# nv-tlabs/DiffusionTexturePainting

Hardware: AMD Instinct MI355X
Metric: 512x512 inpaint stamps/sec @20 DDIM steps (higher is better)
Workload: dtype f16

## Files before the change

diffusiontexturepainting_amd/_lib.py:

```python
import ctypes as C
import os

import torch

_HERE = os.path.dirname(os.path.abspath(__file__))
LIB_PATH = os.environ.get("DTP_LIB") or os.path.join(_HERE, "libdtp.so")
_lib = None
MAX_SLOTS = 16
SCHEDULERS = {"DDIM": 0, "DPM": 1, "LMSD": 2}
SCHED_ROW = 8


def scheduler_id(name):
    if name not in SCHEDULERS:
        raise ValueError(f"scheduler {name!r} is not supported: choose one of {', '.join(SCHEDULERS)}")
    return SCHEDULERS[name]


class DtpError(RuntimeError):
    pass


class Settings(C.Structure):
    _fields_ = [("steps", C.c_int), ("context_pad", C.c_int), ("tg_steps", C.c_int), ("cfg_weight", C.c_float),
# ... 85 lines not shown
                                   "host_ids_offset", "host_tiles_offset", "host_bytes")]


class ProfRow(C.Structure):
    _fields_ = [("kind", C.c_int), ("launches", C.c_int), ("ms", C.c_double), ("flops", C.c_double), ("bytes", C.c_double)]


_SHAPES = [(128, 128), (128, 64), (64, 64), (64, 128)]
PROF_KINDS = [f"gemm_kernel<{_SHAPES[i & 3][0]}, {_SHAPES[i & 3][1]}, {2 + i // 4}>" for i in range(12)] + \
    ["attention_kernel", "groupnorm (gn_stats+gn_apply | gn_fused)", "layernorm_kernel", "concat_kernel / small elementwise",
     "softmax_rows_kernel", "conv_halo_kernel<8, 16, 64>", "conv_halo_kernel<8, 16, 128>", "conv_halo_kernel<8, 8, 64>",
     "conv_halo_kernel<8, 8, 128>", "gemm_kernel<256, 128, 2>", "gemm_kernel<256, 128, 3>", "gemm_kernel<128, 256, 2>",
     "gemm_kernel<128, 256, 3>", "gemm_wide_kernel<256, 256>", "gemm_wide_kernel<256, 320>", "gemm_fp8_kernel"] + \
    [f"gemm_kernel<{_SHAPES[i & 3][0]}, {_SHAPES[i & 3][1]}, {2 + i // 4}, 2>" for i in range(8)] + \
    [f"gemm_kernel<{_SHAPES[i & 3][0]}, {_SHAPES[i & 3][1]}, 3, 1, {(4, 8)[i // 4]}>" for i in range(8)] + \
    ["xattn_kernel (cross-attention GEMM pair)", "conv_halo_kernel<8, 8, 64, 3 images>", "conv_halo_kernel<8, 8, 128, 3 images>",
     "lnlin_kernel (activation-stationary LayerNorm-folded Linear / GEGLU)", "convws_kernel<8, 8, 3 images>", "convws_kernel<16, 16>", "convws_kernel<8, 16, 2 n-tiles>", "convws_kernel<8, 16, 2 n-tiles, 2 workgroups per CU>",
     "gemmws_kernel (weight-streaming dense GEMM)", "gemm_f8f8_kernel (two-operand e4m3 GEMM)", "quant8_kernel (e4m3 quantise pass)"]


class GemmDesc(C.Structure):
    _fields_ = [("A", C.c_void_p), ("W", C.c_void_p), ("C", C.c_void_p), ("bias", C.c_void_p), ("R", C.c_void_p),
                ("M", C.c_int), ("N", C.c_int), ("K", C.c_int),
                ("lda", C.c_int), ("ldw", C.c_int), ("ldc", C.c_int), ("ldr", C.c_int),
                ("conv", C.c_int), ("Hi", C.c_int), ("Wi", C.c_int), ("Ho", C.c_int), ("Wo", C.c_int), ("Cin", C.c_int),
                ("stride", C.c_int), ("pad", C.c_int), ("upsample2x", C.c_int),
                ("flags", C.c_int), ("tile", C.c_int), ("splits", C.c_int), ("lns", C.c_void_p), ("ln_eps", C.c_float),
                ("A2", C.c_void_p), ("lda2", C.c_int), ("Cin2", C.c_int), ("Wcb", C.c_void_p),
                ("batch", C.c_int), ("a_bs", C.c_int64), ("w_bs", C.c_int64), ("c_bs", C.c_int64), ("r_bs", C.c_int64),
                ("bias_bs", C.c_int), ("lns_bs", C.c_int), ("sm_valid", C.c_int),
                ("st_out", C.c_void_p), ("st_in", C.c_void_p), ("st_parts", C.c_int), ("st_parts_out", C.c_int),
                ("W8", C.c_void_p), ("ldw8", C.c_int), ("a_scale", C.c_float), ("w_scale", C.c_float), ("gn_cpg", C.c_int), ("Wfr", C.c_void_p),
                ("A8", C.c_void_p), ("lda8", C.c_int), ("A2_8", C.c_void_p), ("lda2_8", C.c_int), ("C8", C.c_void_p), ("ldc8", C.c_int),
                ("c_scale", C.c_float), ("a2_scale", C.c_float)]


GF_BIAS, GF_BIAS_M, GF_RESID, GF_GEGLU, GF_GELU, GF_QUICKGELU, GF_OUT_F32, GF_SILU, GF_LNFOLD = 1, 2, 4, 8, 64, 128, 256, 512, 1024
GF_SOFTMAX16 = 4096
GF_ROWSTATS = 2048
GF_GNSTATS = 1 << 24
GF_RAGGED = 1 << 25

_vp, _i, _f, _i64 = C.c_void_p, C.c_int, C.c_float, C.c_int64
SYMBOLS = {
    "dtp_abi_version": (_i, []),
    "dtp_last_error": (C.c_char_p, []),
    "dtp_create": (_i, [_i, _i, _i, C.POINTER(_vp)]),
    "dtp_destroy": (None, [_vp]),
    "dtp_load_tensor": (_i, [_vp, C.c_char_p, _vp, _i, C.POINTER(_i64), _i]),
    "dtp_finalize_weights": (_i, [_vp]),
    "dtp_vae_encode": (_i, [_vp, _vp, _vp, _vp, _i, _vp]),
    "dtp_unet": (_i, [_vp, _vp, _f, _vp, _vp, _i, _vp]),
    "dtp_vae_decode": (_i, [_vp, _vp, _vp, _i, _vp]),
    "dtp_set_brush": (_i, [_vp, _vp, _i, _i, _vp, _vp]),
    "dtp_set_conditioning": (_i, [_vp, _vp, _vp, _vp, _vp]),
    "dtp_get_conditioning": (_i, [_vp, _vp, _vp, _vp]),
    "dtp_stamp": (_i, [_vp, _vp, C.POINTER(Settings), _vp, _vp, _vp, _i, _vp]),
    "dtp_stamp_slots": (_i, [_vp, _vp, C.POINTER(Settings), _vp, _vp, _vp, _i, C.POINTER(_i), _vp]),
    "dtp_stamp_mixed": (_i, [_vp, _vp, C.POINTER(Settings), _vp, _vp, _vp, _i, C.POINTER(_i), _vp]),
    "dtp_set_brush_slot": (_i, [_vp, _i, _vp, _i, _i, _vp, _vp]),
    "dtp_set_conditioning_slot": (_i, [_vp, _i, _vp, _vp, _vp, _vp]),
    "dtp_get_conditioning_slot": (_i, [_vp, _i, _vp, _vp, _vp]),
    "dtp_ddim_tables": (_i, [_i, C.POINTER(_i64), C.POINTER(_f), C.POINTER(_f)]),
    "dtp_last_stamp_times": (_i, [_vp, C.POINTER(_f * 3)]),
    "dtp_last_stamp_info": (_i, [_vp, C.POINTER(_i), C.POINTER(_i)]),
    "dtp_last_stamp_unet_rows": (_i, [_vp, C.POINTER(_i)]),
    "dtp_profile": (_i, [_vp, _i]),
    "dtp_profile_rows": (_i, [_vp, C.POINTER(ProfRow), _i, C.POINTER(_i)]),
    "dtp_profile_dump": (_i, [_vp, C.c_char_p]),
    "dtp_set_option": (_i, [_vp, C.c_char_p, _i]),
    "dtp_last_stamp_finite": (_i, [_vp, C.POINTER(_i)]),
    "dtp_op_gemm": (_i, [C.POINTER(GemmDesc), _vp]),
    "dtp_op_gemm_f8f8": (_i, [C.POINTER(GemmDesc), _vp]),
    "dtp_op_quant_e4m3": (_i, [_vp, _i, _vp, _i, _i, _f, _i, _vp, _i, _vp, _i, _i, _f, _i, _i, _vp, _i, _f, _vp]),
    "dtp_op_pack_linear": (_i, [_vp, _vp, _i, _i, _i, _i, _vp]),
    "dtp_op_pack_conv": (_i, [_vp, _vp, _i, _i, _i, _i, _i, _vp]),
    "dtp_op_rowsum": (_i, [_vp, _i, _i, _vp, _i, _vp]),
    "dtp_op_quantize_w8": (_i, [_vp, _i, _i, _i, _vp, _i, C.POINTER(_f), _vp]),
    "dtp_op_pack_conv_cb": (_i, [_vp, _vp, _i, _i, _i, _vp]),
    "dtp_op_groupnorm_apply": (_i, [_vp, _i, _vp, _i, _vp, _vp, _vp, _i, _i, _i, _i, _i, _f, _i, _vp]),
    "dtp_op_groupnorm_stats_apply": (_i, [_vp, _i, _vp, _vp, _vp, _vp, _vp, _vp, _i, _i, _i, _i, _f, _i, _vp]),
    "dtp_op_pack_conv_ws": (_i, [_vp, _vp, _vp, _i, _i, _i, _vp]),
    "dtp_op_pack_conv_ws_elems": (C.c_longlong, [_i, _i, _i]),
    "dtp_op_pack_linear_ws": (_i, [_vp, _i, _vp, _i, _i, _vp]),
    "dtp_op_pack_linear_ws_elems": (C.c_longlong, [_i, _i]),
    "dtp_op_groupnorm": (_i, [_vp, _i, _vp, _i, _vp, _vp, _i, _i, _i, _i, _f, _i, _vp]),
    "dtp_op_measure_peaks": (_i, [C.POINTER(C.c_double), C.POINTER(C.c_double)]),
    "dtp_op_reduce_groupnorm": (_i, [_vp, _i, _vp, _vp, _vp, _vp, _vp, _vp, _i, _i, _i, _i, _f, _i, _vp]),
    "dtp_op_xattn": (_i, [_vp, _vp, _vp, _vp, _vp, _i, _vp, _vp, _vp, _vp, _vp, _i, _i, _i, _i, _f, _vp]),
    "dtp_op_reduce_groupnorm_cx": (_i, [_vp, _i, _vp, _vp, _vp, _vp, _vp, _vp, _i, _i, _i, _i, _f, _i, _i, _vp]),
    "dtp_op_xattn_ct": (_i, [_vp, _vp, _vp, _vp, _vp, _i, _vp, _vp, _vp, _vp, _vp, _i, _i, _i, _i, _f, _i, _vp]),
    "dtp_op_gn_fold_weights": (_i, [_vp, _vp, _i, _vp, _vp, _vp, _i, _i, _i, _i, _i, _f, _vp, _vp, _vp]),
    "dtp_op_ffchain": (_i, [_vp, _vp, _i, _vp, _vp, _vp, _i, _vp, _vp, _vp, _i, _i, _f, _vp]),
    "dtp_op_xchain": (_i, [_vp, _vp, _i, _vp, _vp, _vp, _vp, _vp, _vp, _vp, _vp, _vp, _i, _i, _i, _i, _f, _vp]),
    "dtp_op_gn_linear": (_i, [_vp, _vp, _i, _vp, _vp, _vp, _i, _i, _i, _i, _i, _f, _vp, _vp, _i, _vp]),
    "dtp_op_layernorm": (_i, [_vp, _i, _vp, _i, _vp, _vp, _i, _i, _f, _vp]),
    "dtp_op_attention": (_i, [_vp, _vp, _vp, _vp, _i, _i, _i, _i, _i, _i, _i, _i, _i, _i64, _i64, _i64, _i64, _f, _vp]),
    "dtp_op_attention_dma": (_i, [_vp, _vp, _vp, _vp, _i, _i, _i, _i, _i, _i, _i, _i, _i, _i64, _i64, _i64, _i64, _f, _i, _vp]),
    "dtp_op_softmax_rows": (_i, [_vp, _i, _vp, _i, _i, _i, _f, _vp]),
    "dtp_op_attention_fp8": (_i, [_vp, _vp, _vp, _vp, _i, _i, _i, _i, _i, _i, _i, _i, _i, _i64, _i64, _i64, _i64, _f, _f, _f, _vp]),
    "dtp_op_dilate": (_i, [_vp, _vp, _vp, _i, _i, _i, _vp]),
    "dtp_op_dilate_pads": (_i, [_vp, _vp, _vp, _i, _i, C.POINTER(_i), _vp]),
    "dtp_scheduler_tables": (_i, [_i, _i, C.POINTER(_i), C.POINTER(_f), C.POINTER(_f), C.POINTER(_f), C.POINTER(_f)]),
    "dtp_op_sched_step": (_i, [_i, _vp, _vp, _vp, _vp, _vp, _vp, _vp, _vp, _vp, _i, _i, _i, _i, _vp]),
    "dtp_stamp_strength": (_i, [_vp, _vp, C.POINTER(Settings), _vp, _vp, _vp, C.c_double, _vp, _i, C.POINTER(_i), _vp]),
    "dtp_strength_schedule": (_i, [_i, _i, C.c_double, C.POINTER(_i), C.POINTER(_i), C.POINTER(_f)]),
    "dtp_op_strength_init": (_i, [_vp, _vp, _f, _f, _vp, C.c_longlong, _vp]),
    "dtp_stamp_seeded": (_i, [_vp, _vp, C.POINTER(Settings), C.POINTER(C.c_uint64), _i, C.c_double, _vp, _i, C.POINTER(_i), _vp]),
    "dtp_op_stamp_noise": (_i, [C.c_uint64, _i, _vp, C.c_longlong, _vp]),
    "dtp_philox4x32": (_i, [C.POINTER(C.c_uint32), C.POINTER(C.c_uint32), C.POINTER(C.c_uint32)]),
    "dtp_refit_stage": (_i, [_vp, C.c_char_p, _vp, _i, C.POINTER(_i64), _i]),
    "dtp_refit_lora": (_i, [_vp, _f]),
    "dtp_last_refit_info": (_i, [_vp, C.POINTER(_i), C.POINTER(_i), C.POINTER(_f)]),
    "dtp_op_lora_refit": (_i, [_vp, _vp, _vp, _i, _f, _vp, _vp, _i, _i, _i, _i, _vp]),
    "dtp_stroke": (_i, [_vp, _vp, _i, _i, C.POINTER(StrokeStamp), _i, C.POINTER(Settings), C.POINTER(StrokeOpts), _vp, _vp]),
    "dtp_stroke_plan": (_i, [_i, _i, _i, _i, C.POINTER(StrokeStamp), _i, _i, C.POINTER(_i), C.POINTER(_i)]),
    "dtp_last_stroke_info": (_i, [_vp, C.POINTER(_i), C.POINTER(_i), C.POINTER(_i)]),
    "dtp_op_stroke_gather": (_i, [_vp, _i, _i, _vp, _i, _i, C.POINTER(_i), C.POINTER(_i), C.POINTER(_i), _i, _i, _i, _vp]),
    "dtp_op_stroke_paste": (_i, [_vp, _vp, _vp, _i, _i, _i, _i, C.POINTER(_i), C.POINTER(_i), C.POINTER(_i), _i, _vp]),
    "dtp_mesh_create": (_i, [_vp, _vp, _i, _vp, _i, _vp, C.POINTER(_vp)]),
    "dtp_mesh_destroy": (_i, [_vp]),
    "dtp_mesh_camera": (_i, [C.POINTER(_f * 3), C.POINTER(_f * 3), C.POINTER(_f * 3), _f, C.POINTER(_f * 12)]),
    "dtp_mesh_stroke": (_i, [_vp, _vp, _vp, _i, _i, C.POINTER(MeshStamp), _i, C.POINTER(Settings), C.POINTER(MeshStrokeOpts), _vp, _vp]),
    "dtp_op_mesh_render": (_i, [_vp, C.POINTER(_f * 12), _f, _i, _vp, _i, _i, _i, _i, _i, _i, _vp, _vp, _vp]),
    "dtp_op_mesh_backproject": (_i, [_vp, _vp, _i, _vp, _vp, _i, _vp, _i, _i, _vp]),
    "dtp_mesh_stroke_bleed": (_i, [_vp, _vp, _vp, _i, _i, C.POINTER(MeshStamp), _i, C.POINTER(Settings), C.POINTER(MeshStrokeOpts), _vp, _i, _vp]),
    "dtp_mesh_bleed": (_i, [_vp, _vp, _i, _i, _i, C.POINTER(_i * 4), _vp]),
    "dtp_op_mesh_coverage": (_i, [_vp, _i, _i, _vp, _vp]),
    "dtp_mesh_bleed_offsets": (_i, [_i, C.POINTER(_i), C.POINTER(C.c_byte)]),
    "dtp_mesh_pick": (_i, [_vp, C.POINTER(Ray), _i, _vp, _vp]),
    "dtp_mesh_ray_frame": (_i, [C.POINTER(_f * 3), C.POINTER(_f * 3), C.POINTER(_f * 12)]),
    "dtp_mesh_path_plan": (_i, [_vp, _i, _f, C.POINTER(PathState), _vp, _vp, _vp, _i, C.POINTER(_i)]),
    "dtp_op_mesh_pick": (_i, [_vp, C.POINTER(Ray), _i, _vp, _vp]),
    "dtp_view_camera": (_i, [C.POINTER(_f * 3), C.POINTER(_f * 3), C.POINTER(_f * 3), _f, _i, _i, _f, C.POINTER(ViewCam)]),
    "dtp_view_rays": (_i, [C.POINTER(ViewCam), _i, _i, _vp, _i, _vp]),
    "dtp_mesh_view": (_i, [_vp, _vp, _i, _i, C.POINTER(ViewCam), _i, _i, C.POINTER(ViewOpts), _vp, _vp, _vp, _vp]),
    "dtp_op_mesh_view": (_i, [_vp, _vp, _i, _i, C.POINTER(ViewCam), _i, _i, C.POINTER(ViewOpts), _vp, _vp, _vp, _i, _vp]),
    "dtp_mip_layout": (_i, [_i, _i, C.POINTER(MipLevels)]),
    "dtp_texture_mips": (_i, [_vp, _i, _i, _vp, C.c_uint64, _vp]),
    "dtp_mesh_view_mips": (_i, [_vp, _vp, _i, _i, _vp, C.POINTER(ViewCam), _i, _i, C.POINTER(ViewOpts), _vp, _vp, _vp, _vp, _vp]),
    "dtp_mesh_view_clip": (_i, [_vp, _vp, _i, _i, _vp, C.POINTER(ViewCam), _i, _i, C.POINTER(ViewOpts), _i, _vp, _vp, _vp, _vp, _vp]),
    "dtp_op_mesh_view_clip": (_i, [_vp, _vp, _i, _i, _vp, C.POINTER(ViewCam), _i, _i, C.POINTER(ViewOpts), _i, _vp, _vp, _vp, _vp, _i, _vp]),
    "dtp_mesh_view_aa": (_i, [_vp, _vp, _i, _i, _vp, C.POINTER(ViewCam), _i, _i, C.POINTER(ViewOpts), _i, _i, _i, _vp, _vp, _vp, _vp, _vp, _vp]),
    "dtp_op_mesh_view_aa": (_i, [_vp, _vp, _i, _i, _vp, C.POINTER(ViewCam), _i, _i, C.POINTER(ViewOpts), _i, _i, _i, _vp, _vp, _vp, _vp, _vp, _i,
                                 _vp]),
    "dtp_mesh_view_aniso": (_i, [_vp, _vp, _i, _i, _vp, C.POINTER(ViewCam), _i, _i, C.POINTER(ViewOpts), _i, _i, _i, _vp, _vp, _vp, _vp, _vp, _vp,
                                 _vp]),
    "dtp_op_mesh_view_aniso": (_i, [_vp, _vp, _i, _i, _vp, C.POINTER(ViewCam), _i, _i, C.POINTER(ViewOpts), _i, _i, _i, _vp, _vp, _vp, _vp, _vp, _vp,
                                    _i, _vp]),
    "dtp_mesh_select": (_i, [_vp, _vp, _i, _i, _vp, _i, _i, _vp, _i, _vp]),
    "dtp_mesh_stroke_masked": (_i, [_vp, _vp, _vp, _i, _i, C.POINTER(MeshStamp), _i, C.POINTER(Settings), C.POINTER(MeshStrokeOpts), _vp, _i, _vp, _i,
                                    _vp]),
    "dtp_view_tint": (_i, [_vp, _vp, _vp, _i, _i, _vp, _i, _i, C.POINTER(C.c_uint8 * 3), _i, _vp]),
    "dtp_op_mesh_backproject_masked": (_i, [_vp, _vp, _i, _vp, _vp, _i, _vp, _i, _i, _vp, _i, _vp]),
    "dtp_journal_create": (_i, [_vp, _vp, _i, _i, _i, _i, C.POINTER(_vp)]),
    "dtp_journal_destroy": (_i, [_vp]),
    "dtp_journal_begin": (_i, [_vp, _vp]),
    "dtp_journal_end": (_i, [_vp, _vp]),
    "dtp_journal_touch": (_i, [_vp, C.POINTER(_i), _i, _vp]),
    "dtp_journal_undo": (_i, [_vp, _vp]),
    "dtp_journal_redo": (_i, [_vp, _vp]),
    "dtp_journal_info": (_i, [_vp, C.POINTER(_i), C.POINTER(_i), C.POINTER(_i), C.POINTER(C.c_uint64)]),
    "dtp_journal_record_info": (_i, [_vp, _i, C.POINTER(C.c_uint64), C.POINTER(C.c_uint64), C.POINTER(_i)]),
    "dtp_op_journal_tiles": (_i, [_vp, _i, C.POINTER(_i), _i, C.POINTER(_i)]),
    "dtp_journal_window_tiles": (_i, [_i, _i, _i, _i, _i, _i, C.POINTER(_i), _i, C.POINTER(_i)]),
    "dtp_delta_layout": (_i, [_i, _i, _i, C.POINTER(DeltaSizes)]),
# ... 38 lines not shown
```

diffusiontexturepainting_amd/csrc/api_ops.hip:

```cpp
#include <stdarg.h>
#include <stdio.h>
#include <stdlib.h>
#include <mutex>
#include <vector>

#include "../../include/dtp.h"
#include "common.h"

static thread_local char g_err[1024] = "";

void dtp_set_error(const char* fmt, ...) {
  va_list ap;
  va_start(ap, fmt);
  vsnprintf(g_err, sizeof(g_err), fmt, ap);
  va_end(ap);
}

namespace {
struct OpsScratch {
  f16* zero = nullptr;
  float* ws = nullptr;
  size_t ws_bytes = 0;
  int* geglu_map = nullptr;
  int geglu_map_n = 0;
  int num_cu = 256;
  bool init = false;
};
OpsScratch g_ops;
std::mutex g_ops_mu;

int ops_init() {
  if (g_ops.init) return DTP_OK;
  HIP_CHECK(hipMalloc(&g_ops.zero, 256));
  HIP_CHECK(hipMemset(g_ops.zero, 0, 256));
  hipDeviceProp_t prop;
  int dev = 0;
  HIP_CHECK(hipGetDevice(&dev));
  HIP_CHECK(hipGetDeviceProperties(&prop, dev));
  g_ops.num_cu = prop.multiProcessorCount;
  g_ops.init = true;
  return DTP_OK;
}

int ops_ws(size_t bytes) {
  if (bytes <= g_ops.ws_bytes) return DTP_OK;
  HIP_CHECK(hipDeviceSynchronize());
  if (g_ops.ws) HIP_CHECK(hipFree(g_ops.ws));
  g_ops.ws = nullptr;
  g_ops.ws_bytes = 0;
  HIP_CHECK(hipMalloc(&g_ops.ws, bytes));
  g_ops.ws_bytes = bytes;
  return DTP_OK;
}
}

extern "C" {

int dtp_abi_version(void) { return DTP_ABI_VERSION; }
const char* dtp_last_error(void) { return g_err; }

int dtp_op_gemm(dtp_gemm_desc* d, dtp_stream s) {
  std::lock_guard<std::mutex> lk(g_ops_mu);
  int rc = ops_init();
  if (rc) return rc;
  static bool halo_init = false;
  if (!halo_init) { dtp_conv_halo_init(); dtp_gemm_wide_init(); dtp_lnlin_init(); dtp_conv_ws_init(); dtp_gemm_ws_init(); halo_init = true; }
  GemmParams p = {};
  p.A = (const f16*)d->A; p.W = (const f16*)d->W; p.C = d->C; p.bias = d->bias; p.R = (const f16*)d->R;
  p.zero = g_ops.zero;
  p.M = d->M; p.N = d->N; p.K = d->K;
  p.lda = d->lda; p.ldw = d->ldw; p.ldc = d->ldc; p.ldr = d->ldr;
  p.nkb = (d->K + 63) / 64;
  p.Hi = d->Hi; p.Wi = d->Wi; p.Ho = d->Ho; p.Wo = d->Wo; p.Cin = d->Cin; p.stride = d->stride; p.pad = d->pad;
  p.flags = d->flags | (d->conv ? GF_CONV3 : 0) | (d->upsample2x ? GF_UPS2 : 0);
  p.lns = d->lns; p.ln_eps = d->ln_eps;
  p.A2 = (const f16*)d->A2; p.lda2 = d->lda2; p.Cin2 = d->Cin2;
  p.batch = d->batch; p.a_bs = d->a_bs; p.w_bs = d->w_bs; p.c_bs = d->c_bs; p.r_bs = d->r_bs;
  p.bias_bs = d->bias_bs; p.lns_bs = d->lns_bs; p.sm_valid = d->sm_valid;
  p.st_out = d->st_out; p.st_in = d->st_in; p.st_parts = d->st_parts;
  if (p.batch > 1) p.st_rows = p.batch * p.M;
  p.W8 = (const unsigned char*)d->W8; p.ldw8 = d->ldw8; p.a_scale = d->a_scale; p.w_scale = d->w_scale;
  p.Wfr = (const f16*)d->Wfr;
  p.gn_cpg = d->gn_cpg;
  static bool fp8_init = false;
  if (!fp8_init) { dtp_gemm_fp8_init(); fp8_init = true; }
  if (p.ldw < p.nkb * 64) { dtp_set_error("gemm: ldw=%d smaller than padded K=%d", p.ldw, p.nkb * 64); return DTP_ERR_ARG; }
  int tile = 0;
  dtp_gemm_pick(p, &tile, g_ops.num_cu);
  if (d->tile >= 0) tile = d->tile;
  const DtpTile t = dtp_tile(tile);
  int sp = t.split == SPLIT_COLS ? 4 : t.split == SPLIT_K ? p.splits : 1;
  if (d->splits >= 1 && (d->batch <= 1 || t.split != SPLIT_K)) sp = d->splits;
  if ((t.fam == TF_FP8) != (p.W8 != nullptr)) { dtp_set_error("gemm: tiles 24..28 and W8 go together"); return DTP_ERR_ARG; }
  if (t.fam == TF_HALO && !d->Wcb) { dtp_set_error("conv_halo: Wcb missing"); return DTP_ERR_ARG; }
  p.Wcb = (const f16*)d->Wcb;
  (void)dtp_tile_apply(p, tile, sp);
  rc = ops_ws(dtp_gemm_workspace_bytes(p));
  if (rc) return rc;
  p.part = g_ops.ws;
  if (p.flags & GF_ROWSTATS) d->st_parts_out = dtp_tile_row_parts(p, tile);
  return dtp_launch_tile(p, tile, (hipStream_t)s);
}

int dtp_op_gemm_f8f8(dtp_gemm_desc* d, dtp_stream s) {
  std::lock_guard<std::mutex> lk(g_ops_mu);
  int rc = ops_init();
  if (rc) return rc;
  static bool f8f8_init = false;
  if (!f8f8_init) { dtp_gemm_f8f8_init(); f8f8_init = true; }
  GemmParams p = {};
  p.A8 = (const unsigned char*)d->A8; p.lda8 = d->lda8;
  p.A2_8 = (const unsigned char*)d->A2_8; p.lda2_8 = d->lda2_8; p.Cin2 = d->A2_8 ? d->Cin2 : 0;
  p.W8 = (const unsigned char*)d->W8; p.ldw8 = d->ldw8;
  p.C = d->C; p.ldc = d->ldc; p.C8 = (unsigned char*)d->C8; p.ldc8 = d->ldc8;
  p.bias = d->bias; p.R = (const f16*)d->R; p.ldr = d->ldr;
  p.zero = g_ops.zero;
  p.M = d->M; p.N = d->N; p.K = d->K;
  p.flags = d->flags;
  p.st_out = d->st_out;
  p.a_scale = d->a_scale; p.w_scale = d->w_scale; p.c_scale = d->c_scale; p.a2_scale = d->a2_scale;
  p.splits = 1;
  const int tile = d->tile >= 0 ? d->tile : dtp_gemm_f8f8_pick(p, g_ops.num_cu);
  if (p.flags & GF_ROWSTATS) d->st_parts_out = (p.N + 127) / 128;
  return dtp_launch_gemm_f8f8(p, tile, (hipStream_t)s);
}

int dtp_op_quant_e4m3(const void* x, int ldx, void* y, int ldy, int K, float scale, int ln, const void* x2, int ldx2, void* y2, int ldy2,
                      int K2, float scale2, int ln2, int M, const float* st_in, int st_parts, float eps, dtp_stream s) {
  Quant8Params q = {};
  q.M = M; q.njobs = x2 ? 2 : 1;
  q.job[0] = Quant8Job{(const f16*)x, ldx, K, (unsigned char*)y, ldy, scale, ln};
  if (x2) q.job[1] = Quant8Job{(const f16*)x2, ldx2, K2, (unsigned char*)y2, ldy2, scale2, ln2};
  q.st_in = st_in; q.st_parts = st_parts; q.st_rows = M; q.eps = eps;
  return dtp_launch_quant8(q, (hipStream_t)s);
}

int dtp_op_pack_linear(const float* w, void* out, int N, int K, int ldw, int geglu, dtp_stream s) {
  std::lock_guard<std::mutex> lk(g_ops_mu);
  int rc = ops_init();
  if (rc) return rc;
  const int* map = nullptr;
  if (geglu) {
    if (N % 256) { dtp_set_error("pack_linear: GEGLU needs N %% 256 == 0"); return DTP_ERR_ARG; }
    std::vector<int> h(N);
    for (int f = 0; f < N / 2; ++f) {
      h[f] = (f / 64) * 128 + (f % 64);
      h[N / 2 + f] = (f / 64) * 128 + 64 + (f % 64);
    }
    if (g_ops.geglu_map_n < N) {
      if (g_ops.geglu_map) HIP_CHECK(hipFree(g_ops.geglu_map));
      HIP_CHECK(hipMalloc(&g_ops.geglu_map, sizeof(int) * N));
      g_ops.geglu_map_n = N;
    }
    HIP_CHECK(hipMemcpyAsync(g_ops.geglu_map, h.data(), sizeof(int) * N, hipMemcpyHostToDevice, (hipStream_t)s));
    HIP_CHECK(hipStreamSynchronize((hipStream_t)s));
    map = g_ops.geglu_map;
  }
  return dtp_launch_pack_linear_weight(w, (f16*)out, N, K, ldw, map, (hipStream_t)s);
}

int dtp_op_quantize_w8(const void* w, int ldw, int K, int rows, void* out, int ldw8, float* w_scale, dtp_stream s) {
  if (!w || !out || !w_scale || (ldw8 & 127) || ldw8 < K) { dtp_set_error("quantize_w8: bad argument"); return DTP_ERR_ARG; }
  return dtp_quantize_weights_fp8((const f16*)w, ldw, K, rows, (unsigned char*)out, ldw8, w_scale, (hipStream_t)s);
}

int dtp_op_rowsum(const void* w, int ld, int K, float* out, int rows, dtp_stream s) {
  return dtp_launch_rowsum_f16((const f16*)w, ld, K, out, rows, (hipStream_t)s);
}

int dtp_op_pack_conv(const float* w, void* out, int Cout, int Cin, int Cin_pad, int taps, int ldw, dtp_stream s) {
  return dtp_launch_pack_conv_weight(w, (f16*)out, Cout, Cin, Cin_pad, taps, ldw, (hipStream_t)s);
}

int dtp_op_pack_conv_cb(const float* w, void* out, int Cout, int Cin, int ldw, dtp_stream s) {
  return dtp_launch_pack_conv_weight_cb(w, (f16*)out, Cout, Cin, ldw, (hipStream_t)s);
}

int dtp_op_pack_conv_ws(const float* w, const float* w1, void* out, int Cout, int Cin, int Cin2, dtp_stream s) {
  return dtp_launch_pack_conv_ws(w, w1, (f16*)out, Cout, Cin, Cin2, (hipStream_t)s);
}
int dtp_op_pack_linear_ws(const void* w, int ldw, void* out, int N, int K, dtp_stream s) {
  return dtp_launch_pack_linear_ws((const f16*)w, ldw, (f16*)out, N, K, (hipStream_t)s);
}
long long dtp_op_pack_linear_ws_elems(int N, int K) { return (long long)dtp_gemm_ws_packed_elems(N, K); }
long long dtp_op_pack_conv_ws_elems(int Cout, int Cin, int Cin2) { return (long long)dtp_conv_ws_packed_elems(Cout, Cin, Cin2); }

int dtp_op_groupnorm(const void* x, int ldx, void* y, int ldy, const float* gamma, const float* beta, int B, int HW, int C,
                     int groups, float eps, int silu, dtp_stream s) {
  std::lock_guard<std::mutex> lk(g_ops_mu);
  int rc = ops_init();
  if (rc) return rc;
  rc = ops_ws(dtp_groupnorm_ws_bytes(B, HW, C, groups));
  if (rc) return rc;
  return dtp_launch_groupnorm(GnParams{(const f16*)x, ldx, (f16*)y, ldy, gamma, beta, B, HW, C, groups, eps, silu}, g_ops.ws, (hipStream_t)s);
}

int dtp_op_groupnorm_apply(const void* x, int ldx, void* y, int ldy, const float* gamma, const float* beta, const float* partial, int nchunk,
                           int B, int HW, int C, int groups, float eps, int silu, dtp_stream s) {
  return dtp_launch_groupnorm_apply(GnParams{(const f16*)x, ldx, (f16*)y, ldy, gamma, beta, B, HW, C, groups, eps, silu}, partial, nchunk, (hipStream_t)s);
}

int dtp_op_reduce_groupnorm_cx(const float* part, int splits, const float* bias, const void* resid, void* conv_out, void* y, const float* gamma,
                               const float* beta, int B, int HW, int C, int groups, float eps, int silu, int cx, dtp_stream s) {
  std::lock_guard<std::mutex> lk(g_ops_mu);
  int rc = ops_init();
  if (rc) return rc;
  rc = ops_ws(dtp_groupnorm_ws_bytes(B, HW, C, groups));
  if (rc) return rc;
  if (cx <= 0 || cx > C) { dtp_set_error("reduce_groupnorm: cx %d outside (0, C = %d]", cx, C); return DTP_ERR_ARG; }
  const GnReduceSrc rd = {part, splits, (long long)B * HW * cx, cx, bias, (const f16*)resid, cx};
  return dtp_launch_reduce_groupnorm(GnParams{(const f16*)conv_out, C, (f16*)y, C, gamma, beta, B, HW, C, groups, eps, silu}, rd, cx, g_ops.ws, (hipStream_t)s);
}

int dtp_op_reduce_groupnorm(const float* part, int splits, const float* bias, const void* resid, void* conv_out, void* y, const float* gamma,
                            const float* beta, int B, int HW, int C, int groups, float eps, int silu, dtp_stream s) {
  return dtp_op_reduce_groupnorm_cx(part, splits, bias, resid, conv_out, y, gamma, beta, B, HW, C, groups, eps, silu, C, s);
}

int dtp_op_gn_fold_weights(const void* x, const void* W, int ldw, const float* bias, const float* gamma, const float* beta, int B, int HW, int C,
                           int Nout, int groups, float eps, void* Wout, float* bias_out, dtp_stream s) {
  std::lock_guard<std::mutex> lk(g_ops_mu);
  int rc = ops_init();
  if (rc) return rc;
  rc = ops_ws(dtp_groupnorm_ws_bytes(B, HW, C, groups));
  if (rc) return rc;
  const GnParams gp = {(const f16*)x, C, nullptr, 0, gamma, beta, B, HW, C, groups, eps, 0};
  rc = dtp_launch_groupnorm_stats(gp, g_ops.ws, nullptr, (hipStream_t)s);
  if (rc) return rc;
  const int rows = (Nout + 127) / 128 * 128;
  return dtp_launch_gn_fold_weights(gp, g_ops.ws, 0, (const f16*)W, ldw, bias, Nout, (f16*)Wout, (long long)rows * ldw, bias_out, rows, (hipStream_t)s);
}

int dtp_op_groupnorm_stats_apply(const float* part, int splits, const float* bias, const void* resid, void* x, void* y, const float* gamma,
                                 const float* beta, int B, int HW, int C, int groups, float eps, int silu, dtp_stream s) {
  if (part && splits < 1) { dtp_set_error("groupnorm_stats_apply: %d slabs", splits); return DTP_ERR_ARG; }
  std::lock_guard<std::mutex> lk(g_ops_mu);
  int rc = ops_init();
  if (rc) return rc;
  rc = ops_ws(dtp_groupnorm_ws_bytes(B, HW, C, groups));
  if (rc) return rc;
  const GnParams gp = {(const f16*)x, C, (f16*)y, C, gamma, beta, B, HW, C, groups, eps, silu};
  const GnReduceSrc rd = {part, splits, (long long)B * HW * C, C, bias, (const f16*)resid, C};
  rc = dtp_launch_groupnorm_stats(gp, g_ops.ws, part ? &rd : nullptr, (hipStream_t)s);
  if (rc) return rc;
  return dtp_launch_groupnorm_apply(gp, g_ops.ws, dtp_groupnorm_stat_chunks(HW), (hipStream_t)s);
}

int dtp_op_gn_linear(const void* x, const void* W, int ldw, const float* bias, const float* gamma, const float* beta, int B, int HW, int C,
                     int Nout, int groups, float eps, void* y, float* st_out, int col_ranges, dtp_stream s) {
  std::lock_guard<std::mutex> lk(g_ops_mu);
  int rc = ops_init();
  if (rc) return rc;
  static bool init = false;
  if (!init) { dtp_lnlin_init(); init = true; }
  if (groups != 32) { dtp_set_error("gn_linear: 32 groups (got %d)", groups); return DTP_ERR_ARG; }
  rc = ops_ws(dtp_groupnorm_ws_bytes(B, HW, C, groups));
  if (rc) return rc;
  rc = dtp_launch_groupnorm_stats(GnParams{(const f16*)x, C, nullptr, 0, gamma, beta, B, HW, C, groups, eps, 0}, g_ops.ws, nullptr, (hipStream_t)s);
  if (rc) return rc;
  GemmParams p = {};
  p.A = (const f16*)x; p.lda = C; p.W = (const f16*)W; p.ldw = ldw; p.nkb = ldw / 64;
  p.M = HW; p.N = Nout; p.K = C; p.C = y; p.ldc = Nout;
  p.bias = bias; p.flags = (bias ? GF_BIAS : 0) | GF_GNAPPLY | (st_out ? GF_ROWSTATS : 0);
  p.batch = B; p.a_bs = (long long)HW * C; p.c_bs = (long long)HW * Nout; p.w_bs = 0; p.bias_bs = 0;
  p.st_out = st_out; p.st_rows = B * HW;
  p.gn_part = g_ops.ws; p.gn_gamma = gamma; p.gn_beta = beta; p.gn_nchunk = dtp_groupnorm_stat_chunks(HW); p.gn_cpg = C / groups; p.gn_eps = eps;
  p.zero = g_ops.zero;
  return dtp_launch_lnlin(p, col_ranges >= 1 ? col_ranges : 4, (hipStream_t)s);
// ... 99 lines not shown
```

diffusiontexturepainting_amd/csrc/builder.hip:

```cpp
#include "engine.h"

#include <math.h>
#include <stdio.h>

#include <algorithm>

static Op make_gemm_op(Ctx* c, GemmParams p, int tile, int bias_step_off);

static const float* step_bias(const Ctx* c, int bias_step_off, int step, const float* fallback) {
  return bias_step_off >= 0 ? c->temb_table + (size_t)step * c->unet.temb_total + bias_step_off : fallback;
}
static constexpr int GF_CLAIMABLE = GF_BIAS | GF_RESID | GF_CONV3 | GF_UPS2 | GF_MFAST | GF_RAGGED;

void prog_push(Ctx* c, Prog* prog, int kind, double flops, double bytes, Op fn, const std::string& label) {
  prog->last_gemm.valid = false;
  prog->ops.push_back([=](hipStream_t s, int step) -> int {
    if (!c->profile) return fn(s, step);
    ProfRec r;
    r.kind = kind; r.flops = flops; r.bytes = bytes; r.label = label.c_str();
    HIP_CHECK(hipEventCreate(&r.e0));
    HIP_CHECK(hipEventCreate(&r.e1));
    HIP_CHECK(hipEventRecord(r.e0, s));
    const int rc = fn(s, step);
    HIP_CHECK(hipEventRecord(r.e1, s));
// ... 23 lines not shown
  if ((p.flags & ~GF_CLAIMABLE) || !(p.flags & GF_CONV3) || p.batch > 1) return false;
  if ((p.N % 32) || p.N / 32 < 4 || p.N / 32 > 64) return false;
  if (!(p.flags & GF_RAGGED) && ((p.Ho & 7) || (p.Wo & 15))) return false;
  if (dtp_conv_ws_gn_chunks(p.Ho, p.Wo) > 1024) return false;
  return true;
}

static void* pool_get_clear_of(Ctx* c, size_t need, const std::vector<MemRange>& ranges, int attempts = 6) {
  std::vector<void*> aside;
  void* got = nullptr;
  for (int attempt = 0; attempt < attempts; ++attempt) {
    void* pp = nullptr;
    if (ctx_pool_get(c, need, &pp) != DTP_OK) break;
    bool hit = false;
    for (const MemRange& r : ranges)
      if (r.p && r.bytes && (const char*)pp < (const char*)r.p + r.bytes && (const char*)r.p < (const char*)pp + need) { hit = true; break; }
    if (!hit) { got = pp; break; }
    aside.push_back(pp);
  }
  for (void* q : aside) ctx_pool_put(c, q);
  return got;
}
static std::vector<MemRange> gemm_operand_ranges(const GemmParams& gp, long long images) {
  const size_t in_bytes = (gp.flags & GF_CONV3) ? (size_t)images * gp.Hi * gp.Wi * gp.lda * sizeof(f16) : (size_t)gp.M * gp.lda * sizeof(f16);
  return {{gp.A, in_bytes}, {gp.A2, gp.A2 ? (size_t)gp.M * gp.lda2 * sizeof(f16) : 0}, {gp.R, gp.R ? (size_t)gp.M * gp.ldr * sizeof(f16) : 0}};
}

ReduceClaim Builder::claim_reduce(const T& x, bool allow_concat) {
  const LastGemm lg = prog->last_gemm;
  const bool whole = lg.p.N == x.C;
  const bool front = allow_concat && lg.p.N < x.C && (lg.p.N & 7) == 0 && x.H * x.W <= 256 && dtp_reduce_groupnorm_supported(x.H * x.W, x.C, 32);
  if (!(c->fuse_reduce_gn && lg.valid && lg.p.splits > 1 && (f16*)lg.p.C == x.p && lg.p.ldc == x.ld && lg.p.M == (int)x.rows() && (whole || front) &&
        !(lg.p.flags & ~GF_CLAIMABLE) && lg.p.batch <= 1 && (x.C & 7) == 0))
    return ReduceClaim();
  if (!dtp_groupnorm_reduce_accepts(x.C, 32, x.ld, lg.p.N, (lg.p.flags & GF_RESID) ? lg.p.ldr : 0)) return ReduceClaim();
  ReduceClaim claim = {true, lg.p, lg.bias_step_off};
  claim.p.flags |= GF_NOREDUCE;
  prog->ops[lg.op_index] = Op();
  prog->ops.pop_back();
  prog_push(c, prog, lg.kind, lg.flops, lg.bytes, make_gemm_op(c, claim.p, lg.tile, lg.bias_step_off), lg.label + " (reduce in gn)");
  return claim;
}

size_t ReduceClaim::slab_bytes() const { return claimed ? ((dtp_gemm_workspace_bytes(p) + 255) & ~(size_t)255) : 0; }
std::vector<MemRange> ReduceClaim::busy() const {
  return claimed && (p.flags & GF_RESID) ? std::vector<MemRange>{{p.R, (size_t)p.M * p.ldr * sizeof(f16)}} : std::vector<MemRange>();
}
GnReduceSrc ReduceClaim::src(const Ctx* c, int step) const {
  const float* bias = (p.flags & GF_BIAS) ? step_bias(c, bias_step_off, step, p.bias) : nullptr;
  return {c->ws, p.splits, (long long)p.M * p.N, p.N, bias, (p.flags & GF_RESID) ? p.R : nullptr, p.ldr};
}

static void* block_clear_of_claim(Ctx* c, size_t bytes, const ReduceClaim& claim, const char* who, const char* what) {
  void* p = pool_get_clear_of(c, bytes, claim.busy());
  if (!p) dtp_set_error("%s: no %s block clear of the claimed reduce's residual", who, what);
  return p;
}

static GnParams gn_params(const T& x, const NormW& n, float eps, bool silu, const T* y = nullptr) {
  return {x.p, x.ld, y ? y->p : nullptr, y ? y->ld : 0, n.g, n.b, x.B, x.H * x.W, x.C, 32, eps, silu ? 1 : 0};
}
static std::string gn_label(const GnParams& gp) { return " B=" + std::to_string(gp.B) + " HW=" + std::to_string(gp.HW) + " C=" + std::to_string(gp.C); }

static void push_gn_stats(Builder& b, const GnParams& gp, float* part, const ReduceClaim& claim, const char* label_suffix) {
  Ctx* cc = b.c;
  const size_t slab_bytes = claim.slab_bytes();
  b.push(PK_GN, 0.0, 2.0 * (double)gp.B * gp.HW * gp.C, [=](hipStream_t s, int step) {
    const GnReduceSrc rd = claim.src(cc, step);
    return dtp_launch_groupnorm_stats(gp, part ? part : (float*)((char*)cc->ws + slab_bytes), claim ? &rd : nullptr, s);
  }, (claim ? "reduce+gn-stats" : "gn-stats") + gn_label(gp) + label_suffix);
}

static bool emit_rowstats(GemmParams& p, const RowStats* emit) {
  if (!emit || !emit->buf) return false;
  p.flags |= GF_ROWSTATS;
  p.st_out = emit->buf; p.st_rows = (p.batch > 1 ? p.batch : 1) * p.M;
  if (emit->rows_total > 0) { p.st_out = emit->buf + (size_t)emit->row_off * 2; p.st_rows = emit->rows_total; }
  return true;
}

bool Builder::claim_stats(const T& x, float** partials, int* nchunk) {
  const LastGemm lg = prog->last_gemm;
  const DtpTile t = dtp_tile(lg.tile);
  if (!c->gn_epilogue || !lg.valid || t.fam != TF_CONVWS || t.var < 2 || lg.p.splits != 1 || (f16*)lg.p.C != x.p || lg.p.ldc != x.ld ||
      lg.p.M != (int)x.rows() || lg.p.N != x.C || !dtp_conv_output_can_carry_gn_stats(lg.p))
    return false;
  GemmParams gp = lg.p;
  const int chunks = dtp_conv_ws_gn_chunks(gp.Ho, gp.Wo);
  const size_t need = (size_t)x.B * chunks * 32 * 2 * sizeof(float);
  void* pp = pool_get_clear_of(c, need, gemm_operand_ranges(gp, x.B), 4);
  if (!pp) return false;
  gp.flags |= GF_GNSTATS;
  gp.st_out = (float*)pp;
  gp.gn_cpg = x.C / 32;
  if (!dtp_conv_ws_supported(gp, t.var, 1)) { ctx_pool_put(c, pp); return false; }
  prog->ops.pop_back();
  prog_push(c, prog, lg.kind, lg.flops, lg.bytes, make_gemm_op(c, gp, lg.tile, lg.bias_step_off), lg.label + " (+gn stats)");
  *partials = (float*)pp;
  *nchunk = chunks;
  return true;
}

int Builder::gn(const T& x, const NormW& n, float eps, bool silu, T& y) {
  Ctx* cc = c;
  const ReduceClaim claim = claim_reduce(x, cc->reduce_in_concat_gn);
  y = T();
  y.B = x.B; y.H = x.H; y.W = x.W; y.C = x.C; y.ld = x.C;
  y.p = (f16*)block_clear_of_claim(cc, (size_t)x.B * x.H * x.W * x.C * sizeof(f16), claim, "gn", "output");
  if (!y.p) return DTP_ERR_HIP;
  const size_t slab_bytes = claim.slab_bytes();
  cc->ws_need = std::max(cc->ws_need, slab_bytes + dtp_groupnorm_ws_bytes(x.B, x.H * x.W, x.C, 32));
  const GnParams gp = gn_params(x, n, eps, silu, &y);
  const double bytes = 4.0 * (double)x.rows() * x.C;
  if (claim) {
    const int Cx = claim.p.N;
    push(PK_GN, 0.0, bytes, [=](hipStream_t s, int step) {
      return dtp_launch_reduce_groupnorm(gp, claim.src(cc, step), Cx, (float*)((char*)cc->ws + slab_bytes), s);
    }, (Cx < x.C ? "reduce(front " + std::to_string(Cx) + ")+gn" : std::string("reduce+gn")) + gn_label(gp) + " splits=" + std::to_string(claim.p.splits));
    return DTP_OK;
  }
  float* partials = nullptr;
  int nchunk = 0;
  if (claim_stats(x, &partials, &nchunk)) {
    push(PK_GN, 0.0, bytes, [=](hipStream_t s, int) { return dtp_launch_groupnorm_apply(gp, partials, nchunk, s); }, "gn-apply" + gn_label(gp));
    ctx_pool_put(cc, partials);
    return DTP_OK;
  }
  push(PK_GN, 0.0, bytes, [=](hipStream_t s, int) { return dtp_launch_groupnorm(gp, cc->ws, s); }, "gn" + gn_label(gp));
  return DTP_OK;
}

bool Builder::gn_linear_supported(const T& x, const ConvW& w) const {
  const int HW = x.H * x.W, C = x.C;
  return c->fold_gn_linear && HW >= 1024 && w.taps == 1 && w.K == C && w.ldw == C && (C % 64) == 0 && C <= 2048 && (C % 32) == 0 && !w.lns &&
         !(fp8 && w.w8) && C / 32 >= 8;
}

int Builder::gn_linear(const T& x, const NormW& n, float eps, const ConvW& w, T& y, RowStats* emit) {
  Ctx* cc = c;
  const int HW = x.H * x.W, C = x.C, N = x.B, Cp = (w.cout + 127) / 128 * 128;
  const GnParams gp = gn_params(x, n, eps, false);
  const ReduceClaim claim = claim_reduce(x);
  float* ep_part = nullptr;
  int ep_chunks = 0;
  const bool from_epilogue = !claim && claim_stats(x, &ep_part, &ep_chunks);
  const size_t slab_bytes = claim.slab_bytes();
  cc->ws_need = std::max(cc->ws_need, slab_bytes + dtp_groupnorm_ws_bytes(N, HW, C, 32));
  GemmParams lin = {};
  lin.A = x.p; lin.lda = x.ld; lin.ldw = w.ldw; lin.nkb = w.ldw / 64;
  lin.M = HW; lin.N = w.cout; lin.K = w.K;
  lin.batch = N; lin.a_bs = (long long)HW * x.ld;
  if (cc->gna_lnlin && (C == 320 || C == 640) && (HW & 127) == 0 && !fp8) {
    GemmParams g = lin;
    g.W = w.w; g.bias = w.b; g.flags = (w.b ? GF_BIAS : 0) | GF_GNAPPLY;
    g.c_bs = (long long)HW * w.cout;
    g.gn_gamma = n.g; g.gn_beta = n.b; g.gn_eps = eps; g.gn_cpg = C / 32;
    g.gn_nchunk = from_epilogue ? ep_chunks : dtp_groupnorm_stat_chunks(HW);
    g.gn_part = (const float*)x.p;
    g.ldc = w.cout;
    if (lnlin_default_ranges(g) > 0) {
      float* part = ep_part;
      if (!from_epilogue) {
        part = (float*)block_clear_of_claim(cc, dtp_groupnorm_ws_bytes(N, HW, C, 32), claim, "gn_linear", "partials");
        if (!part) return DTP_ERR_HIP;
        push_gn_stats(*this, gp, part, claim, " (apply in proj_in)");
      }
      g.gn_part = part;
      y = alloc(x.B, x.H, x.W, w.cout);
      if (!y.p) return DTP_ERR_HIP;
      g.C = y.p; g.ldc = y.ld; g.c_bs = (long long)HW * y.ld;
      RC(push_gemm(cc, prog, g, -1, (double)w.K, emit));
      ctx_pool_put(cc, part);
      return DTP_OK;
    }
  }
  void *pw = nullptr, *pb = nullptr;
  RC(ctx_pool_get(cc, (size_t)N * Cp * w.ldw * sizeof(f16), &pw));
  RC(ctx_pool_get(cc, (size_t)N * Cp * sizeof(float), &pb));
// ... 39 lines not shown
  Fp8Cal r;
  r.kind = 0; r.slot0 = c->fp8_nslots; r.s0 = &c->fp8_scales.back();
  c->fp8_cals.push_back(r);
  *slot1 = ++c->fp8_nslots;
  return r.s0;
}

int fp8_calibrate(Ctx* c, UNetProg* up, hipStream_t s, int step) {
  if (up->fp8_calibrated || up->cal_begin == up->cal_end) { up->fp8_calibrated = true; return DTP_OK; }
  if (!c->fp8_amax) { void* p; RC(ctx_persistent(c, DTP_FP8_SLOTS * sizeof(unsigned int), &p, true)); c->fp8_amax = (unsigned int*)p; }
  HIP_CHECK(hipMemsetAsync(c->fp8_amax, 0, DTP_FP8_SLOTS * sizeof(unsigned int), s));
  c->calibrating = true;
  const int rc = up->main.run(s, step);
  c->calibrating = false;
  RC(rc);
  std::vector<float> amax(DTP_FP8_SLOTS);
  HIP_CHECK(hipMemcpyAsync(amax.data(), c->fp8_amax, DTP_FP8_SLOTS * sizeof(float), hipMemcpyDeviceToHost, s));
  HIP_CHECK(hipStreamSynchronize(s));
  auto pow2_for = [](float a) { return a > 0.f ? exp2f(ceilf(log2f(a * DTP_FP8_MARGIN / 448.0f))) : 1.0f; };
  for (size_t i = up->cal_begin; i < up->cal_end; ++i) {
    Fp8Cal& r = c->fp8_cals[i];
    if (r.kind == 0) {
      *r.s0 = pow2_for(amax[r.slot0]);
    } else {
      const float aq = amax[r.slot0] * r.softmax_scale * 1.4426950408889634f, ak = amax[r.slot0 + 1], av = amax[r.slot0 + 2];
      *r.s0 = (aq > 0.f && ak > 0.f) ? exp2f(roundf(0.5f * log2f(ak / aq))) : 1.0f;
      *r.s1 = pow2_for(av);
    }
  }
  up->fp8_calibrated = true;
  return DTP_OK;
}

static Op make_gemm_op(Ctx* c, GemmParams p, int tile, int bias_step_off) {
  return [=](hipStream_t s, int step) -> int {
    GemmParams q = p;
    q.part = c->ws;
    if (p.a_scale_host) {
      if (c->calibrating && p.amax_slot1 > 0) {
        const int ka = p.A2 ? p.K - p.Cin2 : p.K;
        RC(dtp_launch_amax_f16(p.A, p.M, ka, p.lda, c->fp8_amax + p.amax_slot1 - 1, s));
        if (p.A2) RC(dtp_launch_amax_f16(p.A2, p.M, p.Cin2, p.lda2, c->fp8_amax + p.amax_slot1 - 1, s));
      }
      q.a_scale = *p.a_scale_host;
    }
    q.bias = step_bias(c, bias_step_off, step, q.bias);
    return dtp_launch_tile(q, tile, s);
  };
}

int push_gemm(Ctx* c, Prog* prog, GemmParams p, int bias_step_off, double k_alg, RowStats* emit) {
  if (!emit_rowstats(p, emit)) emit = nullptr;
  int tile = 0;
  dtp_gemm_pick(p, &tile, c->num_cu);
  int sp = p.splits;
  if (p.W8) { tile = 24 + ((p.flags & GF_GEGLU) ? (p.M >= 512 ? 0 : 3) : (p.M >= 512 ? 0 : 2)); sp = 1; }
  if ((p.flags & GF_GNAPPLY) && (p.flags & GF_CONV3)) { tile = (p.Hi * p.Wi <= 256) ? 14 : 12; sp = 1; }
  if ((p.flags & GF_GNAPPLY) && !(p.flags & GF_CONV3)) {
    tile = DTP_TILE_LNLIN;
    sp = lnlin_default_ranges(p);
    if (!sp) { dtp_set_error("push_gemm: no lnlin configuration for the GroupNorm-on-load Linear (M %d N %d K %d)", p.M, p.N, p.K); return DTP_ERR_ARG; }
  }
  if (c->autotune) RC(tune_gemm(c, p, &tile, &sp));
  (void)dtp_tile_apply(p, tile, sp);
  const DtpTile t = dtp_tile(tile);
  if (emit) {
    emit->parts = dtp_tile_row_parts(p, tile);
    emit->M = p.M * (p.batch > 1 ? p.batch : 1);
  }
  c->ws_need = std::max(c->ws_need, dtp_gemm_workspace_bytes(p));
  p.zero = c->zero;
  const double n_out = (p.flags & GF_GEGLU) ? p.N / 2.0 : (double)p.N;
  const double a_elems = (p.flags & GF_CONV3) ? (double)p.M * (k_alg / 9.0) * ((p.flags & GF_UPS2) ? 0.25 : (double)(p.stride * p.stride))
                                               : (double)p.M * k_alg;
  const double nb = p.batch > 1 ? (double)p.batch : 1.0;
  const double bytes = 2.0 * nb * (a_elems + (double)p.N * k_alg + (double)p.M * n_out);
  char lab[160];
  const bool f8tile = t.fam == TF_FP8;
  snprintf(lab, sizeof(lab), "%s M=%d N=%d K=%d tile=%d splits=%d%s%s%s%s", (p.flags & GF_CONV3) ? "conv3" : "gemm", p.M, p.N, p.K, tile,
           t.split == SPLIT_COLS ? p.col_ranges : p.splits, (p.flags & GF_UPS2) ? " ups" : "", (p.flags & GF_GEGLU) ? (f8tile ? " geglu fp8" : " geglu") : (f8tile ? " fp8" : ""), p.stride == 2 ? " s2" : "",
           p.batch > 1 ? (" x" + std::to_string(p.batch)).c_str() : "");
  const double flops = 2.0 * nb * p.M * (double)p.N * k_alg;
  prog_push(c, prog, t.pk, flops, bytes, make_gemm_op(c, p, tile, bias_step_off), lab);
  if (p.splits > 1 || (t.fam == TF_CONVWS && t.var >= 2)) {
    LastGemm& lg = prog->last_gemm;
    lg.valid = true; lg.p = p; lg.tile = tile; lg.bias_step_off = bias_step_off; lg.op_index = prog->ops.size() - 1;
    lg.kind = t.pk; lg.flops = flops; lg.bytes = bytes; lg.label = lab;
  }
  return DTP_OK;
}

int Builder::conv3(const T& x, const ConvW& w, int stride, int pad, bool ups, int Ho, int Wo, const T* resid, int bias_step_off, T& y,
                   const Conv3Opts& o) {
  if ((w.cin2 > 0) != (o.tail != nullptr) || (o.tail && o.tail->C != w.cin2)) { dtp_set_error("conv3: shortcut tail mismatch"); return DTP_ERR_ARG; }
  if (x.C != w.cin || w.taps != 9) { dtp_set_error("conv3: channel mismatch %d vs %d", x.C, w.cin); return DTP_ERR_ARG; }
  GemmParams p = {};
  p.A = x.p; p.W = w.w;
  p.M = x.B * Ho * Wo; p.N = w.cout; p.K = w.K;
  p.lda = x.ld; p.ldw = w.ldw;
  p.nkb = w.ldw / 64;
  p.Hi = x.H; p.Wi = x.W; p.Ho = Ho; p.Wo = Wo; p.Cin = w.cin; p.stride = stride; p.pad = pad;
  p.flags = GF_CONV3 | (ups ? GF_UPS2 : 0) | o.extra_flags;
  if (c->R % 64) p.flags |= GF_RAGGED;
  if (o.tail) { p.A2 = o.tail->p; p.lda2 = o.tail->ld; p.Cin2 = w.cin2; }
  p.Wcb = w.wcb;
  p.Wfr = w.wfr;
  if (o.extra_flags & GF_GNAPPLY) {
    if (!o.gn.part) { dtp_set_error("conv3: GF_GNAPPLY without GroupNorm parameters"); return DTP_ERR_ARG; }
    p.gn_part = o.gn.part; p.gn_gamma = o.gn.gamma; p.gn_beta = o.gn.beta; p.gn_eps = o.gn.eps;
    p.gn_nchunk = o.gn.nchunk; p.gn_cpg = o.gn.cpg; p.gn_silu = 1;
  }
  if (o.out_override) {
    y = T();
    y.p = (f16*)o.out_override; y.B = x.B; y.H = Ho; y.W = Wo; y.C = w.cout; y.ld = o.ldc_override;
  } else if (o.dst) {
    if (o.dst->C != w.cout || o.dst->rows() != (long long)x.B * Ho * Wo) { dtp_set_error("conv3: destination view mismatch"); return DTP_ERR_ARG; }
    y = *o.dst;
  } else {
    y = alloc(x.B, Ho, Wo, w.cout);
    if (!y.p) return DTP_ERR_HIP;
  }
  p.C = y.p; p.ldc = y.ld;
  if (w.b || bias_step_off >= 0) { p.flags |= GF_BIAS; p.bias = w.b; }
  if (resid) { p.flags |= GF_RESID; p.R = resid->p; p.ldr = resid->ld; }
  return push_gemm(c, prog, p, bias_step_off, 9.0 * w.cin_true + w.cin2);
}

int Builder::gn_conv3(const T& x, const NormW& n, float eps, const ConvW& w, const T* resid, int bias_step_off, T& y, const T* tail, const T* dst) {
  Ctx* cc = c;
  const int HW = x.H * x.W, C = x.C;
  Conv3Opts opts;
  opts.tail = tail; opts.dst = dst;
  const bool fuse = cc->fuse_gn_conv && HW >= 1024 && x.rows() <= 16384 && w.wcb && w.taps == 9 && (C & 63) == 0 && C <= 1024 && x.C == w.cin && (C % 32) == 0 && C / 32 >= 8 &&
                    (w.cout & 7) == 0 && (x.ld & 7) == 0;
  if (!fuse) {
    T t;
    RC(gn(x, n, eps, true, t));
    RC(conv3(t, w, 1, 1, false, x.H, x.W, resid, bias_step_off, y, opts));
    release(t);
    return DTP_OK;
  }
  const ReduceClaim claim = claim_reduce(x);
  float* partials = (float*)block_clear_of_claim(cc, dtp_groupnorm_ws_bytes(x.B, HW, C, 32), claim, "gn_conv3", "partials");
  if (!partials) return DTP_ERR_HIP;
  cc->ws_need = std::max(cc->ws_need, claim.slab_bytes());
  push_gn_stats(*this, gn_params(x, n, eps, true), partials, claim, " (apply in conv)");
  opts.extra_flags = GF_GNAPPLY; opts.gn = {partials, n.g, n.b, eps, dtp_groupnorm_stat_chunks(HW), C / 32};
  const int rc = conv3(x, w, 1, 1, false, x.H, x.W, resid, bias_step_off, y, opts);
  ctx_pool_put(cc, partials);
  return rc;
}

int Builder::alloc_stats(long long rows, int C, RowStats& st) {
  void* p = nullptr;
  RC(ctx_pool_get(c, (size_t)((C + 63) / 64) * rows * 2 * sizeof(float), &p));
  st.buf = (float*)p;
  st.parts = 0;
  st.M = (int)rows;
  return DTP_OK;
}
void Builder::release_stats(RowStats& st) { ctx_pool_put(c, st.buf); st.buf = nullptr; }

int Builder::linear(const T& x, const ConvW& w, const T* resid, int flags, T& y, RowStats* emit, const RowStats* use, const T* dst) {
  if (x.C != w.K || w.taps != 1) { dtp_set_error("linear: K mismatch %d vs %d", x.C, w.K); return DTP_ERR_ARG; }
  GemmParams p = {};
  p.A = x.p; p.W = w.w; p.Wfr = w.wfr;
  p.M = (int)x.rows(); p.N = w.cout; p.K = w.K;
  p.lda = x.ld; p.ldw = w.ldw; p.nkb = w.ldw / 64;
  p.flags = flags;
  if (dst) {
    if (dst->C != w.cout || (flags & GF_GEGLU) || dst->rows() != x.rows()) { dtp_set_error("linear: destination view mismatch"); return DTP_ERR_ARG; }
    y = *dst;
  } else {
    y = alloc(x.B, x.H, x.W, (flags & GF_GEGLU) ? w.cout / 2 : w.cout);
    if (!y.p) return DTP_ERR_HIP;
  }
  p.C = y.p; p.ldc = y.ld;
  if (w.b) { p.flags |= GF_BIAS; p.bias = w.b; }
  if (w.lns) {
    p.flags |= GF_LNFOLD; p.lns = w.lns; p.ln_eps = 1e-5f;
    if (use && use->buf && use->parts > 0 && use->M == p.M) { p.st_in = use->buf; p.st_parts = use->parts; }
  }
  if (resid) { p.flags |= GF_RESID; p.R = resid->p; p.ldr = resid->ld; }
  if (fp8 && w.w8) {
    GemmParams q = p;
    q.W8 = w.w8; q.ldw8 = w.ldw8; q.w_scale = w.w8_scale; q.splits = 1;
    q.a_scale = (p.flags & GF_LNFOLD) ? DTP_FP8_LN_A_SCALE : DTP_FP8_LN_A_SCALE * 8.0f;
    if (dtp_gemm_fp8_supported(q)) {
      if (!(p.flags & GF_LNFOLD) && (q.K & 7) == 0) q.a_scale_host = fp8_new_linear_scale(c, &q.amax_slot1);
// ... 146 lines not shown
```

diffusiontexturepainting_amd/csrc/common.h:

```cpp
#pragma once
#include <hip/hip_runtime.h>
#include <stdint.h>

#include "../../include/dtp.h"

typedef _Float16 f16;
typedef f16 f16x2 __attribute__((ext_vector_type(2)));
typedef f16 f16x4 __attribute__((ext_vector_type(4)));
typedef f16 f16x8 __attribute__((ext_vector_type(8)));
typedef float f32x4 __attribute__((ext_vector_type(4)));
typedef float f32x16 __attribute__((ext_vector_type(16)));

static __device__ __forceinline__ uint32_t lds_addr(const void* p) {
  return (uint32_t)(uintptr_t)(const __attribute__((address_space(3))) void*)p;
}
static __device__ __forceinline__ f16x8 lds_read16(uint32_t addr) {
  f16x8 v;
  asm volatile("ds_read_b128 %0, %1" : "=v"(v) : "v"(addr));
  return v;
}
template <int N, int NF>
static __device__ __forceinline__ void wait_lds_frags(f16x8 (&f)[NF]) {
  static_assert(NF == 2 || NF == 3 || NF == 4 || NF == 5 || NF == 6 || NF == 7 || NF == 8, "fragment count");
  if constexpr (NF == 2) asm volatile("s_waitcnt lgkmcnt(%2)" : "+v"(f[0]), "+v"(f[1]) : "n"(N));
// ... 150 lines not shown
}

#define DTP_WAVE 64

#define HIP_CHECK(x)                                                                        \
  do {                                                                                      \
    hipError_t e_ = (x);                                                                    \
    if (e_ != hipSuccess) {                                                                 \
      dtp_set_error("%s:%d %s -> %s", __FILE__, __LINE__, #x, hipGetErrorString(e_));       \
      return DTP_ERR_HIP;                                                                   \
    }                                                                                       \
  } while (0)


void dtp_set_error(const char* fmt, ...);

enum {
  GF_BIAS = 1,
  GF_BIAS_M = 2,
  GF_RESID = 4,
  GF_GEGLU = 8,
  GF_CONV3 = 16,
  GF_UPS2 = 32,
  GF_GELU = 64,
  GF_QUICKGELU = 128,
  GF_OUT_F32 = 256,
  GF_SILU = 512,
  GF_LNFOLD = 1024,
  GF_ROWSTATS = 2048,
  GF_SOFTMAX16 = 4096,
  GF_MFAST = 1 << 20,
  GF_NOREDUCE = 1 << 21,
  GF_XCDSPLIT = 1 << 23,
  GF_GNSTATS = 1 << 24,
  GF_RAGGED = 1 << 25,
  GF_GNAPPLY = 1 << 22,
};

struct GemmParams {
  const f16* A;
  const f16* W;
  const f16* Wcb;
  const f16* Wfr;
  void* C;
  float* part;
  const float* bias;
  const f16* R;
  const f16* zero;
  const float* lns;
  float ln_eps;
  const float* st_in;
  int st_parts;
  float* st_out;
  int M, N, K;
  int lda, ldw, ldc, ldr;
  int nkb;
  int splits;
  int kb_per_split;
  int col_ranges;
  int Hi, Wi, Ho, Wo, Cin, stride, pad;
  const f16* A2;
  int lda2, Cin2;
  int flags;
  int batch;
  long long a_bs, w_bs, c_bs, r_bs;
  int bias_bs, lns_bs, st_rows;
  int sm_valid;
  const float *gn_part, *gn_gamma, *gn_beta;
  int gn_nchunk, gn_cpg, gn_silu;
  float gn_eps;
  const unsigned char* W8;
  int ldw8;
  float a_scale, w_scale;
  const float* a_scale_host;
  int amax_slot1;
  const unsigned char* A8;
  int lda8;
  const unsigned char* A2_8;
  int lda2_8;
  unsigned char* C8;
  int ldc8;
  float c_scale;
  float a2_scale;
};

struct Quant8Job {
  const f16* x; int ld, K;
  unsigned char* y; int ldy;
  float scale;
  int ln;
};
struct Quant8Params {
  int M, njobs;
  Quant8Job job[2];
  const float* st_in; int st_parts, st_rows;
  float eps;
};
bool dtp_quant8_supported(const Quant8Params& q);
int dtp_launch_quant8(const Quant8Params& q, hipStream_t s);
bool dtp_gemm_f8f8_supported(const GemmParams& p);
int dtp_gemm_f8f8_pick(const GemmParams& p, int num_cu);
int dtp_launch_gemm_f8f8(const GemmParams& p, int tile, hipStream_t s);
void dtp_gemm_f8f8_init();

static inline bool dtp_xcd_split_ok(int tiles, int splits) {
  if (splits < 2 || (splits & (splits - 1)) || splits > 32) return false;
  return splits >= 8 || (tiles % (8 / splits)) == 0;
}
static __device__ __forceinline__ void dtp_xcd_split(int id, int tiles, int splits, int& tile, int& z) {
  const int xcd = id & 7, idx = id >> 3;
  if (splits >= 8) { const int r = splits >> 3; z = xcd + 8 * (idx % r); tile = idx / r; }
  else { const int g = 8 / splits; z = xcd % splits; tile = idx * g + xcd / splits; }
}

int dtp_launch_gemm(const GemmParams& p, int tile, hipStream_t s);
void dtp_gemm_init();
int dtp_launch_tile(const GemmParams& p, int tile, hipStream_t s);
int dtp_launch_splitk_reduce(const GemmParams& p, hipStream_t s);
size_t dtp_gemm_workspace_bytes(const GemmParams& p);
void dtp_gemm_pick(GemmParams& p, int* tile, int num_cu);

struct GnParams {
  const f16* x; int ldx; f16* y; int ldy; const float *gamma, *beta; int B, HW, C, groups; float eps; int silu;
};
struct GnReduceSrc {
  const float* part; int splits; long long slab; int ldp; const float* bias; const f16* R; int ldr;
};
int dtp_launch_groupnorm(const GnParams& p, float* stats_ws, hipStream_t s);
size_t dtp_groupnorm_ws_bytes(int B, int HW, int C, int groups);
int dtp_groupnorm_stat_chunks(int HW);
int dtp_launch_groupnorm_apply(const GnParams& p, const float* partial, int nchunk, hipStream_t s);
int dtp_launch_groupnorm_stats(const GnParams& p, float* ws, const GnReduceSrc* rd, hipStream_t s);
bool dtp_reduce_groupnorm_supported(int HW, int C, int groups);
int dtp_launch_reduce_groupnorm(const GnParams& p, const GnReduceSrc& rd, int Cx, float* stats_ws, hipStream_t s);
bool dtp_groupnorm_reduce_accepts(int C, int groups, int ldx, int ldp, int ldr);
int dtp_launch_gn_fold_weights(const GnParams& p, const float* partial, int nchunk, const f16* W, int ldw, const float* bias, int Nout, f16* Wout,
                               long long w_bs, float* bias_out, int bias_bs, hipStream_t s);
int dtp_launch_layernorm(const f16* x, int ldx, f16* y, int ldy, const float* gamma, const float* beta, int rows, int C,
                         float eps, hipStream_t s);
int dtp_launch_softmax_rows(const f16* x, int ldx, f16* y, int ldy, int rows, int cols, float scale, hipStream_t s);

struct AttnParams {
  const f16 *Q, *K, *V;
  f16* O;
  int ldq, ldk, ldv, ldo;
  int B, H, Sq, Skv, D;
  long long qbs, kbs, vbs, obs;
  float scale;
  int prio;
  int skew;
};
int dtp_launch_attention(const AttnParams& p, hipStream_t s);
bool dtp_attention_uses_dma(const AttnParams& p);
bool dtp_attention_dma_supported(const AttnParams& p);
int dtp_launch_attention_dma(const AttnParams& p, hipStream_t s, int nw_force = 0);
int dtp_launch_attention_fp8(const AttnParams& p, float q_scale, float v_scale, hipStream_t s);

struct XattnParams {
  const f16* X; int ldx;
  const f16* W1; long long w1_bs;
  const float *b1, *lns1;
  const float* st_in; int st_parts, st_rows; float ln_eps;
  const f16* W2; long long w2_bs;
  const float* b2;
  const f16* R; int ldr;
  f16* Y; int ldy;
  float* st_out;
  int S, C, N, sm_valid;
  const f16* zero;
  int ct;
};
int dtp_xattn_tiles_per_wg(int S, int C, int N);
bool dtp_xattn_supported(const XattnParams& p);
int dtp_launch_xattn(const XattnParams& p, hipStream_t s);
void dtp_xattn_init();

struct XchainParams {
  const f16* A; int lda;
  const f16* Wo; int ldwo;
  const float* bo;
  const f16* Y; int ldy;
  const f16* W1; long long w1_bs;
  const float *b1, *lns1;
  const f16* W2; long long w2_bs;
  const float* b2;
  f16* Y3; int ldy3;
  float* st_out;
  int S, C, N, sm_valid;
  float ln_eps;
  int dup;
};
bool dtp_xchain_supported(const XchainParams& p);
int dtp_launch_xchain(const XchainParams& p, hipStream_t s);
void dtp_xchain_init();

struct FfchainParams {
  const f16* X; int ldx;
  const f16* W1; int ldw1;
  const float *lns1, *b1;
  const f16* Wm; int ldwm;
  const float* bm;
  const f16* R; int ldr;
  f16* Out; int ldo;
  int M, C;
  float ln_eps;
};
bool dtp_ffchain_supported(const FfchainParams& p);
int dtp_launch_ffchain(const FfchainParams& p, hipStream_t s);
void dtp_ffchain_init();

int dtp_launch_concat_channels(const f16* a, int lda, int Ca, const f16* b, int ldb, int Cb, f16* y, int ldy, long long rows,
                               hipStream_t s);
#define DTP_COPY_SEGS 8
struct CopySegs {
  int n;
  const char* src[DTP_COPY_SEGS];
  char* dst[DTP_COPY_SEGS];
  long long rows[DTP_COPY_SEGS], row_bytes[DTP_COPY_SEGS], src_stride[DTP_COPY_SEGS], dst_stride[DTP_COPY_SEGS];
  long long chunks[DTP_COPY_SEGS], total;
};
int dtp_launch_copy_rows(CopySegs segs, hipStream_t s);
int dtp_launch_f32_to_f16(const float* x, f16* y, long long n, hipStream_t s);
int dtp_launch_nchw_f32_to_nhwc_f16(const float* x, f16* y, int B, int C, int HW, int Cpad, hipStream_t s);
int dtp_launch_nhwc_f16_to_nchw_f32(const f16* x, int ldx, float* y, int B, int C, int HW, hipStream_t s);
int dtp_launch_pack_conv_weight(const float* w, f16* out, int Cout, int Cin, int Cin_pad, int taps, int ldw, hipStream_t s);
int dtp_launch_pack_linear_weight(const float* w, f16* out, int N, int K, int ldw, const int* row_map, hipStream_t s);
int dtp_launch_rowdot(const float* w, const float* v, float* out, int N, int K, hipStream_t s);
int dtp_launch_scale_cols(float* w, const float* g, int N, int K, hipStream_t s);
int dtp_launch_rowsum_f16(const f16* w, int ld, int K, float* out, int rows, hipStream_t s);
int dtp_launch_matmul_f32(const float* A, const float* B, float* C, int M, int N, int K, hipStream_t s);
int dtp_launch_expand_kv(const f16* kv, f16* kexp, f16* vexp, int N, int T, int C, int H, float scale, hipStream_t s);
int dtp_launch_transpose_f16(const f16* src, int lds_, f16* dst, int ldd, int rows, int cols, hipStream_t s);
int dtp_launch_rowdot_f16(const f16* a, int ld, const float* v, float* out, int rows, int K, hipStream_t s);
bool dtp_gemm_fp8_supported(const GemmParams& p);
int dtp_launch_gemm_fp8(const GemmParams& p, int tile, hipStream_t s);
void dtp_gemm_fp8_init();
int dtp_quantize_weights_fp8(const f16* w, int ldw, int K, int rows, unsigned char* out, int ldw8, float* scale_out, hipStream_t s);
bool dtp_gemm_wide_supported(const GemmParams& p, int variant);
int dtp_launch_gemm_wide(const GemmParams& p, int variant, hipStream_t s);
void dtp_gemm_wide_init();
constexpr int DTP_TILE_LNLIN = 50;
constexpr int DTP_TILE_WS0 = 51;
constexpr int DTP_WS_VARIANTS = 4;
constexpr int DTP_TILE_GEMMWS = 55;
constexpr int DTP_TILE_IDS = 56;

enum { PK_GEMM0 = 0, PK_ATTN = 12, PK_GN = 13, PK_LN = 14, PK_ELEM = 15, PK_SOFTMAX = 16, PK_HALO0 = 17, PK_BIG0 = 21, PK_WIDE0 = 25, PK_FP8 = 27, PK_KH2 = 28, PK_LW = 36, PK_XATTN = 44, PK_HALO3 = 45, PK_LNLIN = 47, PK_WS0 = 48, PK_GEMMWS = 52, PK_F8F8 = 53, PK_QUANT8 = 54, PK_COUNT = 55 };

enum DtpFamily : unsigned char { TF_NONE, TF_GEMM, TF_HALO, TF_WIDE, TF_FP8, TF_LNLIN, TF_CONVWS, TF_GEMMWS };
enum DtpSplit : unsigned char {
  SPLIT_K,
  SPLIT_HALO,
  SPLIT_BLOCKS,
  SPLIT_COLS,
  SPLIT_NONE,
};
struct DtpTile {
  DtpFamily fam;
  int var;
  int bm, bn, ns;
  int kh, lw;
  DtpSplit split;
  int pk;
};
inline DtpTile dtp_tile(int id) {
  static constexpr int sm[4] = {128, 128, 64, 64}, sn[4] = {128, 64, 64, 128};
  const int s = id & 3;
  if (id >= 0 && id < 12) return {TF_GEMM, 0, sm[s], sn[s], 2 + id / 4, 1, 0, SPLIT_K, PK_GEMM0 + id};
  if (id >= 12 && id < 16) return {TF_HALO, id - 12, 0, 0, 0, 0, 0, SPLIT_HALO, PK_HALO0 + id - 12};
  if (id >= 16 && id < 20) return {TF_GEMM, 0, id < 18 ? 256 : 128, id < 18 ? 128 : 256, 2 + (id & 1), 1, 0, SPLIT_K, PK_BIG0 + id - 16};
  if (id == 20 || id == 21) return {TF_WIDE, id - 20, 256, id == 20 ? 256 : 320, 2, 0, 0, SPLIT_NONE, PK_WIDE0 + id - 20};
  if (id >= 24 && id < 28) return {TF_FP8, id - 24, sm[s], sn[s], 2, 0, 0, SPLIT_NONE, PK_FP8};
  if (id == 28) return {TF_FP8, 4, 256, 256, 2, 0, 0, SPLIT_NONE, PK_FP8};
  if (id >= 32 && id < 40) return {TF_GEMM, 0, sm[s], sn[s], 2 + (id - 32) / 4, 2, 0, SPLIT_K, PK_KH2 + id - 32};
  if (id >= 40 && id < 48) return {TF_GEMM, 0, sm[s], sn[s], 3, 1, id < 44 ? 4 : 8, SPLIT_K, PK_LW + id - 40};
  if (id == 48 || id == 49) return {TF_HALO, id - 44, 0, 0, 0, 0, 0, SPLIT_HALO, PK_HALO3 + id - 48};
  if (id == DTP_TILE_LNLIN) return {TF_LNLIN, 0, 0, 0, 0, 0, 0, SPLIT_COLS, PK_LNLIN};
  if (id >= DTP_TILE_WS0 && id < DTP_TILE_WS0 + DTP_WS_VARIANTS) return {TF_CONVWS, id - DTP_TILE_WS0, 0, 0, 0, 0, 0, SPLIT_BLOCKS, PK_WS0 + id - DTP_TILE_WS0};
  if (id == DTP_TILE_GEMMWS) return {TF_GEMMWS, 0, 64, 64, 0, 0, 0, SPLIT_BLOCKS, PK_GEMMWS};
  return {};
}
inline bool dtp_tile_apply(GemmParams& p, int tile, int sp) {
  const DtpTile t = dtp_tile(tile);
  if (sp < 1) sp = 1;
  if (t.fam == TF_HALO) p.W = p.Wcb;
  if (t.split == SPLIT_NONE || t.split == SPLIT_COLS) {
    p.kb_per_split = p.nkb; p.splits = 1;
    if (t.split == SPLIT_COLS) p.col_ranges = sp;
    return t.split == SPLIT_COLS || sp == 1;
  }
  p.kb_per_split = (p.nkb + sp - 1) / sp;
  if (t.split == SPLIT_BLOCKS) { p.splits = sp; return true; }
  if (t.split == SPLIT_HALO && sp > 1) p.kb_per_split = (((p.nkb + 8) / 9 + sp - 1) / sp) * 9;
  p.splits = (p.nkb + p.kb_per_split - 1) / p.kb_per_split;
  return p.splits == sp;
}
inline int dtp_tile_row_parts(const GemmParams& p, int tile) {
  const DtpTile t = dtp_tile(tile);
  if (t.split == SPLIT_COLS) return p.col_ranges;
  if (!t.bn) return 0;
  return p.splits > 1 ? 1 : (p.N + t.bn - 1) / t.bn;
}
bool dtp_lnlin_supported(const GemmParams& p, int nsplit);
int dtp_launch_lnlin(const GemmParams& p, int nsplit, hipStream_t s);
void dtp_lnlin_init();
bool dtp_conv_ws_supported(const GemmParams& p, int variant, int nsplit);
int dtp_launch_conv_ws(const GemmParams& p, int variant, hipStream_t s);
void dtp_conv_ws_init();
size_t dtp_conv_ws_packed_elems(int Cout, int Cin, int Cin2);
int dtp_conv_ws_gn_chunks(int Ho, int Wo);
int dtp_launch_pack_conv_ws(const float* w, const float* w1, f16* out, int Cout, int Cin, int Cin2, hipStream_t s);
bool dtp_gemm_ws_supported(const GemmParams& p, int nsplit);
int dtp_launch_gemm_ws(const GemmParams& p, hipStream_t s);
void dtp_gemm_ws_init();
size_t dtp_gemm_ws_packed_elems(int N, int K);
int dtp_launch_pack_linear_ws(const f16* w, int ldw, f16* out, int N, int K, hipStream_t s);
bool dtp_conv_halo_supported(const GemmParams& p);
bool dtp_conv_halo3_supported(const GemmParams& p);
int dtp_launch_conv_halo(const GemmParams& p, int variant, hipStream_t s);
void dtp_conv_halo_init();
int dtp_launch_pack_conv_weight_cb(const float* w, f16* out, int Cout, int Cin, int ldw, hipStream_t s);
int dtp_launch_touch(const void* p, size_t bytes, float* sink, hipStream_t s);
int dtp_launch_amax_f16(const f16* x, long long rows, int cols, int ld, unsigned int* slot, hipStream_t s);
int dtp_launch_lora_merge(float* w, const float* up, const float* down, int N, int K, int rank, float scale, hipStream_t s);
```

diffusiontexturepainting_amd/csrc/context.hip:

```cpp
#include <stdio.h>
#include <stdlib.h>
#include <string.h>
#include <algorithm>

#include "engine.h"

int stamp_init(Ctx* c) {
  void* p;
  const size_t hw = (size_t)c->h * c->h, RR = (size_t)c->R * c->R;
  RC(ctx_persistent(c, c->maxB * hw * 4 * 4, &p, true)); c->x32 = (float*)p;
  RC(ctx_persistent(c, 3 * c->maxB * hw * 4 * 4, &p, true)); c->hist32 = (float*)p;
  RC(ctx_persistent(c, c->maxB * 4 * RR * 4, &p, true)); c->canvas32 = (float*)p;
  RC(ctx_persistent(c, 2 * c->maxB * RR * 4, &p, true)); c->alpha_tmp = (float*)p;
  RC(ctx_persistent(c, sizeof(StampParams), &p, true)); c->stamp_params = (StampParams*)p;
  RC(ctx_persistent(c, (size_t)DTP_MAX_SLOTS * 2 * 14 * 768 * 4, &p, true)); c->cond32 = (float*)p;
  RC(ctx_persistent(c, (size_t)DTP_MAX_SLOTS * 3 * RR * 4, &p, true)); c->brush32 = (float*)p;
  RC(ctx_persistent(c, 64 * sizeof(int), &p, true)); c->slot_map = (int*)p;
  RC(ctx_persistent(c, 256, &p, true)); c->finite_flag = (int*)p;
  RC(ctx_persistent(c, RR * 4, &p, true)); c->mesh_face_idx = (int*)p;
  return DTP_OK;
}

extern "C" {

int dtp_create(int device, int resolution, int max_batch, dtp_ctx** out) {
  if (!out || resolution < 64 || resolution % 8 || max_batch < 1 || max_batch > 64) {
    dtp_set_error("dtp_create: resolution must be a multiple of 8 and at least 64, 1 <= max_batch <= 64 (got resolution %d, max_batch %d)", resolution, max_batch);
    return DTP_ERR_ARG;
  }
  HIP_CHECK(hipSetDevice(device));
  Ctx* c = new Ctx();
  c->device = device; c->R = resolution; c->h = resolution / 8; c->maxB = max_batch;
  hipDeviceProp_t prop;
  HIP_CHECK(hipGetDeviceProperties(&prop, device));
  c->num_cu = prop.multiProcessorCount;
  void* z;
  HIP_CHECK(hipMalloc(&z, 4096));
  HIP_CHECK(hipMemset(z, 0, 4096));
  c->zero = (f16*)z;
  for (int i = 0; i < 4; ++i) HIP_CHECK(hipEventCreate(&c->ev[i]));
  tune_cache_load(c);
  auto on = [](const char* name) { const char* e = getenv(name); return e && e[0] && e[0] != '0'; };
  c->fuse_reduce_gn = !on("DTP_NO_FUSE_REDUCE_GN"); c->dedupe_prefix = !on("DTP_NO_DEDUPE");
#ifdef DTP_EXPERIMENTAL
  c->fuse_gn_conv = on("DTP_GN_CONV");
#endif
  c->fuse_xattn = !on("DTP_NO_XATTN"); c->fold_gn_linear = !on("DTP_NO_FOLD_GN");
  c->conv_ws = !on("DTP_NO_WS"); c->conv_ws_vae = !on("DTP_NO_WS_VAE"); c->gemm_ws = on("DTP_GEMMWS");
  c->gn_epilogue = !on("DTP_NO_GN_EPILOGUE"); c->reduce_in_concat_gn = !on("DTP_NO_REDUCE_IN_CONCAT_GN"); c->gna_lnlin = !on("DTP_NO_GNA_LNLIN");
  c->tune_lnlin = !on("DTP_NO_LNLIN"); c->tune_halo3 = !on("DTP_NO_HALO3");
  c->xchain = !on("DTP_NO_XCHAIN"); c->xattn_tiles = !on("DTP_XATTN_CT1");
  if (const char* e = getenv("DTP_FFCHAIN")) c->ffchain = atoi(e);
  *out = (dtp_ctx*)c;
  return DTP_OK;
}

void dtp_destroy(dtp_ctx* ctx) {
  Ctx* c = (Ctx*)ctx;
  if (!c) return;
  (void)hipSetDevice(c->device);
  (void)hipDeviceSynchronize();
  graphs_drop_all(c);
  journal_drop_ctx(c);
  delta_drop_ctx(c);
  mesh_drop_ctx(c);
  for (auto& s : c->staged) (void)hipFree(s.second.d);
  for (auto& s : c->refit_staged) (void)hipFree(s.second.d);
  for (int i = 0; i < 2; ++i) if (c->refit_ev[i]) (void)hipEventDestroy(c->refit_ev[i]);
  for (void* p : c->chunks) (void)hipFree(p);
  for (auto& b : c->pool.blocks) (void)hipFree(b.p);
  for (void* p : c->persistent) (void)hipFree(p);
  if (c->ws) (void)hipFree(c->ws);
  if (c->zero) (void)hipFree(c->zero);
  if (c->tune_thrash) (void)hipFree(c->tune_thrash);
  for (int i = 0; i < 4; ++i) if (c->ev[i]) (void)hipEventDestroy(c->ev[i]);
  delete c;
}

int dtp_load_tensor(dtp_ctx* ctx, const char* name, const float* data, int is_device, const int64_t* shape, int ndim) {
  Ctx* c = (Ctx*)ctx;
  if (!c || !name || !data || ndim < 1 || ndim > 4) { dtp_set_error("dtp_load_tensor: bad argument"); return DTP_ERR_ARG; }
  if (c->finalized) { dtp_set_error("dtp_load_tensor: weights already finalized"); return DTP_ERR_STATE; }
  HIP_CHECK(hipSetDevice(c->device));
  Staged s;
  s.n = 1;
  for (int i = 0; i < ndim; ++i) { s.shape.push_back(shape[i]); s.n *= (size_t)shape[i]; }
  HIP_CHECK(hipMalloc(&s.d, std::max<size_t>(s.n * 4, 16)));
  HIP_CHECK(hipMemcpy(s.d, data, s.n * 4, is_device ? hipMemcpyDeviceToDevice : hipMemcpyHostToDevice));
  auto it = c->staged.find(name);
  if (it != c->staged.end()) { (void)hipFree(it->second.d); c->staged.erase(it); }
  c->staged.emplace(name, std::move(s));
  return DTP_OK;
}

int dtp_finalize_weights(dtp_ctx* ctx) {
  Ctx* c = (Ctx*)ctx;
  if (!c) { dtp_set_error("dtp_finalize_weights: null handle"); return DTP_ERR_ARG; }
  if (c->finalized) { dtp_set_error("dtp_finalize_weights: already finalized"); return DTP_ERR_STATE; }
  HIP_CHECK(hipSetDevice(c->device));
  dtp_gemm_init();
  dtp_conv_halo_init();
  dtp_gemm_wide_init();
  dtp_gemm_fp8_init();
  dtp_gemm_f8f8_init();
  dtp_xattn_init();
  dtp_lnlin_init();
  dtp_xchain_init();
  dtp_ffchain_init();
  dtp_conv_ws_init();
  dtp_gemm_ws_init();
  RC(load_unet_weights(c));
  RC(load_vae_weights(c));
  bool has_clip = false;
  for (auto& kv : c->staged)
    if (kv.first.rfind("clip.", 0) == 0) { has_clip = true; break; }
  if (has_clip) RC(load_imgenc_weights(c));
  HIP_CHECK(hipDeviceSynchronize());
  for (auto& s : c->staged) (void)hipFree(s.second.d);
  c->staged.clear();
  RC(stamp_init(c));
  c->finalized = true;
  return DTP_OK;
}

int dtp_set_conditioning_slot(dtp_ctx* ctx, int slot, const float* cond, const float* uncond, const float* brush, dtp_stream s_) {
  Ctx* c = (Ctx*)ctx;
  hipStream_t s = (hipStream_t)s_;
  if (!c || !c->finalized || !cond || !uncond || !brush) { dtp_set_error("dtp_set_conditioning: bad state/argument"); return DTP_ERR_STATE; }
  if (slot < 0 || slot >= DTP_MAX_SLOTS) { dtp_set_error("dtp_set_conditioning: slot %d outside 0..%d", slot, DTP_MAX_SLOTS - 1); return DTP_ERR_ARG; }
  HIP_CHECK(hipSetDevice(c->device));
  float* dst = c->cond32 + (size_t)slot * 2 * 14 * 768;
  HIP_CHECK(hipMemcpyAsync(dst, cond, 14 * 768 * 4, hipMemcpyDeviceToDevice, s));
  HIP_CHECK(hipMemcpyAsync(dst + 14 * 768, uncond, 14 * 768 * 4, hipMemcpyDeviceToDevice, s));
  HIP_CHECK(hipMemcpyAsync(c->brush32 + (size_t)slot * 3 * c->R * c->R, brush, (size_t)3 * c->R * c->R * 4, hipMemcpyDeviceToDevice, s));
  c->slot_set[slot] = true;
  c->slot_version[slot] = ++c->cond_version;
  return DTP_OK;
}

int dtp_set_conditioning(dtp_ctx* ctx, const float* cond, const float* uncond, const float* brush, dtp_stream s) {
  return dtp_set_conditioning_slot(ctx, 0, cond, uncond, brush, s);
}

int dtp_get_conditioning_slot(dtp_ctx* ctx, int slot, float* cond, float* uncond, dtp_stream s_) {
  Ctx* c = (Ctx*)ctx;
  hipStream_t s = (hipStream_t)s_;
  if (!c || slot < 0 || slot >= DTP_MAX_SLOTS || !c->slot_set[slot]) { dtp_set_error("dtp_get_conditioning: no brush set in slot %d", slot); return DTP_ERR_STATE; }
  const float* src = c->cond32 + (size_t)slot * 2 * 14 * 768;
  HIP_CHECK(hipMemcpyAsync(cond, src, 14 * 768 * 4, hipMemcpyDeviceToDevice, s));
  HIP_CHECK(hipMemcpyAsync(uncond, src + 14 * 768, 14 * 768 * 4, hipMemcpyDeviceToDevice, s));
  return DTP_OK;
}

int dtp_get_conditioning(dtp_ctx* ctx, float* cond, float* uncond, dtp_stream s) { return dtp_get_conditioning_slot(ctx, 0, cond, uncond, s); }

int dtp_last_stamp_finite(dtp_ctx* ctx, int* finite) {
  Ctx* c = (Ctx*)ctx;
  if (!c || !finite) return DTP_ERR_ARG;
  if (!c->finite_pending) { dtp_set_error("dtp_last_stamp_finite: the last stamp ran without the \"check_finite\" option"); return DTP_ERR_STATE; }
  HIP_CHECK(hipEventSynchronize(c->ev[3]));
  int flag = 0;
  HIP_CHECK(hipMemcpy(&flag, c->finite_flag, sizeof(int), hipMemcpyDeviceToHost));
  *finite = flag ? 0 : 1;
  return DTP_OK;
}

int dtp_last_stamp_times(dtp_ctx* ctx, float ms[3]) {
  Ctx* c = (Ctx*)ctx;
  if (!c || !ms) return DTP_ERR_ARG;
  HIP_CHECK(hipEventSynchronize(c->ev[3]));
  for (int i = 0; i < 3; ++i) HIP_CHECK(hipEventElapsedTime(&ms[i], c->ev[i], c->ev[i + 1]));
  return DTP_OK;
}

int dtp_profile(dtp_ctx* ctx, int enable) {
  Ctx* c = (Ctx*)ctx;
  if (!c) return DTP_ERR_ARG;
  HIP_CHECK(hipDeviceSynchronize());
  for (ProfRec& r : c->prof) { (void)hipEventDestroy(r.e0); (void)hipEventDestroy(r.e1); }
  c->prof.clear();
  c->profile = enable != 0;
  return DTP_OK;
}

int dtp_profile_rows(dtp_ctx* ctx, dtp_prof_row* rows, int max_rows, int* n_rows) {
  Ctx* c = (Ctx*)ctx;
  if (!c || !rows || !n_rows) return DTP_ERR_ARG;
  HIP_CHECK(hipDeviceSynchronize());
  dtp_prof_row acc[PK_COUNT] = {};
  for (int k = 0; k < PK_COUNT; ++k) acc[k].kind = k;
  for (const ProfRec& r : c->prof) {
    float ms = 0.f;
// ... 93 lines not shown
```

diffusiontexturepainting_amd/csrc/engine.h:

```cpp
#pragma once
#include <deque>
#include <functional>
#include <map>
#include <string>
#include <tuple>
#include <unordered_map>
#include <vector>

#include "../../include/dtp.h"
#include "common.h"

#define RC(x)            \
  do {                   \
    int rc_ = (x);       \
    if (rc_) return rc_; \
  } while (0)

struct Staged {
  float* d = nullptr;
  std::vector<int64_t> shape;
  size_t n = 0;
};

struct ConvW {
  f16* w = nullptr;
  f16* wcb = nullptr;
  f16* wfr = nullptr;
  float* b = nullptr;
  float* lns = nullptr;
  int cout = 0, cin = 0 , cin_true = 0, taps = 1, K = 0, ldw = 0;
  int cin2 = 0;
  unsigned char* w8 = nullptr;
  int ldw8 = 0;
  float w8_scale = 1.f;
};
struct NormW {
  float *g = nullptr, *b = nullptr;
  int c = 0;
};

struct T {
  f16* p = nullptr;
  int B = 0, H = 0, W = 0, C = 0, ld = 0;
  long long rows() const { return (long long)B * H * W; }
};

struct T8 {
  unsigned char* p = nullptr;
  int B = 0, H = 0, W = 0, C = 0, ld = 0;
  const float* scale_host = nullptr;
  float scale = 1.f;
  int amax_slot1 = 0;
  long long rows() const { return (long long)B * H * W; }
  float now() const { return scale_host ? *scale_host : scale; }
};

struct Ctx;

using Op = std::function<int(hipStream_t, int )>;
struct ProfRec {
  int kind;
  double flops, bytes;
  hipEvent_t e0, e1;
  const char* label;
};
struct LastGemm {
  bool valid = false;
  GemmParams p;
  int tile = 0, bias_step_off = -1;
  size_t op_index = 0;
  int kind = 0;
  double flops = 0, bytes = 0;
  std::string label;
};
struct Prog {
  std::vector<Op> ops;
  LastGemm last_gemm;
  int run(hipStream_t s, int step) const {
    for (const Op& o : ops) RC(o(s, step));
    return DTP_OK;
  }
};

struct ResW {
  NormW n1, n2;
  ConvW c1, c2, sc;
  bool has_sc = false;
  int temb_off = -1;
};
struct XfW {
  NormW gn, ln1, ln2, ln3;
  ConvW proj_in, qkv, out1, q2, kv2, out2, ff1;
  ConvW ff2_proj;
  int kv_index = -1;
  f16* q2T = nullptr;
};
struct VaeAttnW {
  NormW gn;
  ConvW qk, out;
  f16* wv = nullptr;
  float* bv = nullptr;
};

struct LoraRefitJob {
  const float *base, *up, *down;
  const float* gamma;
  const float* beta;
  float* wbeta;
  f16* dst;
  int rank, N, K, row0, ldw;
// ... 114 lines not shown
  int k0 = 0;
  bool vae_eps = false, init_image = false, init_eps = false;
  int sched = 0, steps = 0, row0 = 0;
  std::vector<int> tg_profile;
  bool operator<(const StageKey& o) const {
    return std::tie(stage, B, k0, vae_eps, init_image, init_eps, sched, steps, row0, tg_profile) <
           std::tie(o.stage, o.B, o.k0, o.vae_eps, o.init_image, o.init_eps, o.sched, o.steps, o.row0, o.tg_profile);
  }
};
constexpr int DTP_LOOP_GRAPH_CAP = 16;

constexpr int DTP_STAMP_MAXB = 64;
struct StampCoefs {
  float cfg[DTP_STAMP_MAXB], tg[DTP_STAMP_MAXB];
  int order[DTP_STAMP_MAXB];
  int rank[DTP_STAMP_MAXB];
};
struct StampStrength {
  float a, b;
  int row;
  int pad_;
};
struct StampParams {
  StampCoefs coef;
  StampStrength strength;
  float sched[DTP_SCHED_ROW * 1000];
  float in_scale[1001];
  float init_sigma;
};

struct Ctx {
  int device = 0, R = 0, h = 0, maxB = 1, num_cu = 256;
  bool finalized = false;
  std::unordered_map<std::string, Staged> staged;

  std::vector<void*> chunks;
  char* cur = nullptr;
  size_t cur_left = 0, arena_total = 0;
  Pool pool;
  std::vector<void*> persistent;
  f16* zero = nullptr;
  float* ws = nullptr;
  size_t ws_bytes = 0, ws_need = 0;

  UNetW unet;
  VaeW vae;
  ImgEncW ienc;

  std::map<int, UNetProg> unet_progs;
  std::map<int, VaeEncProg> enc_progs;
  std::map<int, VaeDecProg> dec_progs;

  float* temb_table = nullptr;
  int temb_rows = 0;
  f16* temb_sin = nullptr;
  f16 *temb_h1 = nullptr, *temb_h2 = nullptr;
  int sched_steps = -1;
  int sched_kind = -1;
  int scheduler = DTP_SCHED_DDIM;

  float* cond32 = nullptr;
  float* brush32 = nullptr;
  bool slot_set[DTP_MAX_SLOTS] = {};
  unsigned long long slot_version[DTP_MAX_SLOTS] = {};
  unsigned long long cond_version = 0;
  int* slot_map = nullptr;

  float* x32 = nullptr;
  float* hist32 = nullptr;
  float* canvas32 = nullptr;
  float* alpha_tmp = nullptr;
  StampParams* stamp_params = nullptr;
  std::map<int, StampBufs> stamp_bufs;
  IencBufs ienc_bufs;
  int* finite_flag = nullptr;
  bool check_finite = false;
  bool dedupe_prefix = true;
  bool fuse_gn_conv = false;
  bool fuse_xattn = true;
  bool fold_gn_linear = true;
  bool fuse_reduce_gn = true;
  bool pack_ws = false;
  bool conv_ws = true, conv_ws_vae = true;
  bool gemm_ws = false;
  bool gn_epilogue = true;
  bool reduce_in_concat_gn = true;
  bool gna_lnlin = true;
  bool tune_lnlin = true, tune_halo3 = true;
  bool xchain = true;
  bool xattn_tiles = true;
  int ffchain = -1;
  bool fp8_linear = false;
  bool fp8_attention = false;
  bool fp8_operands = false;
  std::deque<float> fp8_scales;
  std::deque<Fp8Cal> fp8_cals;
  unsigned int* fp8_amax = nullptr;
  int fp8_nslots = 0;
  bool calibrating = false;
  bool finite_pending = false;
  std::map<StageKey, StampGraph> graphs;
  unsigned long long graph_clock = 0;
  hipEvent_t ev[4] = {nullptr, nullptr, nullptr, nullptr};
  int last_evals = 0, last_nodes = 0, last_unet_rows = 0;
  std::map<int, unsigned char*> stroke_masks;
  int last_stroke_stamps = -1, last_stroke_groups = 0, last_stroke_evals = 0;
  int* mesh_face_idx = nullptr;
  unsigned char* mesh_disc = nullptr;
  struct Journal* journal_open = nullptr;
  bool use_graph = true;
  bool exec_imgenc_ready = false;
  bool profile = false;
  std::vector<ProfRec> prof;
  bool autotune = true;
  std::map<std::string, std::pair<int, int>> tuned;
  std::map<std::string, std::pair<float, float>> tune_ms;
  double rep_cold_ms = 0, rep_hot_ms = 0;
  hipEvent_t tune_ev[2] = {nullptr, nullptr};
  void* tune_thrash = nullptr;
  std::string tune_cache_path;
  size_t tune_saved = 0;

  std::unordered_map<std::string, float*> refit_base;
  std::vector<RefitTarget> refit_targets;
  std::vector<RowsumJob> refit_rowsums;
  std::vector<TransposeJob> refit_transposes;
  std::unordered_map<std::string, Staged> refit_staged;
  void* refit_tables = nullptr;
  hipEvent_t refit_ev[2] = {nullptr, nullptr};
  int refit_matrices = -1, refit_launches = 0;
  float refit_ms = 0.f;
};

int ctx_arena_alloc(Ctx* c, size_t bytes, void** out);
int ctx_pool_get(Ctx* c, size_t bytes, void** out);
void ctx_pool_put(Ctx* c, void* p);
int ctx_persistent(Ctx* c, size_t bytes, void** out, bool zero);
void mesh_drop_ctx(Ctx* c);
void journal_drop_ctx(Ctx* c);
struct Journal* journal_armed(Ctx* c, const void* texture, int H, int W);
int journal_save_windows(struct Journal* j, int R, const int* xs, const int* ys, int k, int wrap, hipStream_t s);
int journal_save_box(struct Journal* j, const int* bb, int grow, hipStream_t s);
void delta_drop_ctx(Ctx* c);
const Staged* ctx_find(Ctx* c, const std::string& name);
int ctx_fetch_host(Ctx* c, const std::string& name, std::vector<float>& out);
int ctx_upload_f32(Ctx* c, const std::vector<float>& v, float** out);
int load_norm(Ctx* c, const std::string& name, NormW& n);
int load_conv(Ctx* c, const std::string& name, ConvW& w, int cin_pad = 0, bool bias = true);
int load_conv_with_shortcut(Ctx* c, const std::string& conv, const std::string& shortcut, ConvW& w);
int load_linear_pair(Ctx* c, const std::string& first, const std::string& second, ConvW& w);
int load_linear(Ctx* c, const std::vector<std::string>& names, ConvW& w, bool bias, bool geglu = false,
                const std::string& fold_ln = std::string());
int load_plain_f16(Ctx* c, const std::string& name, f16** out);

int dtp_launch_lora_refit(const LoraRefitJob* jobs, int njobs, int max_n, int max_k, float scale, hipStream_t s);
int dtp_launch_lora_wbeta(const LoraRefitJob* jobs, int njobs, int max_n, float scale, hipStream_t s);
int dtp_launch_rowsum_f16_grouped(const RowsumJob* jobs, int njobs, int max_rows, hipStream_t s);
int dtp_launch_transpose_f16_grouped(const TransposeJob* jobs, int njobs, int max_rows, int max_cols, hipStream_t s);

struct RowStats {
  float* buf = nullptr;
  int parts = 0, M = 0;
  int rows_total = 0, row_off = 0;
};

void prog_push(Ctx* c, Prog* prog, int kind, double flops, double bytes, Op fn, const std::string& label);
// ... 136 lines not shown
```

diffusiontexturepainting_amd/csrc/engine.hip:

```cpp
#include "engine.h"

#include <algorithm>

static size_t up_to(size_t x, size_t m) { return (x + m - 1) / m * m; }

int ctx_arena_alloc(Ctx* c, size_t bytes, void** out) {
  bytes = up_to(bytes, 256);
  if (bytes > c->cur_left) {
    const size_t chunk = std::max(bytes, (size_t)512 << 20);
    void* p = nullptr;
    HIP_CHECK(hipMalloc(&p, chunk));
    HIP_CHECK(hipMemset(p, 0, chunk));
    c->chunks.push_back(p);
    c->cur = (char*)p;
    c->cur_left = chunk;
    c->arena_total += chunk;
  }
  *out = c->cur;
  c->cur += bytes;
  c->cur_left -= bytes;
  return DTP_OK;
}

int ctx_pool_get(Ctx* c, size_t bytes, void** out) {
  bytes = up_to(bytes, 4096);
  int best = -1;
  for (size_t i = 0; i < c->pool.blocks.size(); ++i) {
    const Pool::Block& b = c->pool.blocks[i];
    if (b.free && b.bytes >= bytes && b.bytes <= bytes + bytes / 2 + (1 << 20) &&
        (best < 0 || b.bytes < c->pool.blocks[best].bytes))
      best = (int)i;
  }
  if (best < 0) {
    void* p = nullptr;
    HIP_CHECK(hipMalloc(&p, bytes + (256 << 10)));
    HIP_CHECK(hipMemset(p, 0, bytes + (256 << 10)));
    c->pool.blocks.push_back({(char*)p, bytes, false});
    c->pool.total += bytes;
    *out = p;
    return DTP_OK;
  }
  c->pool.blocks[best].free = false;
  *out = c->pool.blocks[best].p;
  return DTP_OK;
}

void ctx_pool_put(Ctx* c, void* p) {
  for (auto& b : c->pool.blocks)
    if (b.p == (char*)p) { b.free = true; return; }
}

int ctx_persistent(Ctx* c, size_t bytes, void** out, bool zero) {
  void* p = nullptr;
  HIP_CHECK(hipMalloc(&p, bytes + (256 << 10)));
  if (zero) HIP_CHECK(hipMemset(p, 0, bytes + (256 << 10)));
  c->persistent.push_back(p);
  *out = p;
  return DTP_OK;
}

const Staged* ctx_find(Ctx* c, const std::string& name) {
  auto it = c->staged.find(name);
  return it == c->staged.end() ? nullptr : &it->second;
}

int ctx_fetch_host(Ctx* c, const std::string& name, std::vector<float>& out) {
  const Staged* s = ctx_find(c, name);
  if (!s) { dtp_set_error("missing tensor '%s'", name.c_str()); return DTP_ERR_MISSING; }
  out.resize(s->n);
  HIP_CHECK(hipMemcpy(out.data(), s->d, s->n * sizeof(float), hipMemcpyDeviceToHost));
  return DTP_OK;
}

int ctx_upload_f32(Ctx* c, const std::vector<float>& v, float** out) {
  void* p;
  RC(ctx_arena_alloc(c, v.size() * sizeof(float), &p));
  HIP_CHECK(hipMemcpy(p, v.data(), v.size() * sizeof(float), hipMemcpyHostToDevice));
  *out = (float*)p;
  return DTP_OK;
}

int load_norm(Ctx* c, const std::string& name, NormW& n) {
  const Staged *g = ctx_find(c, name + ".weight"), *b = ctx_find(c, name + ".bias");
  if (!g || !b) { dtp_set_error("missing norm '%s'", name.c_str()); return DTP_ERR_MISSING; }
  void *pg, *pb;
  RC(ctx_arena_alloc(c, g->n * 4, &pg));
  RC(ctx_arena_alloc(c, b->n * 4, &pb));
  HIP_CHECK(hipMemcpy(pg, g->d, g->n * 4, hipMemcpyDeviceToDevice));
  HIP_CHECK(hipMemcpy(pb, b->d, b->n * 4, hipMemcpyDeviceToDevice));
  n.g = (float*)pg; n.b = (float*)pb; n.c = (int)g->n;
  return DTP_OK;
}

int load_conv(Ctx* c, const std::string& name, ConvW& w, int cin_pad, bool bias) {
  const Staged* s = ctx_find(c, name + ".weight");
  if (!s) { dtp_set_error("missing weight '%s.weight'", name.c_str()); return DTP_ERR_MISSING; }
  const int cout = (int)s->shape[0], cin = (int)s->shape[1];
  const int taps = s->shape.size() == 4 ? (int)(s->shape[2] * s->shape[3]) : 1;
  if (cin_pad <= 0) cin_pad = (int)up_to(cin, 8);
  w.cout = cout; w.cin = cin_pad; w.cin_true = cin; w.taps = taps; w.K = taps * cin_pad; w.ldw = (int)up_to(w.K, 64);
  void* p;
  RC(ctx_arena_alloc(c, up_to(cout, 128) * (size_t)w.ldw * 2, &p));
  w.w = (f16*)p;
  RC(dtp_launch_pack_conv_weight(s->d, w.w, cout, cin, cin_pad, taps, w.ldw, 0));
  if (taps == 9 && (cin & 63) == 0) {
    void* p2;
    RC(ctx_arena_alloc(c, up_to(cout, 128) * (size_t)w.ldw * 2, &p2));
    w.wcb = (f16*)p2;
    RC(dtp_launch_pack_conv_weight_cb(s->d, w.wcb, cout, cin, w.ldw, 0));
  }
  if (c->pack_ws && taps == 9 && (cin & 63) == 0 && cout >= 32) {
    void* p3;
    RC(ctx_arena_alloc(c, dtp_conv_ws_packed_elems(cout, cin, 0) * 2, &p3));
    w.wfr = (f16*)p3;
    RC(dtp_launch_pack_conv_ws(s->d, nullptr, w.wfr, cout, cin, 0, 0));
  }
  w.b = nullptr;
  if (bias) {
    const Staged* b = ctx_find(c, name + ".bias");
    if (!b) { dtp_set_error("missing bias '%s.bias'", name.c_str()); return DTP_ERR_MISSING; }
    void* pb;
    RC(ctx_arena_alloc(c, b->n * 4, &pb));
    HIP_CHECK(hipMemcpy(pb, b->d, b->n * 4, hipMemcpyDeviceToDevice));
    w.b = (float*)pb;
  }
  return DTP_OK;
}

int load_conv_with_shortcut(Ctx* c, const std::string& conv, const std::string& shortcut, ConvW& w) {
  const Staged *s = ctx_find(c, conv + ".weight"), *t = ctx_find(c, shortcut + ".weight");
  const Staged *sb = ctx_find(c, conv + ".bias"), *tb = ctx_find(c, shortcut + ".bias");
  if (!s || !t || !sb || !tb) { dtp_set_error("missing tensors for '%s' + '%s'", conv.c_str(), shortcut.c_str()); return DTP_ERR_MISSING; }
  const int cout = (int)s->shape[0], cin = (int)s->shape[1], cin2 = (int)t->shape[1];
  if ((int)t->shape[0] != cout || ((9 * cin) & 63) || (cin2 & 63)) { dtp_set_error("shortcut fusion: unsupported shape at '%s'", conv.c_str()); return DTP_ERR_ARG; }
  w.cout = cout; w.cin = cin; w.cin_true = cin; w.taps = 9; w.cin2 = cin2;
  w.K = 9 * cin + cin2; w.ldw = (int)up_to(w.K, 64);
  void* p;
  RC(ctx_arena_alloc(c, up_to(cout, 128) * (size_t)w.ldw * 2, &p));
  w.w = (f16*)p;
  RC(dtp_launch_pack_conv_weight(s->d, w.w, cout, cin, cin, 9, w.ldw, 0));
  RC(dtp_launch_pack_conv_weight(t->d, w.w + 9 * cin, cout, cin2, cin2, 1, w.ldw, 0));
  void* p2;
  RC(ctx_arena_alloc(c, up_to(cout, 128) * (size_t)w.ldw * 2, &p2));
  w.wcb = (f16*)p2;
  RC(dtp_launch_pack_conv_weight_cb(s->d, w.wcb, cout, cin, w.ldw, 0));
  RC(dtp_launch_pack_conv_weight(t->d, w.wcb + 9 * cin, cout, cin2, cin2, 1, w.ldw, 0));
  if (c->pack_ws && (cin & 63) == 0 && cout >= 32) {
    void* p3;
    RC(ctx_arena_alloc(c, dtp_conv_ws_packed_elems(cout, cin, cin2) * 2, &p3));
    w.wfr = (f16*)p3;
    RC(dtp_launch_pack_conv_ws(s->d, t->d, w.wfr, cout, cin, cin2, 0));
  }
  std::vector<float> b1, b2;
  RC(ctx_fetch_host(c, conv + ".bias", b1));
  RC(ctx_fetch_host(c, shortcut + ".bias", b2));
  for (size_t i = 0; i < b1.size(); ++i) b1[i] += b2[i];
  b1.resize(up_to(b1.size(), 128), 0.f);
  return ctx_upload_f32(c, b1, &w.b);
}

static int pack_linear_ws(Ctx* c, ConvW& w) {
  if (!c->pack_ws || !c->gemm_ws || w.taps != 1 || (w.K & 63) || w.K < 128 || w.cout < 32 || (w.cout & 3)) return DTP_OK;
  void* p;
  RC(ctx_arena_alloc(c, dtp_gemm_ws_packed_elems(w.cout, w.K) * 2, &p));
  w.wfr = (f16*)p;
  return dtp_launch_pack_linear_ws(w.w, w.ldw, w.wfr, w.cout, w.K, 0);
}

int load_linear_pair(Ctx* c, const std::string& first, const std::string& second, ConvW& w) {
  const Staged *wa = ctx_find(c, first + ".weight"), *wb = ctx_find(c, second + ".weight");
  const Staged *ba = ctx_find(c, first + ".bias"), *bb = ctx_find(c, second + ".bias");
  if (!wa || !wb || !ba || !bb) { dtp_set_error("linear pair: missing '%s' / '%s'", first.c_str(), second.c_str()); return DTP_ERR_MISSING; }
  const int Na = (int)wa->shape[0], Ka = (int)(wa->n / Na), Nb = (int)wb->shape[0], Kb = (int)(wb->n / Nb);
  if (Kb != Na || (Ka & 63) || (Kb & 63)) { dtp_set_error("linear pair: shapes [%d,%d] then [%d,%d] do not chain", Na, Ka, Nb, Kb); return DTP_ERR_ARG; }
  const int K = Ka + Kb;
  float *prod = nullptr, *cat = nullptr, *bias = nullptr;
  HIP_CHECK(hipMalloc(&prod, (size_t)Nb * Ka * 4));
  HIP_CHECK(hipMalloc(&cat, (size_t)Nb * K * 4));
  HIP_CHECK(hipMalloc(&bias, (size_t)Nb * 4));
  RC(dtp_launch_matmul_f32(wb->d, wa->d, prod, Nb, Ka, Kb, 0));
  HIP_CHECK(hipMemcpy2DAsync(cat, (size_t)K * 4, prod, (size_t)Ka * 4, (size_t)Ka * 4, Nb, hipMemcpyDeviceToDevice, 0));
  HIP_CHECK(hipMemcpy2DAsync(cat + Ka, (size_t)K * 4, wb->d, (size_t)Kb * 4, (size_t)Kb * 4, Nb, hipMemcpyDeviceToDevice, 0));
  RC(dtp_launch_rowdot(wb->d, ba->d, bias, Nb, Kb, 0));
  w = ConvW();
  w.cout = Nb; w.cin = K; w.cin_true = K; w.taps = 1; w.K = K; w.ldw = (int)up_to(K, 64);
  void* p;
  RC(ctx_arena_alloc(c, up_to(Nb, 128) * (size_t)w.ldw * 2, &p));
  w.w = (f16*)p;
  RC(dtp_launch_pack_linear_weight(cat, w.w, Nb, K, w.ldw, nullptr, 0));
  RC(pack_linear_ws(c, w));
  std::vector<float> hb(Nb), hb2;
  HIP_CHECK(hipMemcpy(hb.data(), bias, (size_t)Nb * 4, hipMemcpyDeviceToHost));
  RC(ctx_fetch_host(c, second + ".bias", hb2));
  for (int i = 0; i < Nb; ++i) hb[i] += hb2[i];
  hb.resize(up_to(hb.size(), 128), 0.f);
  RC(ctx_upload_f32(c, hb, &w.b));
  HIP_CHECK(hipDeviceSynchronize());
  HIP_CHECK(hipFree(prod)); HIP_CHECK(hipFree(cat)); HIP_CHECK(hipFree(bias));
  return DTP_OK;
}

int load_linear(Ctx* c, const std::vector<std::string>& names, ConvW& w, bool bias, bool geglu, const std::string& fold_ln) {
  int N = 0, K = -1;
  for (const auto& nm : names) {
    const Staged* s = ctx_find(c, nm + ".weight");
    if (!s) { dtp_set_error("missing weight '%s.weight'", nm.c_str()); return DTP_ERR_MISSING; }
    const int k = (int)(s->n / s->shape[0]);
    if (K >= 0 && k != K) { dtp_set_error("stacked linear '%s': K mismatch", nm.c_str()); return DTP_ERR_ARG; }
    K = k;
    N += (int)s->shape[0];
  }
  w.cout = N; w.cin = K; w.cin_true = K; w.taps = 1; w.K = K; w.ldw = (int)up_to(K, 64);
  void* p;
  RC(ctx_arena_alloc(c, up_to(N, 128) * (size_t)w.ldw * 2, &p));
  w.w = (f16*)p;
  std::vector<int> map;
  int* dmap = nullptr;
  if (geglu) {
    if (names.size() != 1 || N % 256) { dtp_set_error("geglu pack: bad shape"); return DTP_ERR_ARG; }
    map.resize(N);
    for (int f = 0; f < N / 2; ++f) {
      map[f] = (f / 64) * 128 + (f % 64);
      map[N / 2 + f] = (f / 64) * 128 + 64 + (f % 64);
    }
    HIP_CHECK(hipMalloc(&dmap, N * sizeof(int)));
    HIP_CHECK(hipMemcpy(dmap, map.data(), N * sizeof(int), hipMemcpyHostToDevice));
  }
  std::vector<float> wbeta;
  if (!fold_ln.empty()) {
    const Staged *g = ctx_find(c, fold_ln + ".weight"), *be = ctx_find(c, fold_ln + ".bias");
    if (!g || !be || (int)g->n != K) { dtp_set_error("LN fold: missing or mismatched norm '%s'", fold_ln.c_str()); return DTP_ERR_MISSING; }
    float* tmp = nullptr;
    HIP_CHECK(hipMalloc(&tmp, (size_t)N * 4));
    int r0 = 0;
// ... 79 lines not shown
```

diffusiontexturepainting_amd/csrc/gemm_conv.hip:

```cpp
#include <stdlib.h>
#include <type_traits>

#include "common.h"
#include "tile_epilogue.h"

namespace {

__device__ __forceinline__ void glds16(const void* src, void* lds_uniform) {
  __builtin_amdgcn_global_load_lds((const __attribute__((address_space(1))) void*)src,
                                   (__attribute__((address_space(3))) void*)lds_uniform, 16, 0, 0);
}

typedef __attribute__((address_space(3))) void* lds_ptr_t;
template <int N>
__device__ __forceinline__ void wait_vmcnt() { asm volatile("s_waitcnt vmcnt(%0)" ::"n"(N) : "memory"); }

template <int BM, int BN, int NS, int KH = 1, int LW = 0, bool CONV = false>
__global__ __launch_bounds__(256 * KH + 64 * LW) void gemm_kernel(const GemmParams pin) {
  GemmParams p = pin;
  const int st_rows = p.st_rows > 0 ? p.st_rows : p.M;
  const int st_m0 = (p.batch > 1) ? (int)blockIdx.y * p.M : 0;
  if (p.batch > 1) {
    const long long bz = blockIdx.y;
    p.A += bz * p.a_bs; p.W += bz * p.w_bs;
// ... 649 lines not shown
  static_assert(lds <= 160 * 1024, "LDS budget");
  const dim3 grid = xs ? dim3(tiles * p.splits, 1, 1) : dim3(tiles, p.batch > 1 ? p.batch : 1, p.splits);
  hipLaunchKernelGGL((gemm_kernel<BM, BN, NS, KH, LW, CONV>), grid, dim3(256 * KH + 64 * LW), lds, s, p);
  return hipGetLastError() == hipSuccess ? DTP_OK : DTP_ERR_HIP;
}

template <int BM, int BN, int NS, int KH = 1, int LW = 0>
int launch_tile(const GemmParams& p, hipStream_t s) {
  return (p.flags & GF_CONV3) ? launch_tile_mode<BM, BN, NS, KH, LW, true>(p, s) : launch_tile_mode<BM, BN, NS, KH, LW, false>(p, s);
}

}

#define FOR_ALL_VARIANTS(X) \
  X(128, 128, 2) X(128, 128, 3) X(128, 128, 4) X(128, 64, 2) X(128, 64, 3) X(128, 64, 4) \
  X(64, 64, 2) X(64, 64, 3) X(64, 64, 4) X(64, 128, 2) X(64, 128, 3) X(64, 128, 4) \
  X(256, 128, 2) X(256, 128, 3) X(128, 256, 2) X(128, 256, 3)
#define FOR_ALL_KH2(X) \
  X(128, 128, 2) X(128, 128, 3) X(128, 64, 2) X(128, 64, 3) X(64, 64, 2) X(64, 64, 3) X(64, 128, 2) X(64, 128, 3)

#define FOR_ALL_LW(X) \
  X(128, 128, 3, 4) X(128, 64, 3, 4) X(64, 64, 3, 4) X(64, 128, 3, 4) \
  X(128, 128, 3, 8) X(128, 64, 3, 8) X(64, 64, 3, 8) X(64, 128, 3, 8)

void dtp_gemm_init() {
#define SET_ATTR(BM, BN, NS) \
  (void)hipFuncSetAttribute((const void*)gemm_kernel<BM, BN, NS, 1, 0, false>, hipFuncAttributeMaxDynamicSharedMemorySize, gemm_lds_bytes(BM, BN, NS)); \
  (void)hipFuncSetAttribute((const void*)gemm_kernel<BM, BN, NS, 1, 0, true>, hipFuncAttributeMaxDynamicSharedMemorySize, gemm_lds_bytes(BM, BN, NS));
  FOR_ALL_VARIANTS(SET_ATTR)
#undef SET_ATTR
#define SET_ATTR2(BM, BN, NS) \
  (void)hipFuncSetAttribute((const void*)gemm_kernel<BM, BN, NS, 2, 0, false>, hipFuncAttributeMaxDynamicSharedMemorySize, gemm_lds_bytes(BM, BN, NS)); \
  (void)hipFuncSetAttribute((const void*)gemm_kernel<BM, BN, NS, 2, 0, true>, hipFuncAttributeMaxDynamicSharedMemorySize, gemm_lds_bytes(BM, BN, NS));
  FOR_ALL_KH2(SET_ATTR2)
#undef SET_ATTR2
#define SET_ATTR3(BM, BN, NS, LW) \
  (void)hipFuncSetAttribute((const void*)gemm_kernel<BM, BN, NS, 1, LW, false>, hipFuncAttributeMaxDynamicSharedMemorySize, gemm_lds_bytes(BM, BN, NS)); \
  (void)hipFuncSetAttribute((const void*)gemm_kernel<BM, BN, NS, 1, LW, true>, hipFuncAttributeMaxDynamicSharedMemorySize, gemm_lds_bytes(BM, BN, NS));
  FOR_ALL_LW(SET_ATTR3)
#undef SET_ATTR3
}

size_t dtp_gemm_workspace_bytes(const GemmParams& p) {
  return p.splits > 1 ? (size_t)p.splits * p.M * p.N * sizeof(float) : 0;
}

void dtp_gemm_pick(GemmParams& p, int* tile, int num_cu) {
  const bool geglu = (p.flags & GF_GEGLU) != 0;
  int t;
  const bool n128 = (p.N % 128) == 0;
  if (p.M >= 512) t = (n128 || p.N < 64 ? 0 : 1);
  else t = (n128 ? 3 : 2);
  if (p.N <= 64 && p.M >= 512) t = 1;
  if (geglu) t = (p.M >= 512) ? 0 : 3;
  static const int bm[4] = {128, 128, 64, 64}, bn[4] = {128, 64, 64, 128};
  const long long blocks = (long long)((p.M + bm[t] - 1) / bm[t]) * ((p.N + bn[t] - 1) / bn[t]) * (p.batch > 1 ? p.batch : 1);
  int splits = 1;
  if (!geglu && !(p.flags & GF_LNFOLD) && p.batch <= 1 && blocks * 2 <= num_cu && p.nkb >= 8) {
    splits = (int)((2LL * num_cu + blocks - 1) / blocks);
    if (splits > p.nkb / 4) splits = p.nkb / 4;
    if (splits > 32) splits = 32;
    if (splits < 1) splits = 1;
  }
  p.kb_per_split = (p.nkb + splits - 1) / splits;
  p.splits = (p.nkb + p.kb_per_split - 1) / p.kb_per_split;
  const double a_bytes = (double)p.M * (double)(p.flags & GF_CONV3 ? p.Cin : p.K);
  const double w_bytes = (double)p.N * (double)p.K;
  if (w_bytes > a_bytes) p.flags |= GF_MFAST; else p.flags &= ~GF_MFAST;
  *tile = t;
}

static int gemm_family_args(const GemmParams& p) {
  if (p.nkb <= 0 || p.M <= 0 || p.N <= 0) { dtp_set_error("gemm: empty problem"); return DTP_ERR_ARG; }
  if (p.flags & GF_GNAPPLY) { dtp_set_error("gemm: GroupNorm-on-the-staged-patch is a conv_halo_kernel feature (tile ids 12..15)"); return DTP_ERR_ARG; }
  return DTP_OK;
}

int dtp_launch_tile(const GemmParams& p, int tile, hipStream_t s) {
  const DtpTile t = dtp_tile(tile);
  switch (t.fam) {
    case TF_HALO: return dtp_launch_conv_halo(p, t.var, s);
    case TF_LNLIN: return dtp_launch_lnlin(p, p.col_ranges, s);
    case TF_CONVWS: return dtp_launch_conv_ws(p, t.var, s);
    case TF_GEMMWS: return dtp_launch_gemm_ws(p, s);
    case TF_WIDE:
    case TF_FP8: {
      const int rc = gemm_family_args(p);
      if (rc != DTP_OK) return rc;
      return t.fam == TF_WIDE ? dtp_launch_gemm_wide(p, t.var, s) : dtp_launch_gemm_fp8(p, t.var, s);
    }
    default: return dtp_launch_gemm(p, tile, s);
  }
}

int dtp_launch_gemm(const GemmParams& p, int tile, hipStream_t s) {
  const int arc = gemm_family_args(p);
  if (arc != DTP_OK) return arc;
  if ((p.lda & 7) || (p.ldw & 7)) { dtp_set_error("gemm: lda/ldw must be multiples of 8"); return DTP_ERR_ARG; }
  {
    const size_t a_rows = (p.flags & GF_CONV3) ? (size_t)(p.M / (p.Ho * p.Wo) + 1) * p.Hi * p.Wi : (size_t)p.M;
    const size_t lim = (size_t)1 << 31;
    if (a_rows * p.lda * 2 >= lim || (p.A2 && (size_t)p.M * p.lda2 * 2 >= lim) || ((size_t)p.N + 256) * p.ldw * 2 >= lim) {
      dtp_set_error("gemm: an operand of 2 GiB or more (M %d lda %d, N %d ldw %d)", p.M, p.lda, p.N, p.ldw);
      return DTP_ERR_ARG;
    }
  }
  if ((p.flags & GF_CONV3) && (p.Cin & 7)) { dtp_set_error("conv: Cin must be a multiple of 8"); return DTP_ERR_ARG; }
  if (p.A2 && (p.flags & GF_CONV3) && (((9 * p.Cin) & 63) || (p.Cin2 & 63) || (p.lda2 & 7) || p.stride != 1)) {
    dtp_set_error("conv: fused shortcut tail needs stride 1 and 9*Cin, Cin2 multiples of 64");
    return DTP_ERR_ARG;
  }
  if (p.A2 && !(p.flags & GF_CONV3) && ((p.Cin2 & 63) || ((p.K - p.Cin2) & 63) || p.Cin2 <= 0 || p.Cin2 >= p.K || (p.lda2 & 7) ||
                                       (p.flags & GF_LNFOLD))) {
    dtp_set_error("gemm: a second activation matrix needs K - Cin2 and Cin2 to be multiples of 64 and no LayerNorm fold");
    return DTP_ERR_ARG;
  }
  if (p.batch > 1 && (p.splits > 1 || (p.flags & GF_CONV3))) { dtp_set_error("gemm: batched problems are dense and unsplit"); return DTP_ERR_ARG; }
  if ((p.flags & GF_SOFTMAX16) && ((p.N & 15) || p.splits > 1 || p.sm_valid < 1 || p.sm_valid > 16 || (p.ldc & 7) ||
                                   (p.flags & (GF_GEGLU | GF_OUT_F32 | GF_RESID | GF_ROWSTATS)))) {
    dtp_set_error("gemm: the group-softmax epilogue needs N %% 16 == 0, fp16 output, no split-K / residual / row statistics");
    return DTP_ERR_ARG;
  }
  if ((p.flags & GF_ROWSTATS) && (!p.st_out || (p.flags & (GF_GEGLU | GF_OUT_F32)))) {
    dtp_set_error("gemm: row statistics need st_out and an fp16, non-GEGLU output");
    return DTP_ERR_ARG;
  }
  if ((p.flags & GF_LNFOLD) && (p.splits > 1 || (p.flags & GF_CONV3) || !p.lns)) {
    dtp_set_error("gemm: LayerNorm fold needs a dense, unsplit GEMM with lns");
    return DTP_ERR_ARG;
  }
  const DtpTile t = dtp_tile(tile);
  if (t.fam != TF_GEMM) { dtp_set_error("gemm: bad tile id %d", tile); return DTP_ERR_ARG; }
  if ((p.flags & GF_GEGLU) && (p.splits > 1 || t.bn != 128 || (p.N % 128))) {
    dtp_set_error("gemm: GEGLU needs a 128-wide N tile, N %% 128 == 0 and no split-K");
    return DTP_ERR_ARG;
  }
  int rc = -1;
#define DISPATCH(BM, BN, NS) \
  if (rc < 0 && t.kh == 1 && !t.lw && t.bm == BM && t.bn == BN && t.ns == NS) rc = launch_tile<BM, BN, NS>(p, s);
  FOR_ALL_VARIANTS(DISPATCH)
#undef DISPATCH
#define DISPATCH2(BM, BN, NS) \
  if (rc < 0 && t.kh == 2 && t.bm == BM && t.bn == BN && t.ns == NS) rc = launch_tile<BM, BN, NS, 2>(p, s);
  FOR_ALL_KH2(DISPATCH2)
#undef DISPATCH2
#define DISPATCH3(BM, BN, NS, LW) \
  if (rc < 0 && t.lw == LW && t.bm == BM && t.bn == BN && t.ns == NS) rc = launch_tile<BM, BN, NS, 1, LW>(p, s);
  FOR_ALL_LW(DISPATCH3)
#undef DISPATCH3
  if (rc != DTP_OK) { dtp_set_error("gemm launch failed: %s", hipGetErrorString(hipGetLastError())); return rc; }
  if (p.splits > 1 && !(p.flags & GF_NOREDUCE)) return dtp_launch_splitk_reduce(p, s);
  return DTP_OK;
}

int dtp_launch_splitk_reduce(const GemmParams& p, hipStream_t s) {
  if (p.flags & GF_ROWSTATS) {
    if (p.flags & (GF_BIAS_M | GF_GELU | GF_QUICKGELU | GF_SILU | GF_OUT_F32 | GF_LNFOLD)) {
      dtp_set_error("gemm: split-K row statistics support bias/residual epilogues only");
      return DTP_ERR_ARG;
    }
    hipLaunchKernelGGL(splitk_reduce_rows_kernel, dim3((p.M + 3) / 4), dim3(256), 0, s, p);
    return hipGetLastError() == hipSuccess ? DTP_OK : DTP_ERR_HIP;
  }
  long long total = (long long)p.M * p.N;
  const bool vec = (p.N & 3) == 0 && !(p.flags & GF_OUT_F32) && (p.ldc & 3) == 0 && (!(p.flags & GF_RESID) || (p.ldr & 3) == 0) &&
                   (((uintptr_t)p.C | (uintptr_t)p.R) & 7) == 0 && (!(p.flags & GF_BIAS) || ((uintptr_t)p.bias & 15) == 0);
// ... 8 lines not shown
```

diffusiontexturepainting_amd/csrc/tune.hip:

```cpp
#include "engine.h"

#include <stdio.h>
#include <stdlib.h>
#include <string.h>
#include <unistd.h>

#include <algorithm>

static void tune_read_file(Ctx* c, const char* path) {
  FILE* f = fopen(path, "r");
  if (!f) return;
  char key[256];
  int tile, splits;
  while (fscanf(f, "%255s %d %d", key, &tile, &splits) == 3)
    if (tile >= 0 && tile < DTP_TILE_IDS && splits >= 1 && splits <= 64) c->tuned[key] = std::make_pair(tile, splits);
  fclose(f);
}

void tune_cache_load(Ctx* c) {
  const char* seed = getenv("DTP_TUNE_SEED");
  if (seed && *seed) tune_read_file(c, seed);
  const char* e = getenv("DTP_TUNE_CACHE");
  if (!e || !*e) return;
  c->tune_cache_path = e;
  tune_read_file(c, e);
  c->tune_saved = c->tuned.size();
}

static bool tune_entry_valid(const GemmParams& p, int tile, int sp) {
  const DtpTile t = dtp_tile(tile);
  GemmParams q = p;
  if (sp < 1 || (sp > p.nkb && t.fam != TF_LNLIN) || !dtp_tile_apply(q, tile, sp)) return false;
  switch (t.fam) {
    case TF_NONE: return false;
    case TF_GEMMWS: return dtp_gemm_ws_supported(p, sp);
    case TF_LNLIN: return dtp_lnlin_supported(p, sp);
    case TF_CONVWS: return dtp_conv_ws_supported(p, t.var, sp);
    case TF_HALO: return p.Wcb && (t.var >= 4 ? dtp_conv_halo3_supported(p) : dtp_conv_halo_supported(p)) && p.batch <= 1;
    default: break;
  }
  if (p.flags & GF_GNAPPLY) return false;
  if (t.fam == TF_FP8) return dtp_gemm_fp8_supported(q) && !((p.flags & GF_GEGLU) && (t.bn % 128));
  if (t.fam == TF_WIDE) return dtp_gemm_wide_supported(q, t.var);
  if ((p.flags & GF_GEGLU) && (t.bn != 128 || sp != 1)) return false;
  if (sp > 1 && ((p.flags & (GF_LNFOLD | GF_SOFTMAX16)) || p.batch > 1)) return false;
  if (sp > 1 && (size_t)sp * p.M * p.N * sizeof(float) > ((size_t)512 << 20)) return false;
  return true;
}

void tune_cache_save(Ctx* c) {
  if (c->rep_cold_ms > 0) fprintf(stderr, "[tune] sum over pushed GEMMs: cold %.2f ms, hot %.2f ms\n", c->rep_cold_ms, c->rep_hot_ms);
  if (c->tune_thrash) { (void)hipDeviceSynchronize(); (void)hipFree(c->tune_thrash); c->tune_thrash = nullptr; }
  if (c->tune_cache_path.empty() || c->tuned.size() == c->tune_saved) return;
  const std::string tmp = c->tune_cache_path + ".tmp." + std::to_string((long long)getpid());
  FILE* f = fopen(tmp.c_str(), "w");
  if (!f) return;
  for (auto& kv : c->tuned) fprintf(f, "%s %d %d\n", kv.first.c_str(), kv.second.first, kv.second.second);
  fclose(f);
  (void)rename(tmp.c_str(), c->tune_cache_path.c_str());
  c->tune_saved = c->tuned.size();
}

struct TuneCfg { int tile, sp; };
static std::vector<TuneCfg> tune_candidates(const Ctx* c, const GemmParams& p, const bool* ws_ok, bool gw_ok) {
  static const int cand_splits[] = {1, 2, 3, 4, 6, 8, 12, 16, 24, 32};
  const bool geglu = (p.flags & GF_GEGLU) != 0;
  std::vector<TuneCfg> out;
  auto add = [&](int tile, int sp) {
    GemmParams q = p;
    if (dtp_tile_apply(q, tile, sp) && dtp_gemm_workspace_bytes(q) <= ((size_t)512 << 20)) out.push_back({tile, sp});
  };
  for (int tile = 0; tile < DTP_TILE_IDS && !(p.flags & GF_GNAPPLY); ++tile) {
    const DtpTile t = dtp_tile(tile);
    if (t.fam != TF_GEMM && t.fam != TF_WIDE && t.fam != TF_FP8) continue;
    if (t.fam == TF_FP8 ? !p.W8 : (p.W8 && p.M >= 6144)) continue;
    const long long ntiles = (long long)((p.M + t.bm - 1) / t.bm) * ((p.N + t.bn - 1) / t.bn);
    if (t.fam == TF_FP8) {
      if (!(geglu && (t.bn % 128)) && !(t.var == 4 && ntiles < 96)) add(tile, 1);
      continue;
    }
    if (t.fam == TF_WIDE) {
      GemmParams q = p;
      q.splits = 1;
      if (!dtp_gemm_wide_supported(q, t.var) || ntiles < 96) continue;
      if (t.var == 1 && (p.N % 320) > 0 && (p.N % 320) <= 192) continue;
      add(tile, 1);
      continue;
    }
    if (geglu && t.bn != 128) continue;
    if (p.nkb < 3 && t.ns > 2) continue;
    if ((t.bm == 256 && p.M < 192) || (t.bn == 256 && p.N < 192)) continue;
    for (int sp : cand_splits) {
      if (sp > 1 && (geglu || (p.flags & GF_LNFOLD) || p.batch > 1 || p.nkb / sp < 2)) break;
      add(tile, sp);
    }
  }
  {
    static const int ranges[] = {1, 2, 3, 4, 5, 6, 8, 10, 12, 16, 20, 24, 32, 40};
    for (int sp : ranges)
      if (c->tune_lnlin && dtp_lnlin_supported(p, sp)) add(DTP_TILE_LNLIN, sp);
  }
  for (int tile = 0; tile < DTP_TILE_IDS && p.Wcb && dtp_conv_halo_supported(p); ++tile) {
    const DtpTile t = dtp_tile(tile);
    if (t.fam != TF_HALO) continue;
    const bool small = p.Hi * p.Wi <= 256;
    if (t.var < 4 ? (t.var >= 2) != small : (!c->tune_halo3 || !small || !dtp_conv_halo3_supported(p))) continue;
    for (int sp : cand_splits) {
      if (sp > 1 && p.nkb / sp < 9) break;
      add(tile, sp);
    }
  }
  for (int tile = 0; tile < DTP_TILE_IDS; ++tile) {
    const DtpTile t = dtp_tile(tile);
    static const int slices[] = {1, 2, 3, 4, 5, 6, 8, 10};
    if (t.fam != TF_CONVWS) continue;
    for (int sp : slices) {
      if (!c->conv_ws || !ws_ok[t.var] || !dtp_conv_ws_supported(p, t.var, sp)) continue;
      if (t.var >= 2 && sp > 4) continue;
      add(tile, sp);
    }
  }
  if (gw_ok) {
    static const int slices[] = {1, 2, 3, 4, 5, 6, 8};
    for (int sp : slices)
      if (dtp_gemm_ws_supported(p, sp) && !(sp > 1 && p.nkb / sp < 4)) add(DTP_TILE_GEMMWS, sp);
  }
  return out;
}

int tune_gemm(Ctx* c, const GemmParams& p, int* tile, int* sp) {
  char key[200];
  int kl = snprintf(key, sizeof(key), "k8|%d,%d,%d,%d,%d,%d,%d,%d,%d,%d,%d,%d,%d,%d", p.M, p.N, p.K, p.flags & ~GF_MFAST, p.Hi, p.Wi, p.Cin,
                    p.stride, p.lda, p.ldc, p.ldw, p.st_parts, p.Cin2, p.lda2);
  if (p.batch > 1) kl += snprintf(key + kl, sizeof(key) - kl, ",b%d", p.batch);
  if (p.W8) kl += snprintf(key + kl, sizeof(key) - kl, ",f8");
  bool ws_ok[DTP_WS_VARIANTS];
  bool ws_any = false;
  for (int v = 0; v < DTP_WS_VARIANTS; ++v) { ws_ok[v] = p.Wfr && (p.flags & GF_CONV3) && dtp_conv_ws_supported(p, v, 1); ws_any = ws_any || ws_ok[v]; }
  if (ws_any) kl += snprintf(key + kl, sizeof(key) - kl, ",ws2");
  if (!(p.flags & GF_LNFOLD)) {
    bool ll = false;
    for (int r = 1; r <= 40 && !ll; ++r) ll = dtp_lnlin_supported(p, r);
    if (ll) snprintf(key + kl, sizeof(key) - kl, ",ll");
  }
  const bool gw_ok = dtp_gemm_ws_supported(p, 1);
  if (gw_ok) { kl = (int)strlen(key); snprintf(key + kl, sizeof(key) - kl, ",gw"); }
  auto it = c->tuned.find(key);
  if (it != c->tuned.end() && !tune_entry_valid(p, it->second.first, it->second.second)) {
    fprintf(stderr, "[dtp] tune table entry '%s' -> (%d, %d) does not fit the problem; re-tuning\n", key, it->second.first, it->second.second);
    c->tuned.erase(it);
    it = c->tuned.end();
  }
  if (it == c->tuned.end()) {
    if (!c->tune_ev[0]) { HIP_CHECK(hipEventCreate(&c->tune_ev[0])); HIP_CHECK(hipEventCreate(&c->tune_ev[1])); }
    constexpr size_t THRASH_BYTES = (size_t)512 << 20;
    if (!c->tune_thrash) HIP_CHECK(hipMalloc(&c->tune_thrash, THRASH_BYTES));
    const size_t a_bytes = (p.flags & GF_CONV3) ? (size_t)(p.M / (p.Ho * p.Wo)) * p.Hi * p.Wi * p.lda * 2 : (size_t)p.M * p.lda * 2;
    auto time_cfg = [&](int cfg_tile, int cfg_sp, int reps, bool cold, float* out_ms) -> int {
      GemmParams q = p;
      (void)dtp_tile_apply(q, cfg_tile, cfg_sp);
      const size_t need = dtp_gemm_workspace_bytes(q);
      if (need > c->ws_bytes) { c->ws_need = std::max(c->ws_need, need); RC(ensure_ws(c)); }
      q.part = c->ws;
      q.zero = c->zero;
      float ms = 1e30f;
      for (int rep = 0; rep < reps; ++rep) {
        if (cold) {
          HIP_CHECK(hipMemsetAsync(c->tune_thrash, rep, THRASH_BYTES, 0));
          RC(dtp_launch_touch(q.A, a_bytes, (float*)c->tune_thrash, 0));
          if (q.R) RC(dtp_launch_touch(q.R, (size_t)q.M * q.ldr * 2, (float*)c->tune_thrash, 0));
        }
        HIP_CHECK(hipEventRecord(c->tune_ev[0], 0));
        RC(dtp_launch_tile(q, cfg_tile, 0));
        HIP_CHECK(hipEventRecord(c->tune_ev[1], 0));
        HIP_CHECK(hipEventSynchronize(c->tune_ev[1]));
        float ev = 0.f;
        HIP_CHECK(hipEventElapsedTime(&ev, c->tune_ev[0], c->tune_ev[1]));
        if (cold || rep) ms = std::min(ms, ev);
      }
      *out_ms = ms;
      return DTP_OK;
    };
    struct Cand { float ms; int tile, sp; };
    std::vector<Cand> cands;
    for (const TuneCfg& cfg : tune_candidates(c, p, ws_ok, gw_ok)) {
      float ms;
      RC(time_cfg(cfg.tile, cfg.sp, 5, true, &ms));
      cands.push_back({ms, cfg.tile, cfg.sp});
    }
    std::sort(cands.begin(), cands.end(), [](const Cand& x, const Cand& y) { return x.ms < y.ms; });
    for (size_t i = 0; i < cands.size() && i < 3; ++i) {
      float ms;
      RC(time_cfg(cands[i].tile, cands[i].sp, 8, true, &ms));
      cands[i].ms = std::min(cands[i].ms, ms);
    }
    float best = 1e30f;
    int bt = *tile, bs = *sp;
    for (size_t i = 0; i < cands.size() && i < 3; ++i)
      if (cands[i].ms < best) { best = cands[i].ms; bt = cands[i].tile; bs = cands[i].sp; }
    if (ws_any && dtp_tile(bt).fam != TF_CONVWS && dtp_conv_output_can_carry_gn_stats(p)) {
      const float stats_ms = 0.005f + (float)((double)p.M * p.N * 2.0 / 4.0e12 * 1e3);
      for (const Cand& cd : cands) {
        const DtpTile t = dtp_tile(cd.tile);
        if (cd.sp == 1 && t.fam == TF_CONVWS && t.var >= 2 && cd.ms - stats_ms < best) { best = cd.ms - stats_ms; bt = cd.tile; bs = 1; }
      }
    }
    it = c->tuned.emplace(key, std::make_pair(bt, bs)).first;
    if (getenv("DTP_TUNE_REPORT")) {
      float hot;
      RC(time_cfg(bt, bs, 4, false, &hot));
      c->tune_ms[key] = std::make_pair(best, hot);
    }
  }
  {
    auto m = c->tune_ms.find(key);
    if (m != c->tune_ms.end()) {
      c->rep_cold_ms += m->second.first;
      c->rep_hot_ms += m->second.second;
      fprintf(stderr, "[tune] %s tile=%d sp=%d cold %.1f us hot %.1f us\n", key, it->second.first, it->second.second, m->second.first * 1e3,
              m->second.second * 1e3);
    }
  }
  *tile = it->second.first;
  *sp = it->second.second;
  return DTP_OK;
}
```

diffusiontexturepainting_amd/ops.py:

```python
import ctypes as C

import torch

from . import _lib
from ._lib import (GF_BIAS, GF_BIAS_M, GF_GEGLU, GF_GELU, GF_LNFOLD, GF_OUT_F32, GF_QUICKGELU, GF_RESID, GemmDesc, check,
                   ptr)


def _stream():
    return C.c_void_p(torch.cuda.current_stream().cuda_stream)


def _up(x, m):
    return (x + m - 1) // m * m


def pack_linear(w, geglu=False):
    lib = _lib.load()
    n, k = w.shape
    out = torch.zeros(_up(n, 128), _up(k, 64), dtype=torch.float16, device=w.device)
    w = w.contiguous().float()
    check(lib.dtp_op_pack_linear(ptr(w), ptr(out), n, k, out.shape[1], int(geglu), _stream()), "pack_linear")
    return out


def pack_conv(w, cin_pad=None):
    lib = _lib.load()
    cout, cin, kh, kw = w.shape
    cin_pad = cin_pad or _up(cin, 8)
    out = torch.zeros(_up(cout, 128), _up(kh * kw * cin_pad, 64), dtype=torch.float16, device=w.device)
    w = w.contiguous().float()
    check(lib.dtp_op_pack_conv(ptr(w), ptr(out), cout, cin, cin_pad, kh * kw, out.shape[1], _stream()), "pack_conv")
    return out


def pack_conv_cb(w):
    lib = _lib.load()
    cout, cin = w.shape[:2]
    out = torch.zeros(_up(cout, 128), 9 * cin, dtype=torch.float16, device=w.device)
    w = w.contiguous().float()
    check(lib.dtp_op_pack_conv_cb(ptr(w), ptr(out), cout, cin, out.shape[1], _stream()), "pack_conv_cb")
    return out


def pack_conv_ws(w, w1=None):
    lib = _lib.load()
    cout, cin = w.shape[:2]
    cin2 = w1.shape[1] if w1 is not None else 0
    out = torch.zeros(lib.dtp_op_pack_conv_ws_elems(cout, cin, cin2), dtype=torch.float16, device=w.device)
    w = w.contiguous().float()
    w1 = w1.reshape(cout, cin2).contiguous().float() if w1 is not None else None
    check(lib.dtp_op_pack_conv_ws(ptr(w), ptr(w1), ptr(out), cout, cin, cin2, _stream()), "pack_conv_ws")
    return out


def pack_linear_ws(wp, n, k):
    lib = _lib.load()
    out = torch.zeros(lib.dtp_op_pack_linear_ws_elems(n, k), dtype=torch.float16, device=wp.device)
    check(lib.dtp_op_pack_linear_ws(ptr(wp), wp.stride(0), ptr(out), n, k, _stream()), "pack_linear_ws")
    return out


def lora_refit(w0, up, down, scale=1.0, gamma=None, out=None, row0=0):
    lib = _lib.load()
    n, k = w0.shape
    if out is None:
        out = torch.zeros(_up(row0 + n, 128), _up(k, 64), dtype=torch.float16, device=w0.device)
    if out.dim() != 2 or out.dtype != torch.float16 or out.stride(1) != 1 or out.shape[0] < row0 + n:
        raise ValueError(f"lora_refit: out must be f16 [>= {row0 + n}, ldw] with unit column stride, got {tuple(out.shape)}")
    w0 = w0.contiguous().float()
    rank = 0 if up is None else up.shape[1]
    up = up.contiguous().float() if up is not None else None
    down = down.contiguous().float() if down is not None else None
    gamma = gamma.contiguous().float() if gamma is not None else None
    check(lib.dtp_op_lora_refit(ptr(w0), ptr(up), ptr(down), rank, float(scale), ptr(gamma), ptr(out), int(row0), n, k, out.stride(0),
                                _stream()), "lora_refit")
    return out


def rowsum(wp, k):
    lib = _lib.load()
    out = torch.empty(wp.shape[0], dtype=torch.float32, device=wp.device)
    check(lib.dtp_op_rowsum(ptr(wp), wp.stride(0), k, ptr(out), wp.shape[0], _stream()), "rowsum")
    return out


def quantize_w8(wp, k):
    lib = _lib.load()
    out = torch.zeros(wp.shape[0], _up(k, 128), dtype=torch.uint8, device=wp.device)
    sc = C.c_float()
    check(lib.dtp_op_quantize_w8(ptr(wp), wp.stride(0), k, wp.shape[0], ptr(out), out.shape[1], C.byref(sc), _stream()), "quantize_w8")
    return out, sc.value


def quant_e4m3(x, scale, ln=False, stats_in=None, eps=1e-5, k=None, x2=None, scale2=1.0, ln2=False, k2=None):
    lib = _lib.load()
    m = x.shape[0]
    k = k or x.shape[1]
    y = torch.empty(m, k, dtype=torch.uint8, device=x.device)
    y2 = None
    if x2 is not None:
        k2 = k2 or x2.shape[1]
        y2 = torch.empty(m, k2, dtype=torch.uint8, device=x.device)
    st = stats_in.contiguous() if stats_in is not None else None
    check(lib.dtp_op_quant_e4m3(ptr(x), x.stride(0), ptr(y), y.stride(0), k, float(scale), int(ln),
                                ptr(x2), x2.stride(0) if x2 is not None else 0, ptr(y2), y2.stride(0) if y2 is not None else 0,
                                k2 or 0, float(scale2), int(ln2), m, ptr(st), st.shape[0] if st is not None else 0, eps, _stream()),
          "quant_e4m3")
    return (y, y2) if x2 is not None else y


def gemm_f8f8(a8, w8, n, a_scale, w_scale, k=None, bias=None, resid=None, flags=0, tile=-1, tail8=None, row_stats=False,
              out8_scale=None, out16=True, tail_scale=None):
    lib = _lib.load()
    m = a8.shape[0]
    k = k or a8.shape[1]
    n_out = n // 2 if flags & GF_GEGLU else n
    d = GemmDesc()
    out = torch.empty(m, n_out, dtype=torch.float16, device=a8.device) if out16 else None
    out8 = torch.empty(m, n_out, dtype=torch.uint8, device=a8.device) if out8_scale is not None else None
    d.A8, d.lda8 = a8.data_ptr(), a8.stride(0)
    d.W8, d.ldw8, d.a_scale, d.w_scale = w8.data_ptr(), w8.stride(0), a_scale, w_scale
    d.C, d.ldc = (out.data_ptr(), out.stride(0)) if out is not None else (None, 0)
    if out8 is not None:
        d.C8, d.ldc8, d.c_scale = out8.data_ptr(), out8.stride(0), out8_scale
    d.bias = bias.data_ptr() if bias is not None else None
    d.R = resid.data_ptr() if resid is not None else None
    d.ldr = resid.stride(0) if resid is not None else 0
    d.M, d.N, d.K = m, n, k
    d.flags = flags | (GF_BIAS if bias is not None else 0) | (GF_RESID if resid is not None else 0)
    d.tile = tile
    if tail8 is not None:
        d.A2_8, d.lda2_8, d.Cin2 = tail8.data_ptr(), tail8.stride(0), tail8.shape[1]
        d.a2_scale = tail_scale or 0.0
        d.K = k + tail8.shape[1]
# ... 509 lines not shown
```

include/dtp.h:

```cpp
#ifndef DTP_H
#define DTP_H
#include <stddef.h>
#include <stdint.h>

#ifdef __cplusplus
extern "C" {
#endif

#define DTP_ABI_VERSION 3

enum { DTP_OK = 0, DTP_ERR_ARG = 1, DTP_ERR_HIP = 2, DTP_ERR_STATE = 3, DTP_ERR_MISSING = 4 };

typedef struct dtp_ctx dtp_ctx;
typedef void* dtp_stream;

int dtp_abi_version(void);
const char* dtp_last_error(void);

int dtp_create(int device, int resolution, int max_batch, dtp_ctx** out);
void dtp_destroy(dtp_ctx* ctx);

int dtp_load_tensor(dtp_ctx* ctx, const char* name, const float* data, int is_device, const int64_t* shape, int ndim);
int dtp_finalize_weights(dtp_ctx* ctx);

// ... 132 lines not shown
int dtp_delta_device(dtp_delta* d, int** ids, uint8_t** tiles, int** counts);
int dtp_delta_host(dtp_delta* d, int** ids, uint8_t** tiles);
int dtp_delta_pull(dtp_ctx* ctx, dtp_delta* d, const uint8_t* image, int H, int W, dtp_stream s, int* host_ids, uint8_t* host_tiles,
                   int max_tiles, int* count, int* remaining);
int dtp_op_delta_state(dtp_delta* d, uint8_t* shadow_host, uint8_t* stale_host, dtp_stream s);

int dtp_ddim_tables(int steps, int64_t* timesteps, float* alphas, float* final_alpha);

#define DTP_SCHED_DDIM 0
#define DTP_SCHED_DPM 1
#define DTP_SCHED_LMSD 2
#define DTP_SCHED_ROW 8
int dtp_scheduler_tables(int scheduler, int steps, int* evals, float* init_sigma, float* timesteps, float* in_scale, float* coefs);

int dtp_strength_schedule(int scheduler, int steps, double strength, int* t_start, int* evals, float* noise_coefs);

int dtp_last_stamp_times(dtp_ctx* ctx, float ms[3]);
int dtp_last_stamp_info(dtp_ctx* ctx, int* unet_evals, int* graph_nodes);
int dtp_last_stamp_unet_rows(dtp_ctx* ctx, int* rows);

typedef struct { int kind; int launches; double ms; double flops; double bytes; } dtp_prof_row;
int dtp_profile(dtp_ctx* ctx, int enable);
int dtp_profile_rows(dtp_ctx* ctx, dtp_prof_row* rows, int max_rows, int* n_rows);
int dtp_profile_dump(dtp_ctx* ctx, const char* path);
int dtp_set_option(dtp_ctx* ctx, const char* name, int value);
int dtp_last_stamp_finite(dtp_ctx* ctx, int* finite);

typedef struct {
  const void* A;
  const void* W;
  void* C;
  const float* bias;
  const void* R;
  int M, N, K;
  int lda, ldw, ldc, ldr;
  int conv, Hi, Wi, Ho, Wo, Cin, stride, pad, upsample2x;
  int flags;
  int tile;
  int splits;
  const float* lns;
  float ln_eps;
  const void* A2;
  int lda2, Cin2;
  const void* Wcb;
  int batch;
  int64_t a_bs, w_bs, c_bs, r_bs;
  int bias_bs, lns_bs;
  int sm_valid;
  float* st_out;
  const float* st_in;
  int st_parts;
  int st_parts_out;
  const void* W8;
  int ldw8;
  float a_scale, w_scale;
  int gn_cpg;
  const void* Wfr;
  const void* A8;
  int lda8;
  const void* A2_8;
  int lda2_8;
  void* C8;
  int ldc8;
  float c_scale;
  float a2_scale;
} dtp_gemm_desc;
enum { DTP_GF_BIAS = 1, DTP_GF_BIAS_M = 2, DTP_GF_RESID = 4, DTP_GF_GEGLU = 8, DTP_GF_GELU = 64, DTP_GF_QUICKGELU = 128,
       DTP_GF_OUT_F32 = 256, DTP_GF_SILU = 512, DTP_GF_LNFOLD = 1024, DTP_GF_ROWSTATS = 2048, DTP_GF_SOFTMAX16 = 4096,
       DTP_GF_GNSTATS = 1 << 24, DTP_GF_RAGGED = 1 << 25 };

int dtp_op_gemm(dtp_gemm_desc* d, dtp_stream s);
int dtp_op_gemm_f8f8(dtp_gemm_desc* d, dtp_stream s);
int dtp_op_quant_e4m3(const void* x, int ldx, void* y, int ldy, int K, float scale, int ln, const void* x2, int ldx2, void* y2, int ldy2,
                      int K2, float scale2, int ln2, int M, const float* st_in, int st_parts, float eps, dtp_stream s);
int dtp_op_pack_linear(const float* w, void* out, int N, int K, int ldw, int geglu, dtp_stream s);
int dtp_op_lora_refit(const float* w0, const float* up, const float* down, int rank, float scale, const float* gamma, void* out, int row0,
                      int N, int K, int ldw, dtp_stream s);
int dtp_op_rowsum(const void* w, int ld, int K, float* out, int rows, dtp_stream s);
int dtp_op_quantize_w8(const void* w, int ldw, int K, int rows, void* out, int ldw8, float* w_scale, dtp_stream s);
int dtp_op_pack_conv(const float* w, void* out, int Cout, int Cin, int Cin_pad, int taps, int ldw, dtp_stream s);
int dtp_op_pack_conv_cb(const float* w, void* out, int Cout, int Cin, int ldw, dtp_stream s);
int dtp_op_pack_conv_ws(const float* w, const float* w1, void* out, int Cout, int Cin, int Cin2, dtp_stream s);
long long dtp_op_pack_conv_ws_elems(int Cout, int Cin, int Cin2);
int dtp_op_pack_linear_ws(const void* w, int ldw, void* out, int N, int K, dtp_stream s);
long long dtp_op_pack_linear_ws_elems(int N, int K);
int dtp_op_groupnorm(const void* x, int ldx, void* y, int ldy, const float* gamma, const float* beta, int B, int HW, int C,
                     int groups, float eps, int silu, dtp_stream s);
int dtp_op_groupnorm_apply(const void* x, int ldx, void* y, int ldy, const float* gamma, const float* beta, const float* partial, int nchunk,
                           int B, int HW, int C, int groups, float eps, int silu, dtp_stream s);
int dtp_op_groupnorm_stats_apply(const float* part, int splits, const float* bias, const void* resid, void* x, void* y, const float* gamma,
                                 const float* beta, int B, int HW, int C, int groups, float eps, int silu, dtp_stream s);
int dtp_op_measure_peaks(double* mfma_f16_tflops, double* hbm_copy_gbs);
int dtp_op_reduce_groupnorm(const float* part, int splits, const float* bias, const void* resid, void* conv_out, void* y, const float* gamma,
                            const float* beta, int B, int HW, int C, int groups, float eps, int silu, dtp_stream s);
int dtp_op_reduce_groupnorm_cx(const float* part, int splits, const float* bias, const void* resid, void* conv_out, void* y, const float* gamma,
                               const float* beta, int B, int HW, int C, int groups, float eps, int silu, int cx, dtp_stream s);
int dtp_op_xattn(const void* X, const void* W1, const float* b1, const float* lns1, const float* st_in, int st_parts, const void* W2, const float* b2,
                 const void* R, void* Y, float* st_out, int S, int C, int N, int sm_valid, float ln_eps, dtp_stream s);
int dtp_op_xattn_ct(const void* X, const void* W1, const float* b1, const float* lns1, const float* st_in, int st_parts, const void* W2, const float* b2,
                    const void* R, void* Y, float* st_out, int S, int C, int N, int sm_valid, float ln_eps, int ct, dtp_stream s);
int dtp_op_xchain(const void* A, const void* Wo, int ldwo, const float* bo, const void* Y, const void* W1, const float* b1, const float* lns1,
                  const void* W2, const float* b2, void* Y3, float* st_out, int S, int C, int N, int sm_valid, float ln_eps, dtp_stream s);
int dtp_op_ffchain(const void* X, const void* W1, int ldw1, const float* lns1, const float* b1, const void* Wm, int ldwm, const float* bm,
                   const void* R, void* Out, int M, int C, float ln_eps, dtp_stream s);
int dtp_op_gn_fold_weights(const void* x, const void* W, int ldw, const float* bias, const float* gamma, const float* beta, int B, int HW, int C,
                           int Nout, int groups, float eps, void* Wout, float* bias_out, dtp_stream s);
int dtp_op_gn_linear(const void* x, const void* W, int ldw, const float* bias, const float* gamma, const float* beta, int B, int HW, int C,
                     int Nout, int groups, float eps, void* y, float* st_out, int col_ranges, dtp_stream s);
int dtp_op_layernorm(const void* x, int ldx, void* y, int ldy, const float* gamma, const float* beta, int rows, int C,
                     float eps, dtp_stream s);
int dtp_op_attention(const void* Q, const void* K, const void* V, void* O, int ldq, int ldk, int ldv, int ldo, int B, int H,
                     int Sq, int Skv, int D, int64_t qbs, int64_t kbs, int64_t vbs, int64_t obs, float scale, dtp_stream s);
int dtp_op_attention_dma(const void* Q, const void* K, const void* V, void* O, int ldq, int ldk, int ldv, int ldo, int B, int H,
                         int Sq, int Skv, int D, int64_t qbs, int64_t kbs, int64_t vbs, int64_t obs, float scale, int nw, dtp_stream s);
int dtp_op_attention_fp8(const void* Q, const void* K, const void* V, void* O, int ldq, int ldk, int ldv, int ldo, int B, int H,
                         int Sq, int Skv, int D, int64_t qbs, int64_t kbs, int64_t vbs, int64_t obs, float scale, float q_scale,
                         float v_scale, dtp_stream s);
int dtp_op_softmax_rows(const void* x, int ldx, void* y, int ldy, int rows, int cols, float scale, dtp_stream s);
int dtp_op_strength_init(const float* z0, const float* eps, float a, float b, float* x, long long n, dtp_stream s);
int dtp_op_dilate(const float* canvas, float* tmp, float* out, int B, int R, int pad, dtp_stream s);
int dtp_op_dilate_pads(const float* canvas, float* tmp, float* out, int B, int R, const int* pads, dtp_stream s);
int dtp_op_sched_step(int scheduler, const float* eps_out, float* x, float* hist, void* in16, const float* row, const float* next_scale,
                      const float* cfg, const float* tg, const int* rank, int step_index, int B, int hw, int k, dtp_stream s);

int dtp_op_stroke_gather(const uint8_t* texture, int H, int W, float* canvas, int R, int B, const int* xs, const int* ys, const int* modes,
                         int wrap, int over_y, int over_x, dtp_stream s);
int dtp_op_stroke_paste(const float* dec, const uint8_t* mask, uint8_t* texture, int H, int W, int R, int B, const int* xs, const int* ys,
                        const int* modes, int wrap, dtp_stream s);

int dtp_op_mesh_render(dtp_mesh* mesh, const float cam[12], float fov, int flip_normals, const uint8_t* texture, int H, int W, int R, int mode,
                       int over_y, int over_x, float* canvas, int* face_idx, dtp_stream s);
int dtp_op_mesh_backproject(dtp_mesh* mesh, const float* dec, int dec_finished, const uint8_t* mask, const int* face_idx, int R, uint8_t* texture, int H, int W,
                            dtp_stream s);
int dtp_op_mesh_backproject_masked(dtp_mesh* mesh, const float* dec, int dec_finished, const uint8_t* mask, const int* face_idx, int R,
                                   uint8_t* texture, int H, int W, const uint32_t* face_mask, int mask_words, dtp_stream s);
int dtp_op_mesh_pick(dtp_mesh* mesh, const dtp_ray* rays, int n, dtp_mesh_hit* out, dtp_stream s);
int dtp_op_mesh_view(dtp_mesh* mesh, const uint8_t* texture, int TH, int TW, const dtp_view_cam* cam, int H, int W, const dtp_view_opts* opts,
                     uint8_t* image, int* face_idx, float* depth, int binned, dtp_stream s);
int dtp_op_mesh_view_clip(dtp_mesh* mesh, const uint8_t* texture, int TH, int TW, const uint8_t* mips, const dtp_view_cam* cam, int H, int W,
                          const dtp_view_opts* opts, int filter, uint8_t* image, int* face_idx, float* depth, float* lod, int binned, dtp_stream s);
int dtp_op_mesh_view_aa(dtp_mesh* mesh, const uint8_t* texture, int TH, int TW, const uint8_t* mips, const dtp_view_cam* cam, int H, int W,
                        const dtp_view_opts* opts, int filter, int clip, int samples, uint8_t* image, int* face_idx, float* depth, float* lod,
                        uint8_t* coverage, int binned, dtp_stream s);
int dtp_op_mesh_view_aniso(dtp_mesh* mesh, const uint8_t* texture, int TH, int TW, const uint8_t* mips, const dtp_view_cam* cam, int H, int W,
                           const dtp_view_opts* opts, int clip, int samples, int max_aniso, uint8_t* image, int* face_idx, float* depth,
                           float* lod, uint8_t* taps, uint8_t* coverage, int binned, dtp_stream s);
#ifdef __cplusplus
}
#endif
#endif
```

Baseline: 10.36.

## Add 8x16-tile weight-stationary conv3x3 kernel and route autotuner to it

```diff
diff --git a/diffusiontexturepainting_amd/_lib.py b/diffusiontexturepainting_amd/_lib.py
--- a/diffusiontexturepainting_amd/_lib.py
+++ b/diffusiontexturepainting_amd/_lib.py
@@ -191,6 +191,9 @@
     "dtp_op_groupnorm_stats_apply": (_i, [_vp, _i, _vp, _vp, _vp, _vp, _vp, _vp, _i, _i, _i, _i, _f, _i, _vp]),
     "dtp_op_pack_conv_ws": (_i, [_vp, _vp, _vp, _i, _i, _i, _vp]),
     "dtp_op_pack_conv_ws_elems": (C.c_longlong, [_i, _i, _i]),
+    "dtp_op_pack_conv_ws16": (_i, [_vp, _vp, _vp, _i, _i, _i, _vp]),
+    "dtp_op_pack_conv_ws16_elems": (C.c_longlong, [_i, _i, _i]),
+    "dtp_op_pack_conv_ws16_map": (None, [_i, _i, C.c_longlong, C.c_longlong, _vp]),
     "dtp_op_pack_linear_ws": (_i, [_vp, _i, _vp, _i, _i, _vp]),
     "dtp_op_pack_linear_ws_elems": (C.c_longlong, [_i, _i]),
     "dtp_op_groupnorm": (_i, [_vp, _i, _vp, _i, _vp, _vp, _i, _i, _i, _i, _f, _i, _vp]),
diff --git a/diffusiontexturepainting_amd/csrc/api_ops.hip b/diffusiontexturepainting_amd/csrc/api_ops.hip
--- a/diffusiontexturepainting_amd/csrc/api_ops.hip
+++ b/diffusiontexturepainting_amd/csrc/api_ops.hip
@@ -64,7 +64,7 @@
   int rc = ops_init();
   if (rc) return rc;
   static bool halo_init = false;
-  if (!halo_init) { dtp_conv_halo_init(); dtp_gemm_wide_init(); dtp_lnlin_init(); dtp_conv_ws_init(); dtp_gemm_ws_init(); halo_init = true; }
+  if (!halo_init) { dtp_conv_halo_init(); dtp_gemm_wide_init(); dtp_lnlin_init(); dtp_conv_ws_init(); dtp_conv_ws16_init(); dtp_gemm_ws_init(); halo_init = true; }
   GemmParams p = {};
   p.A = (const f16*)d->A; p.W = (const f16*)d->W; p.C = d->C; p.bias = d->bias; p.R = (const f16*)d->R;
   p.zero = g_ops.zero;
@@ -81,6 +81,7 @@
   if (p.batch > 1) p.st_rows = p.batch * p.M;
   p.W8 = (const unsigned char*)d->W8; p.ldw8 = d->ldw8; p.a_scale = d->a_scale; p.w_scale = d->w_scale;
   p.Wfr = (const f16*)d->Wfr;
+  if (d->tile == DTP_TILE_WS16) { p.Wfr16 = p.Wfr; p.Wfr = nullptr; }
   p.gn_cpg = d->gn_cpg;
   static bool fp8_init = false;
   if (!fp8_init) { dtp_gemm_fp8_init(); fp8_init = true; }
@@ -184,6 +185,11 @@
 }
 long long dtp_op_pack_linear_ws_elems(int N, int K) { return (long long)dtp_gemm_ws_packed_elems(N, K); }
 long long dtp_op_pack_conv_ws_elems(int Cout, int Cin, int Cin2) { return (long long)dtp_conv_ws_packed_elems(Cout, Cin, Cin2); }
+int dtp_op_pack_conv_ws16(const float* w, const float* w1, void* out, int Cout, int Cin, int Cin2, dtp_stream s) {
+  return dtp_launch_pack_conv_ws16(w, w1, (f16*)out, Cout, Cin, Cin2, (hipStream_t)s);
+}
+long long dtp_op_pack_conv_ws16_elems(int Cout, int Cin, int Cin2) { return (long long)dtp_conv_ws16_packed_elems(Cout, Cin, Cin2); }
+void dtp_op_pack_conv_ws16_map(int Cin, int tail, long long first, long long count, int* out) { dtp_conv_ws16_pack_map(Cin, tail, first, count, out); }
 
 int dtp_op_groupnorm(const void* x, int ldx, void* y, int ldy, const float* gamma, const float* beta, int B, int HW, int C,
                      int groups, float eps, int silu, dtp_stream s) {
diff --git a/diffusiontexturepainting_amd/csrc/builder.hip b/diffusiontexturepainting_amd/csrc/builder.hip
--- a/diffusiontexturepainting_amd/csrc/builder.hip
+++ b/diffusiontexturepainting_amd/csrc/builder.hip
@@ -129,7 +129,7 @@
 bool Builder::claim_stats(const T& x, float** partials, int* nchunk) {
   const LastGemm lg = prog->last_gemm;
   const DtpTile t = dtp_tile(lg.tile);
-  if (!c->gn_epilogue || !lg.valid || t.fam != TF_CONVWS || t.var < 2 || lg.p.splits != 1 || (f16*)lg.p.C != x.p || lg.p.ldc != x.ld ||
+  if (!c->gn_epilogue || !lg.valid || !dtp_tile_emits_gn_stats(lg.tile) || lg.p.splits != 1 || (f16*)lg.p.C != x.p || lg.p.ldc != x.ld ||
       lg.p.M != (int)x.rows() || lg.p.N != x.C || !dtp_conv_output_can_carry_gn_stats(lg.p))
     return false;
   GemmParams gp = lg.p;
@@ -140,7 +140,7 @@
   gp.flags |= GF_GNSTATS;
   gp.st_out = (float*)pp;
   gp.gn_cpg = x.C / 32;
-  if (!dtp_conv_ws_supported(gp, t.var, 1)) { ctx_pool_put(c, pp); return false; }
+  if (!(t.fam == TF_CONVWS16 ? dtp_conv_ws16_supported(gp, 1) : dtp_conv_ws_supported(gp, t.var, 1))) { ctx_pool_put(c, pp); return false; }
   prog->ops.pop_back();
   prog_push(c, prog, lg.kind, lg.flops, lg.bytes, make_gemm_op(c, gp, lg.tile, lg.bias_step_off), lg.label + " (+gn stats)");
   *partials = (float*)pp;
@@ -346,7 +346,7 @@
            p.batch > 1 ? (" x" + std::to_string(p.batch)).c_str() : "");
   const double flops = 2.0 * nb * p.M * (double)p.N * k_alg;
   prog_push(c, prog, t.pk, flops, bytes, make_gemm_op(c, p, tile, bias_step_off), lab);
-  if (p.splits > 1 || (t.fam == TF_CONVWS && t.var >= 2)) {
+  if (p.splits > 1 || dtp_tile_emits_gn_stats(tile)) {
     LastGemm& lg = prog->last_gemm;
     lg.valid = true; lg.p = p; lg.tile = tile; lg.bias_step_off = bias_step_off; lg.op_index = prog->ops.size() - 1;
     lg.kind = t.pk; lg.flops = flops; lg.bytes = bytes; lg.label = lab;
@@ -368,7 +368,7 @@
   if (c->R % 64) p.flags |= GF_RAGGED;
   if (o.tail) { p.A2 = o.tail->p; p.lda2 = o.tail->ld; p.Cin2 = w.cin2; }
   p.Wcb = w.wcb;
-  p.Wfr = w.wfr;
+  p.Wfr = w.wfr; p.Wfr16 = w.wfr16;
   if (o.extra_flags & GF_GNAPPLY) {
     if (!o.gn.part) { dtp_set_error("conv3: GF_GNAPPLY without GroupNorm parameters"); return DTP_ERR_ARG; }
     p.gn_part = o.gn.part; p.gn_gamma = o.gn.gamma; p.gn_beta = o.gn.beta; p.gn_eps = o.gn.eps;
diff --git a/diffusiontexturepainting_amd/csrc/common.h b/diffusiontexturepainting_amd/csrc/common.h
--- a/diffusiontexturepainting_amd/csrc/common.h
+++ b/diffusiontexturepainting_amd/csrc/common.h
@@ -256,6 +256,7 @@
   int ldc8;
   float c_scale;
   float a2_scale;
+  const f16* Wfr16;
 };
 
 struct Quant8Job {
@@ -417,11 +418,12 @@
 constexpr int DTP_TILE_WS0 = 51;
 constexpr int DTP_WS_VARIANTS = 4;
 constexpr int DTP_TILE_GEMMWS = 55;
-constexpr int DTP_TILE_IDS = 56;
+constexpr int DTP_TILE_WS16 = 56;
+constexpr int DTP_TILE_IDS = 57;
 
 enum { PK_GEMM0 = 0, PK_ATTN = 12, PK_GN = 13, PK_LN = 14, PK_ELEM = 15, PK_SOFTMAX = 16, PK_HALO0 = 17, PK_BIG0 = 21, PK_WIDE0 = 25, PK_FP8 = 27, PK_KH2 = 28, PK_LW = 36, PK_XATTN = 44, PK_HALO3 = 45, PK_LNLIN = 47, PK_WS0 = 48, PK_GEMMWS = 52, PK_F8F8 = 53, PK_QUANT8 = 54, PK_COUNT = 55 };
 
-enum DtpFamily : unsigned char { TF_NONE, TF_GEMM, TF_HALO, TF_WIDE, TF_FP8, TF_LNLIN, TF_CONVWS, TF_GEMMWS };
+enum DtpFamily : unsigned char { TF_NONE, TF_GEMM, TF_HALO, TF_WIDE, TF_FP8, TF_LNLIN, TF_CONVWS, TF_GEMMWS, TF_CONVWS16 };
 enum DtpSplit : unsigned char {
   SPLIT_K,
   SPLIT_HALO,
@@ -452,7 +454,12 @@
   if (id == DTP_TILE_LNLIN) return {TF_LNLIN, 0, 0, 0, 0, 0, 0, SPLIT_COLS, PK_LNLIN};
   if (id >= DTP_TILE_WS0 && id < DTP_TILE_WS0 + DTP_WS_VARIANTS) return {TF_CONVWS, id - DTP_TILE_WS0, 0, 0, 0, 0, 0, SPLIT_BLOCKS, PK_WS0 + id - DTP_TILE_WS0};
   if (id == DTP_TILE_GEMMWS) return {TF_GEMMWS, 0, 64, 64, 0, 0, 0, SPLIT_BLOCKS, PK_GEMMWS};
+  if (id == DTP_TILE_WS16) return {TF_CONVWS16, 0, 0, 0, 0, 0, 0, SPLIT_NONE, PK_WS0 + 3};
   return {};
+}
+inline bool dtp_tile_emits_gn_stats(int id) {
+  const DtpTile t = dtp_tile(id);
+  return (t.fam == TF_CONVWS && t.var >= 2) || t.fam == TF_CONVWS16;
 }
 inline bool dtp_tile_apply(GemmParams& p, int tile, int sp) {
   const DtpTile t = dtp_tile(tile);
@@ -484,6 +491,12 @@
 size_t dtp_conv_ws_packed_elems(int Cout, int Cin, int Cin2);
 int dtp_conv_ws_gn_chunks(int Ho, int Wo);
 int dtp_launch_pack_conv_ws(const float* w, const float* w1, f16* out, int Cout, int Cin, int Cin2, hipStream_t s);
+bool dtp_conv_ws16_supported(const GemmParams& p, int nsplit);
+int dtp_launch_conv_ws16(const GemmParams& p, hipStream_t s);
+void dtp_conv_ws16_init();
+size_t dtp_conv_ws16_packed_elems(int Cout, int Cin, int Cin2);
+int dtp_launch_pack_conv_ws16(const float* w, const float* w1, f16* out, int Cout, int Cin, int Cin2, hipStream_t s);
+void dtp_conv_ws16_pack_map(int Cin, int tail, long long first, long long count, int* out);
 bool dtp_gemm_ws_supported(const GemmParams& p, int nsplit);
 int dtp_launch_gemm_ws(const GemmParams& p, hipStream_t s);
 void dtp_gemm_ws_init();
diff --git a/diffusiontexturepainting_amd/csrc/context.hip b/diffusiontexturepainting_amd/csrc/context.hip
--- a/diffusiontexturepainting_amd/csrc/context.hip
+++ b/diffusiontexturepainting_amd/csrc/context.hip
@@ -47,6 +47,7 @@
 #endif
   c->fuse_xattn = !on("DTP_NO_XATTN"); c->fold_gn_linear = !on("DTP_NO_FOLD_GN");
   c->conv_ws = !on("DTP_NO_WS"); c->conv_ws_vae = !on("DTP_NO_WS_VAE"); c->gemm_ws = on("DTP_GEMMWS");
+  if (const char* e = getenv("DTP_WS16")) c->conv_ws16 = !strcmp(e, "both") ? 2 : !strcmp(e, "0") ? 0 : 1;
   c->gn_epilogue = !on("DTP_NO_GN_EPILOGUE"); c->reduce_in_concat_gn = !on("DTP_NO_REDUCE_IN_CONCAT_GN"); c->gna_lnlin = !on("DTP_NO_GNA_LNLIN");
   c->tune_lnlin = !on("DTP_NO_LNLIN"); c->tune_halo3 = !on("DTP_NO_HALO3");
   c->xchain = !on("DTP_NO_XCHAIN"); c->xattn_tiles = !on("DTP_XATTN_CT1");
@@ -108,6 +109,7 @@
   dtp_xchain_init();
   dtp_ffchain_init();
   dtp_conv_ws_init();
+  dtp_conv_ws16_init();
   dtp_gemm_ws_init();
   RC(load_unet_weights(c));
   RC(load_vae_weights(c));
diff --git a/diffusiontexturepainting_amd/csrc/conv_ws16.hip b/diffusiontexturepainting_amd/csrc/conv_ws16.hip
--- /dev/null
+++ b/diffusiontexturepainting_amd/csrc/conv_ws16.hip
@@ -0,0 +1,428 @@
+#include <stdlib.h>
+#include <type_traits>
+
+#include "common.h"
+
+struct Ws16Src { int n, ch, tap; };
+static __host__ __device__ inline Ws16Src ws16_src(long long i, int Cin, bool tail) {
+  const int e = (int)(i & 7), l = (int)((i >> 3) & 63);
+  long long f = i >> 9;
+  const int it = (int)(f & 3), hf = (int)((f >> 2) & 1); f >>= 3;
+  int tap = 0;
+  if (!tail) { tap = (int)(f % 9); f /= 9; }
+  const int ncb = Cin >> 6;
+  const int cb = (int)(f % ncb), nr = (int)(f / ncb);
+  return {nr * 64 + 16 * it + (l & 15), cb * 64 + 32 * hf + 8 * (l >> 4) + e, tap};
+}
+void dtp_conv_ws16_pack_map(int Cin, int tail, long long first, long long count, int* out) {
+  for (long long k = 0; k < count; ++k) {
+    const Ws16Src src = ws16_src(first + k, Cin, tail != 0);
+    out[3 * k] = src.n; out[3 * k + 1] = src.ch; out[3 * k + 2] = src.tap;
+  }
+}
+
+namespace {
+
+typedef __attribute__((address_space(3))) void* lds_ptr_t;
+typedef unsigned int u32x4 __attribute__((ext_vector_type(4)));
+
+template <int OFF>
+__device__ __forceinline__ f16x8 lds_read16_off(uint32_t addr) {
+  f16x8 v;
+  asm volatile("ds_read_b128 %0, %1 offset:%2" : "=v"(v) : "v"(addr), "n"(OFF));
+  return v;
+}
+template <int N>
+__device__ __forceinline__ void wait_vmcnt() { asm volatile("s_waitcnt vmcnt(%0)" ::"n"(N) : "memory"); }
+
+struct G16 {
+  static constexpr int TH = 8, TW = 16;
+  static constexpr int PW = TW + 3, PH = TH + 2;
+  static constexpr int HP1 = PH * PW;
+  static constexpr int HL = (HP1 + 31) / 32;
+  static constexpr int PBYTES = HL * 32 * 128;
+  static constexpr int CBLK = 1024;
+  static constexpr int CMB = 4 * 2 * TH * CBLK;
+  static constexpr int MAINB = 3 * PBYTES > CMB ? 3 * PBYTES : CMB;
+  static constexpr int STATB = (4 * 64 * 2 + 64 * 2) * 8;
+  static constexpr int LDS = MAINB + STATB;
+  static_assert(LDS <= 80 * 1024, "two workgroups per CU");
+  static_assert((TH + 1) * PW * 128 < 65536, "fragment offsets are 16-bit immediates");
+};
+
+__global__ void pack_conv_ws16_kernel(const float* __restrict__ w, f16* __restrict__ out, int Cout, int Cin, long long total) {
+  for (long long i = (long long)blockIdx.x * 256 + threadIdx.x; i < total; i += (long long)gridDim.x * 256) {
+    const Ws16Src src = ws16_src(i, Cin, false);
+    out[i] = src.n < Cout ? (f16)w[((size_t)src.n * Cin + src.ch) * 9 + src.tap] : (f16)0.f;
+  }
+}
+__global__ void pack_conv_ws16_tail_kernel(const float* __restrict__ w, f16* __restrict__ out, int Cout, int Cin2, long long total) {
+  for (long long i = (long long)blockIdx.x * 256 + threadIdx.x; i < total; i += (long long)gridDim.x * 256) {
+    const Ws16Src src = ws16_src(i, Cin2, true);
+    out[i] = src.n < Cout ? (f16)w[(size_t)src.n * Cin2 + src.ch] : (f16)0.f;
+  }
+}
+
+template <int N>
+__device__ __forceinline__ void wait_lds_frag(f16x8& f) { asm volatile("s_waitcnt lgkmcnt(%1)" : "+v"(f) : "n"(N)); }
+
+template <bool NTW>
+__global__ __launch_bounds__(256, 2) void convws16_kernel(const GemmParams p) {
+  using G = G16;
+  constexpr int TH = G::TH, TW = G::TW, HL = G::HL, PW = G::PW, PH = G::PH, HP1 = G::HP1, PB = G::PBYTES;
+  extern __shared__ __attribute__((aligned(16))) char smem[];
+
+  const int tid = threadIdx.x, lane = tid & 63;
+  const int wave = __builtin_amdgcn_readfirstlane(tid >> 6);
+  const int fpx = lane & 15, fq = lane >> 4;
+  const int half = wave & 1, pair = wave >> 1;
+
+  const int H = p.Ho, W = p.Wo;
+  const int tiles_x = W / TW, tiles_y = H / TH;
+  const int hw = H * W;
+  const bool pow2 = ((hw & (hw - 1)) | (tiles_x & (tiles_x - 1)) | (tiles_y & (tiles_y - 1))) == 0;
+  const int images = pow2 ? (p.M >> __builtin_ctz(hw)) : p.M / hw;
+  const int npg = images * tiles_y * tiles_x;
+  const int units = (p.N + 63) >> 6;
+  const int xcd = blockIdx.x & 7, idx = blockIdx.x >> 3;
+  int pg, nr;
+  if ((units & 7) == 0) { const int q = idx / npg; pg = idx - q * npg; nr = q * 8 + xcd; }
+  else { const int pgq = (npg + 7) >> 3; const int q = idx / pgq; pg = (idx - q * pgq) * 8 + xcd; nr = q; }
+  if (nr >= units || pg >= npg) return;
+  const int ncb = p.Cin >> 6;
+  int tx, ty, img0;
+  if (pow2) {
+    const int sx = __builtin_ctz(tiles_x), sy = __builtin_ctz(tiles_y);
+    tx = pg & (tiles_x - 1); ty = (pg >> sx) & (tiles_y - 1); img0 = pg >> (sx + sy);
+  } else {
+    tx = pg % tiles_x; ty = (pg / tiles_x) % tiles_y; img0 = pg / (tiles_x * tiles_y);
+  }
+  const int y0 = ty * TH, x0 = tx * TW;
+
+  const auto rsW = __builtin_amdgcn_make_buffer_rsrc((void*)p.Wfr16, 0, (int)0x80000000u, 0x00020000);
+  constexpr int OOB = (int)0x80000000u;
+  const int lane16 = lane * 16;
+  const int ntile16 = (p.N - nr * 64 + 15) >> 4;
+  const int wbase = nr * ncb;
+  auto wload = [&](int set, int cb, int tap) -> f16x8 {
+    const int i = set ^ (2 * pair);
+    const u32x4 v = __builtin_amdgcn_raw_buffer_load_b128(rsW, i < ntile16 ? lane16 : OOB, ((((wbase + cb) * 9 + tap) * 2 + half) * 4 + i) * 1024, NTW ? 2 : 0);
+    return __builtin_bit_cast(f16x8, v);
+  };
+  f16x8 wf[4][4], wh[2];
+#pragma unroll
+  for (int k = 0; k < 2; ++k) wh[k] = wload(k, 0, 8);
+#pragma unroll
+  for (int s = 0; s < 4; ++s)
+#pragma unroll
+    for (int i = 0; i < 4; ++i) wf[s][i] = wload(i, 0, 2 * s + pair);
+  __builtin_amdgcn_sched_barrier(0);
+
+  const auto rsA = __builtin_amdgcn_make_buffer_rsrc((void*)p.A, 0, (int)0x80000000u, 0x00020000);
+  int voffA[HL];
+  {
+    const int ups = (p.flags & GF_UPS2) ? 1 : 0;
+    const int s0 = wave * 8 + (lane >> 3);
+    int hy = s0 / PW, hx = s0 - hy * PW;
+    constexpr int DY = 32 / PW, DX = 32 - DY * PW;
+#pragma unroll
+    for (int i = 0; i < HL; ++i) {
+      const int iy = y0 + hy - 1, ix = x0 + hx - 1;
+      const bool ok = hy < PH && hx < TW + 2 && (unsigned)iy < (unsigned)H && (unsigned)ix < (unsigned)W;
+      voffA[i] = ok ? (((img0 * p.Hi + (iy >> ups)) * p.Wi + (ix >> ups)) * p.lda + (((lane & 7) ^ (hx & 7)) << 3)) * 2 : -1;
+      hx += DX; hy += DY;
+      if (hx >= PW) { hx -= PW; ++hy; }
+    }
+  }
+  auto a_piece_at = [&](uint32_t bo, int cb, int i) {
+    const int vo = voffA[i];
+    __builtin_amdgcn_raw_ptr_buffer_load_lds(rsA, (lds_ptr_t)(smem + bo + (i * 4 + wave) * 1024), 16, vo, cb * 128, 0, 0);
+  };
+#pragma unroll
+  for (int i = 0; i < HL; ++i) a_piece_at(0u, 0, i);
+  if (1 < ncb) {
+#pragma unroll
+    for (int i = 0; i < HL; ++i) a_piece_at((uint32_t)PB, 1, i);
+  }
+
+  const uint32_t lds0 = lds_addr(smem);
+  const int fchunk = 4 * half + fq;
+  auto frag_addr = [&](int tap, uint32_t bo) -> uint32_t {
+    const int ky = tap >= 6 ? 2 : tap >= 3 ? 1 : 0, kx = tap - 3 * ky;
+    const int hx = fpx + kx;
+    return lds0 + bo + (uint32_t)(ky * PW * 128) + (uint32_t)(hx << 7) + (uint32_t)((fchunk ^ (hx & 7)) << 4);
+  };
+
+  f32x4 acc[4][TH];
+#pragma unroll
+  for (int i = 0; i < 4; ++i)
+#pragma unroll
+    for (int j = 0; j < TH; ++j) acc[i][j] = f32x4{0.f, 0.f, 0.f, 0.f};
+
+  f16x8 bf[4];
+  {
+    wait_vmcnt<0>();
+    __builtin_amdgcn_s_barrier();
+    {
+      const uint32_t a0 = frag_addr(8, 0u);
+      bf[0] = lds_read16_off<0>(a0); bf[1] = lds_read16_off<PW * 128>(a0); bf[2] = lds_read16_off<2 * PW * 128>(a0);
+    }
+    auto do_cb = [&](auto morec, auto more2c, int cb, uint32_t bo, uint32_t bo1, uint32_t bo2) {
+      constexpr bool MORE = decltype(morec)::value, MORE2 = decltype(more2c)::value;
+      auto unit = [&](auto slotc) {
+        constexpr int S = decltype(slotc)::value;
+        constexpr bool HALFU = S < 0, LAST = S == 3;
+        const int tap = HALFU ? 8 : 2 * S + pair;
+        const uint32_t a_cur = frag_addr(tap, bo);
+        const uint32_t a_nxt = LAST ? frag_addr(8, bo1) : frag_addr(HALFU ? pair : tap + 2, bo);
+        auto row = [&](auto jc) {
+          constexpr int J = decltype(jc)::value;
+          __builtin_amdgcn_sched_barrier(0);
+          if constexpr (LAST && J == 5) {
+            wait_lds_frag<0>(bf[1]);
+            if constexpr (MORE) {
+              wait_vmcnt<12>();
+              __builtin_amdgcn_s_barrier();
+            }
+          }
+          if constexpr (J < 5) bf[(J + 3) & 3] = lds_read16_off<((J + 3) & 7) * PW * 128>(a_cur);
+          else if constexpr (!LAST || MORE) bf[(J + 3) & 3] = lds_read16_off<((J + 3) & 7) * PW * 128>(a_nxt);
+          __builtin_amdgcn_sched_barrier(0);
+          wait_lds_frag<(LAST && !MORE && J >= 5) ? 0 : 3>(bf[J & 3]);
+          if constexpr (HALFU) {
+#pragma unroll
+            for (int k = 0; k < 2; ++k) acc[k][J] = __builtin_amdgcn_mfma_f32_16x16x32_f16(wh[k], bf[J & 3], acc[k][J], 0, 0, 0);
+          } else {
+#pragma unroll
+            for (int i = 0; i < 4; ++i) {
+              acc[i][J] = __builtin_amdgcn_mfma_f32_16x16x32_f16(wf[S][i], bf[J & 3], acc[i][J], 0, 0, 0);
+              if constexpr (MORE2 && S == 0) {
+                if (J * 4 + i < HL) {
+                  __builtin_amdgcn_sched_barrier(0);
+                  a_piece_at(bo2, cb + 2, J * 4 + i);
+                  __builtin_amdgcn_sched_barrier(0);
+                }
+              }
+            }
+          }
+        };
+        row(std::integral_constant<int, 0>{}); row(std::integral_constant<int, 1>{}); row(std::integral_constant<int, 2>{});
+        row(std::integral_constant<int, 3>{}); row(std::integral_constant<int, 4>{}); row(std::integral_constant<int, 5>{});
+        row(std::integral_constant<int, 6>{}); row(std::integral_constant<int, 7>{});
+        if constexpr (MORE) {
+          __builtin_amdgcn_sched_barrier(0);
+          if constexpr (HALFU) {
+#pragma unroll
+            for (int k = 0; k < 2; ++k) wh[k] = wload(k, cb + 1, 8);
+          } else {
+#pragma unroll
+            for (int i = 0; i < 4; ++i) wf[S][i] = wload(i, cb + 1, tap);
+          }
+          __builtin_amdgcn_sched_barrier(0);
+        }
+      };
+      unit(std::integral_constant<int, -1>{});
+      unit(std::integral_constant<int, 0>{});
+      unit(std::integral_constant<int, 1>{});
+      unit(std::integral_constant<int, 2>{});
+      unit(std::integral_constant<int, 3>{});
+    };
+    typedef std::true_type Y;
+    typedef std::false_type N_;
+    uint32_t bo = 0, bo1 = PB, bo2 = 2 * PB;
+    int cb = 0;
+    for (; cb + 2 < ncb; ++cb) {
+      do_cb(Y{}, Y{}, cb, bo, bo1, bo2);
+      const uint32_t t = bo; bo = bo1; bo1 = bo2; bo2 = t;
+    }
+    if (cb + 1 < ncb) {
+      do_cb(Y{}, N_{}, cb, bo, bo1, bo2);
+      ++cb;
+      bo = bo1;
+    }
+    do_cb(N_{}, N_{}, cb, bo, bo1, bo2);
+  }
+
+  if (p.A2) {
+    const int ntb = p.Cin2 >> 6;
+    const auto rsT = __builtin_amdgcn_make_buffer_rsrc((void*)p.A2, 0, (int)0x80000000u, 0x00020000);
+    const int voffT = (((img0 * H + y0) * W + x0 + fpx) * p.lda2 + 8 * fq) * 2;
+    const int rowT = W * p.lda2 * 2;
+    const int tbase = units * ncb * 72 + nr * ntb * 8;
+    f16x8 tw[2][4], tb_[2][TH];
+    auto tload = [&](auto setc, int tb) {
+      constexpr int SET = decltype(setc)::value;
+      const bool in = tb < ntb;
+#pragma unroll
+      for (int set = 0; set < 4; ++set) {
+        const int i = set ^ (2 * pair);
+        const u32x4 v = __builtin_amdgcn_raw_buffer_load_b128(rsW, in && i < ntile16 ? lane16 : OOB, (tbase + (tb * 2 + half) * 4 + i) * 1024, NTW ? 2 : 0);
+        tw[SET][set] = __builtin_bit_cast(f16x8, v);
+      }
+#pragma unroll
+      for (int j = 0; j < TH; ++j) {
+        const u32x4 v = __builtin_amdgcn_raw_buffer_load_b128(rsT, in ? voffT : OOB, j * rowT + tb * 128 + half * 64, 0);
+        tb_[SET][j] = __builtin_bit_cast(f16x8, v);
+      }
+    };
+    auto tmul = [&](auto setc) {
+      constexpr int SET = decltype(setc)::value;
+#pragma unroll
+      for (int j = 0; j < TH; ++j)
+#pragma unroll
+        for (int i = 0; i < 4; ++i) acc[i][j] = __builtin_amdgcn_mfma_f32_16x16x32_f16(tw[SET][i], tb_[SET][j], acc[i][j], 0, 0, 0);
+    };
+    int tb = pair;
+    tload(std::integral_constant<int, 0>{}, tb);
+    for (; tb < ntb; tb += 4) {
+      tload(std::integral_constant<int, 1>{}, tb + 2);
+      tmul(std::integral_constant<int, 0>{});
+      tload(std::integral_constant<int, 0>{}, tb + 4);
+      tmul(std::integral_constant<int, 1>{});
+    }
+  }
+
+  if (pair) {
+#pragma unroll
+    for (int i = 0; i < 2; ++i)
+#pragma unroll
+      for (int j = 0; j < TH; ++j) { const f32x4 t = acc[i][j]; acc[i][j] = acc[i + 2][j]; acc[i + 2][j] = t; }
+  }
+  __builtin_amdgcn_s_barrier();
+  constexpr int CB = G::CBLK;
+  const int epx = tid >> 3, c4 = tid & 7;
+  const int epxl = epx % TW, epyl = epx / TW;
+  const char* const src0 = smem + ((c4 >> 2) * TH + epyl) * CB + ((c4 & 3) * 16 + ((epxl + 4 * (c4 & 3)) & 15)) * 16;
+  const bool stats = (p.flags & GF_GNSTATS) != 0;
+  double* const sred = (double*)(smem + G::MAINB);
+#pragma unroll
+  for (int i0 = 0; i0 < 2; ++i0) {
+    if (i0 > 0) __syncthreads();
+    {
+      char* const mine = smem + wave * 2 * TH * CB + (fq * 16 + ((fpx + 4 * fq) & 15)) * 16;
+#pragma unroll
+      for (int ii = 0; ii < 2; ++ii)
+#pragma unroll
+        for (int j = 0; j < TH; ++j) *(f32x4*)(mine + (ii * TH + j) * CB) = acc[2 * i0 + ii][j];
+    }
+    __syncthreads();
+    const int n = (nr * 2 + i0) * 32 + 4 * c4;
+    const bool ncol = n + 4 <= p.N;
+    f32x4 bv = {0.f, 0.f, 0.f, 0.f};
+    if ((p.flags & GF_BIAS) && ncol) bv = *(const f32x4*)(p.bias + n);
+    float ssum[4] = {0.f, 0.f, 0.f, 0.f}, qsum[4] = {0.f, 0.f, 0.f, 0.f};
+#pragma unroll
+    for (int j = 0; j < TH / 2; ++j) {
+      const char* src = src0 + 2 * j * CB;
+      const f32x4 v0 = *(const f32x4*)src, v1 = *(const f32x4*)(src + 2 * TH * CB), v2 = *(const f32x4*)(src + 4 * TH * CB),
+                  v3 = *(const f32x4*)(src + 6 * TH * CB);
+      f32x4 v;
+#pragma unroll
+      for (int e = 0; e < 4; ++e) v[e] = ((v0[e] + v1[e]) + v2[e]) + v3[e];
+      const size_t m = ((size_t)img0 * H + y0 + 2 * j + epyl) * W + x0 + epxl;
+      if (!ncol) continue;
+#pragma unroll
+      for (int e = 0; e < 4; ++e) v[e] += bv[e];
+      if (p.flags & GF_RESID) {
+        const f16x4 r = *(const f16x4*)(p.R + m * p.ldr + n);
+#pragma unroll
+        for (int e = 0; e < 4; ++e) v[e] += (float)r[e];
+      }
+      const f16x4 o = {(f16)v[0], (f16)v[1], (f16)v[2], (f16)v[3]};
+      *(f16x4*)((f16*)p.C + m * p.ldc + n) = o;
+#pragma unroll
+      for (int e = 0; e < 4; ++e) { const float f = (float)o[e]; ssum[e] += f; qsum[e] += f * f; }
+    }
+    if (stats) {
+      double sd[4], qd[4];
+#pragma unroll
+      for (int e = 0; e < 4; ++e) {
+        sd[e] = (double)ssum[e]; qd[e] = (double)qsum[e];
+#pragma unroll
+        for (int o = 8; o < 64; o <<= 1) { sd[e] += shfl_xor_d(sd[e], o); qd[e] += shfl_xor_d(qd[e], o); }
+      }
+      if (lane < 8) {
+        double* d = sred + ((wave * 2 + i0) * 32 + 4 * c4) * 2;
+#pragma unroll
+        for (int e = 0; e < 4; ++e) { d[2 * e] = sd[e]; d[2 * e + 1] = qd[e]; }
+      }
+    }
+  }
+  if (stats) {
+    __syncthreads();
+    double* const tot = sred + 4 * 64 * 2;
+    if (tid < 128) tot[tid] = ((sred[tid] + sred[128 + tid]) + sred[256 + tid]) + sred[384 + tid];
+    __syncthreads();
+    const int cpg = p.gn_cpg, groups = p.N / cpg;
+    const int c_lo = nr * 64, c_hi = min(p.N, c_lo + 64);
+    const int g_lo = c_lo / cpg, g_hi = (c_hi - 1) / cpg;
+    const int g = g_lo + tid;
+    if (g <= g_hi) {
+      const int a = max(g * cpg, c_lo), b = min((g + 1) * cpg, c_hi);
+      double sg = 0.0, qg = 0.0;
+      for (int c = a; c < b; ++c) { sg += tot[(c - c_lo) * 2]; qg += tot[(c - c_lo) * 2 + 1]; }
+      const int ntile = tiles_x * tiles_y, pt = ty * tiles_x + tx;
+      float* const base = p.st_out + ((size_t)img0 * 2 * ntile + 2 * pt) * groups * 2;
+      float* const mine = base + (size_t)(nr & 1) * groups * 2 + g * 2;
+      mine[0] = (float)sg; mine[1] = (float)qg;
+      if (g * cpg >= c_lo && (g + 1) * cpg <= c_hi) {
+        float* const other = base + (size_t)((nr & 1) ^ 1) * groups * 2 + g * 2;
+        other[0] = 0.f; other[1] = 0.f;
+      }
+    }
+  }
+}
+
+}
+
+void dtp_conv_ws16_init() {
+  (void)hipFuncSetAttribute((const void*)convws16_kernel<true>, hipFuncAttributeMaxDynamicSharedMemorySize, G16::LDS);
+  (void)hipFuncSetAttribute((const void*)convws16_kernel<false>, hipFuncAttributeMaxDynamicSharedMemorySize, G16::LDS);
+}
+
+size_t dtp_conv_ws16_packed_elems(int Cout, int Cin, int Cin2) { return (size_t)((Cout + 63) / 64) * ((size_t)(Cin / 64) * 72 + (size_t)(Cin2 / 64) * 8) * 512; }
+
+int dtp_launch_pack_conv_ws16(const float* w, const float* w1, f16* out, int Cout, int Cin, int Cin2, hipStream_t s) {
+  if ((Cin & 63) || (Cin2 & 63) || (Cin2 > 0) != (w1 != nullptr)) { dtp_set_error("pack_conv_ws16: Cin %d / Cin2 %d must be multiples of 64", Cin, Cin2); return DTP_ERR_ARG; }
+  const long long total = (long long)dtp_conv_ws16_packed_elems(Cout, Cin, 0);
+  const int blocks = (int)((total + 255) / 256 > 65535 ? 65535 : (total + 255) / 256);
+  hipLaunchKernelGGL(pack_conv_ws16_kernel, dim3(blocks), dim3(256), 0, s, w, out, Cout, Cin, total);
+  if (Cin2 > 0) {
+    const long long t2 = (long long)dtp_conv_ws16_packed_elems(Cout, 0, Cin2);
+    const int b2 = (int)((t2 + 255) / 256 > 65535 ? 65535 : (t2 + 255) / 256);
+    hipLaunchKernelGGL(pack_conv_ws16_tail_kernel, dim3(b2), dim3(256), 0, s, w1, out + total, Cout, Cin2, t2);
+  }
+  return hipGetLastError() == hipSuccess ? DTP_OK : DTP_ERR_HIP;
+}
+
+bool dtp_conv_ws16_supported(const GemmParams& p, int nsplit) {
+  if (!p.Wfr16 || !(p.flags & GF_CONV3) || p.batch > 1 || nsplit != 1) return false;
+  if (p.A2 && ((p.Cin2 & 63) || (p.lda2 & 7) || (size_t)p.M * p.lda2 * 2 >= ((size_t)1 << 31))) return false;
+  if (p.flags & (GF_GEGLU | GF_OUT_F32 | GF_LNFOLD | GF_ROWSTATS | GF_BIAS_M | GF_GELU | GF_QUICKGELU | GF_SILU | GF_GNAPPLY | GF_SOFTMAX16)) return false;
+  if (p.stride != 1 || p.pad != 1 || (p.Cin & 63) || p.Cin < 64 || (p.N & 3) || (p.lda & 7) || (p.ldc & 3)) return false;
+  if (p.flags & GF_UPS2) { if (p.Ho != 2 * p.Hi || p.Wo != 2 * p.Wi) return false; }
+  else if (p.Ho != p.Hi || p.Wo != p.Wi) return false;
+  if ((p.flags & GF_RESID) && (p.ldr & 3)) return false;
+  if (p.Ho < 8 || p.Wo < 16 || (p.Ho & 7) || (p.Wo & 15) || p.M % (p.Ho * p.Wo)) return false;
+  if (p.flags & GF_GNSTATS) {
+    if (!p.st_out || p.gn_cpg < 4 || p.gn_cpg > 64 || (p.N % p.gn_cpg) || p.N / p.gn_cpg > 32) return false;
+  }
+  const int images = p.M / (p.Ho * p.Wo);
+  if ((size_t)images * p.Hi * p.Wi * p.lda * 2 >= ((size_t)1 << 31) || dtp_conv_ws16_packed_elems(p.N, p.Cin, p.A2 ? p.Cin2 : 0) * 2 >= ((size_t)1 << 31)) return false;
+  return true;
+}
+
+int dtp_launch_conv_ws16(const GemmParams& p, hipStream_t s) {
+  if (!dtp_conv_ws16_supported(p, p.splits)) {
+    dtp_set_error("conv_ws16: unsupported problem (M %d N %d Cin %d %dx%d flags %#x, %d slices, packing %s)", p.M, p.N, p.Cin, p.Hi, p.Wi, p.flags, p.splits,
+                  p.Wfr16 ? "present" : "missing");
+    return DTP_ERR_ARG;
+  }
+  const int npg = (p.M / (p.Ho * p.Wo)) * (p.Ho / 8) * (p.Wo / 16);
+  const int units = (p.N + 63) / 64;
+  const int blocks = (units & 7) == 0 ? units * npg : ((npg + 7) >> 3) * 8 * units;
+  if (npg == 1) hipLaunchKernelGGL((convws16_kernel<true>), dim3(blocks), dim3(256), G16::LDS, s, p);
+  else hipLaunchKernelGGL((convws16_kernel<false>), dim3(blocks), dim3(256), G16::LDS, s, p);
+  if (hipGetLastError() != hipSuccess) { dtp_set_error("conv_ws16 launch failed"); return DTP_ERR_HIP; }
+  return DTP_OK;
+}
diff --git a/diffusiontexturepainting_amd/csrc/engine.h b/diffusiontexturepainting_amd/csrc/engine.h
--- a/diffusiontexturepainting_amd/csrc/engine.h
+++ b/diffusiontexturepainting_amd/csrc/engine.h
@@ -1,4 +1,5 @@
 #pragma once
+#include <array>
 #include <deque>
 #include <functional>
 #include <map>
@@ -26,6 +27,7 @@
   f16* w = nullptr;
   f16* wcb = nullptr;
   f16* wfr = nullptr;
+  f16* wfr16 = nullptr;
   float* b = nullptr;
   float* lns = nullptr;
   int cout = 0, cin = 0 , cin_true = 0, taps = 1, K = 0, ldw = 0;
@@ -306,6 +308,9 @@
   bool fuse_reduce_gn = true;
   bool pack_ws = false;
   bool conv_ws = true, conv_ws_vae = true;
+  int conv_ws16 = 1;
+  std::map<std::array<int, 3>, int> ws_route;
+  bool ws_route_built = false;
   bool gemm_ws = false;
   bool gn_epilogue = true;
   bool reduce_in_concat_gn = true;
diff --git a/diffusiontexturepainting_amd/csrc/engine.hip b/diffusiontexturepainting_amd/csrc/engine.hip
--- a/diffusiontexturepainting_amd/csrc/engine.hip
+++ b/diffusiontexturepainting_amd/csrc/engine.hip
@@ -1,4 +1,7 @@
 #include "engine.h"
+
+#include <stdio.h>
+#include <string.h>
 
 #include <algorithm>
 
@@ -92,6 +95,28 @@
   return DTP_OK;
 }
 
+struct WsPackings { bool ws, ws16; };
+static WsPackings conv_ws_packings(Ctx* c, int cout, int cin, int cin2) {
+  if (c->conv_ws16 == 2) return {true, true};
+  if (c->conv_ws16 == 0) return {true, false};
+  if (!c->ws_route_built) {
+    for (const auto& kv : c->tuned) {
+      const DtpFamily fam = dtp_tile(kv.second.first).fam;
+      if (fam != TF_CONVWS && fam != TF_CONVWS16) continue;
+      const char* bar = strchr(kv.first.c_str(), '|');
+      int v[14];
+      if (!bar || sscanf(bar + 1, "%d,%d,%d,%d,%d,%d,%d,%d,%d,%d,%d,%d,%d,%d", v, v + 1, v + 2, v + 3, v + 4, v + 5, v + 6, v + 7, v + 8, v + 9, v + 10, v + 11,
+                         v + 12, v + 13) != 14 || !(v[3] & GF_CONV3))
+        continue;
+      c->ws_route[{v[1], v[6], v[12]}] |= fam == TF_CONVWS16 ? 2 : 1;
+    }
+    c->ws_route_built = true;
+  }
+  const auto it = c->ws_route.find({cout, cin, cin2});
+  const int r = it == c->ws_route.end() ? 1 : it->second;
+  return {r != 2, (r & 2) != 0};
+}
+
 int load_conv(Ctx* c, const std::string& name, ConvW& w, int cin_pad, bool bias) {
   const Staged* s = ctx_find(c, name + ".weight");
   if (!s) { dtp_set_error("missing weight '%s.weight'", name.c_str()); return DTP_ERR_MISSING; }
@@ -110,10 +135,18 @@
     RC(dtp_launch_pack_conv_weight_cb(s->d, w.wcb, cout, cin, w.ldw, 0));
   }
   if (c->pack_ws && taps == 9 && (cin & 63) == 0 && cout >= 32) {
+    const WsPackings pk = conv_ws_packings(c, cout, cin, 0);
     void* p3;
-    RC(ctx_arena_alloc(c, dtp_conv_ws_packed_elems(cout, cin, 0) * 2, &p3));
-    w.wfr = (f16*)p3;
-    RC(dtp_launch_pack_conv_ws(s->d, nullptr, w.wfr, cout, cin, 0, 0));
+    if (pk.ws) {
+      RC(ctx_arena_alloc(c, dtp_conv_ws_packed_elems(cout, cin, 0) * 2, &p3));
+      w.wfr = (f16*)p3;
+      RC(dtp_launch_pack_conv_ws(s->d, nullptr, w.wfr, cout, cin, 0, 0));
+    }
+    if (pk.ws16) {
+      RC(ctx_arena_alloc(c, dtp_conv_ws16_packed_elems(cout, cin, 0) * 2, &p3));
+      w.wfr16 = (f16*)p3;
+      RC(dtp_launch_pack_conv_ws16(s->d, nullptr, w.wfr16, cout, cin, 0, 0));
+    }
   }
   w.b = nullptr;
   if (bias) {
@@ -146,10 +179,18 @@
   RC(dtp_launch_pack_conv_weight_cb(s->d, w.wcb, cout, cin, w.ldw, 0));
   RC(dtp_launch_pack_conv_weight(t->d, w.wcb + 9 * cin, cout, cin2, cin2, 1, w.ldw, 0));
   if (c->pack_ws && (cin & 63) == 0 && cout >= 32) {
+    const WsPackings pk = conv_ws_packings(c, cout, cin, cin2);
     void* p3;
-    RC(ctx_arena_alloc(c, dtp_conv_ws_packed_elems(cout, cin, cin2) * 2, &p3));
-    w.wfr = (f16*)p3;
-    RC(dtp_launch_pack_conv_ws(s->d, t->d, w.wfr, cout, cin, cin2, 0));
+    if (pk.ws) {
+      RC(ctx_arena_alloc(c, dtp_conv_ws_packed_elems(cout, cin, cin2) * 2, &p3));
+      w.wfr = (f16*)p3;
+      RC(dtp_launch_pack_conv_ws(s->d, t->d, w.wfr, cout, cin, cin2, 0));
+    }
+    if (pk.ws16) {
+      RC(ctx_arena_alloc(c, dtp_conv_ws16_packed_elems(cout, cin, cin2) * 2, &p3));
+      w.wfr16 = (f16*)p3;
+      RC(dtp_launch_pack_conv_ws16(s->d, t->d, w.wfr16, cout, cin, cin2, 0));
+    }
   }
   std::vector<float> b1, b2;
   RC(ctx_fetch_host(c, conv + ".bias", b1));
diff --git a/diffusiontexturepainting_amd/csrc/gemm_conv.hip b/diffusiontexturepainting_amd/csrc/gemm_conv.hip
--- a/diffusiontexturepainting_amd/csrc/gemm_conv.hip
+++ b/diffusiontexturepainting_amd/csrc/gemm_conv.hip
@@ -755,6 +755,7 @@
     case TF_HALO: return dtp_launch_conv_halo(p, t.var, s);
     case TF_LNLIN: return dtp_launch_lnlin(p, p.col_ranges, s);
     case TF_CONVWS: return dtp_launch_conv_ws(p, t.var, s);
+    case TF_CONVWS16: return dtp_launch_conv_ws16(p, s);
     case TF_GEMMWS: return dtp_launch_gemm_ws(p, s);
     case TF_WIDE:
     case TF_FP8: {
diff --git a/diffusiontexturepainting_amd/csrc/tune.hip b/diffusiontexturepainting_amd/csrc/tune.hip
--- a/diffusiontexturepainting_amd/csrc/tune.hip
+++ b/diffusiontexturepainting_amd/csrc/tune.hip
@@ -36,6 +36,7 @@
     case TF_GEMMWS: return dtp_gemm_ws_supported(p, sp);
     case TF_LNLIN: return dtp_lnlin_supported(p, sp);
     case TF_CONVWS: return dtp_conv_ws_supported(p, t.var, sp);
+    case TF_CONVWS16: return dtp_conv_ws16_supported(p, sp);
     case TF_HALO: return p.Wcb && (t.var >= 4 ? dtp_conv_halo3_supported(p) : dtp_conv_halo_supported(p)) && p.batch <= 1;
     default: break;
   }
@@ -120,6 +121,7 @@
       add(tile, sp);
     }
   }
+  if (c->conv_ws && dtp_conv_ws16_supported(p, 1)) add(DTP_TILE_WS16, 1);
   if (gw_ok) {
     static const int slices[] = {1, 2, 3, 4, 5, 6, 8};
     for (int sp : slices)
@@ -137,7 +139,8 @@
   bool ws_ok[DTP_WS_VARIANTS];
   bool ws_any = false;
   for (int v = 0; v < DTP_WS_VARIANTS; ++v) { ws_ok[v] = p.Wfr && (p.flags & GF_CONV3) && dtp_conv_ws_supported(p, v, 1); ws_any = ws_any || ws_ok[v]; }
-  if (ws_any) kl += snprintf(key + kl, sizeof(key) - kl, ",ws2");
+  const bool w16_ok = dtp_conv_ws16_supported(p, 1);
+  if (ws_any || w16_ok) kl += snprintf(key + kl, sizeof(key) - kl, ",ws2");
   if (!(p.flags & GF_LNFOLD)) {
     bool ll = false;
     for (int r = 1; r <= 40 && !ll; ++r) ll = dtp_lnlin_supported(p, r);
@@ -198,12 +201,10 @@
     int bt = *tile, bs = *sp;
     for (size_t i = 0; i < cands.size() && i < 3; ++i)
       if (cands[i].ms < best) { best = cands[i].ms; bt = cands[i].tile; bs = cands[i].sp; }
-    if (ws_any && dtp_tile(bt).fam != TF_CONVWS && dtp_conv_output_can_carry_gn_stats(p)) {
+    if ((ws_any || w16_ok) && !dtp_tile_emits_gn_stats(bt) && dtp_tile(bt).fam != TF_CONVWS && dtp_conv_output_can_carry_gn_stats(p)) {
       const float stats_ms = 0.005f + (float)((double)p.M * p.N * 2.0 / 4.0e12 * 1e3);
-      for (const Cand& cd : cands) {
-        const DtpTile t = dtp_tile(cd.tile);
-        if (cd.sp == 1 && t.fam == TF_CONVWS && t.var >= 2 && cd.ms - stats_ms < best) { best = cd.ms - stats_ms; bt = cd.tile; bs = 1; }
-      }
+      for (const Cand& cd : cands)
+        if (cd.sp == 1 && dtp_tile_emits_gn_stats(cd.tile) && cd.ms - stats_ms < best) { best = cd.ms - stats_ms; bt = cd.tile; bs = 1; }
     }
     it = c->tuned.emplace(key, std::make_pair(bt, bs)).first;
     if (getenv("DTP_TUNE_REPORT")) {
diff --git a/diffusiontexturepainting_amd/ops.py b/diffusiontexturepainting_amd/ops.py
--- a/diffusiontexturepainting_amd/ops.py
+++ b/diffusiontexturepainting_amd/ops.py
@@ -51,6 +51,17 @@
     w = w.contiguous().float()
     w1 = w1.reshape(cout, cin2).contiguous().float() if w1 is not None else None
     check(lib.dtp_op_pack_conv_ws(ptr(w), ptr(w1), ptr(out), cout, cin, cin2, _stream()), "pack_conv_ws")
+    return out
+
+
+def pack_conv_ws16(w, w1=None):
+    lib = _lib.load()
+    cout, cin = w.shape[:2]
+    cin2 = w1.shape[1] if w1 is not None else 0
+    out = torch.zeros(lib.dtp_op_pack_conv_ws16_elems(cout, cin, cin2), dtype=torch.float16, device=w.device)
+    w = w.contiguous().float()
+    w1 = w1.reshape(cout, cin2).contiguous().float() if w1 is not None else None
+    check(lib.dtp_op_pack_conv_ws16(ptr(w), ptr(w1), ptr(out), cout, cin, cin2, _stream()), "pack_conv_ws16")
     return out
 
 
diff --git a/include/dtp.h b/include/dtp.h
--- a/include/dtp.h
+++ b/include/dtp.h
@@ -238,6 +238,9 @@
 int dtp_op_pack_conv_cb(const float* w, void* out, int Cout, int Cin, int ldw, dtp_stream s);
 int dtp_op_pack_conv_ws(const float* w, const float* w1, void* out, int Cout, int Cin, int Cin2, dtp_stream s);
 long long dtp_op_pack_conv_ws_elems(int Cout, int Cin, int Cin2);
+int dtp_op_pack_conv_ws16(const float* w, const float* w1, void* out, int Cout, int Cin, int Cin2, dtp_stream s);
+long long dtp_op_pack_conv_ws16_elems(int Cout, int Cin, int Cin2);
+void dtp_op_pack_conv_ws16_map(int Cin, int tail, long long first, long long count, int* out);
 int dtp_op_pack_linear_ws(const void* w, int ldw, void* out, int N, int K, dtp_stream s);
 long long dtp_op_pack_linear_ws_elems(int N, int K);
 int dtp_op_groupnorm(const void* x, int ldx, void* y, int ldy, const float* gamma, const float* beta, int B, int HW, int C,
```

Result: no change. 10.37, median of 6 (+0.1%).
